# Zokrates/ZoKrates

Hardware: AMD Instinct MI355X
Metric: groth16_proofs_per_sec (higher is better)
Workload: dtype u32

## Files before the change

### zokrates_amd/csrc/core.cuh

```cuda
#pragma once
#include <algorithm>
#include <atomic>
#include <chrono>
#include <cstdio>
#include <memory>
#include <new>
#include <string>
#include <system_error>
#include <thread>
#include <type_traits>
#include <unordered_set>
#include <vector>

#include "../../include/zkhip.h"
#include "devrt.h"
#include "ntt_geom.h"
#include "msm_geom.h"
#include "ec.cuh"
#include "kernels_msm.cuh"
#include "kernels_ntt.cuh"
#include "zpack.cuh"
#include "wingest.cuh"
#include "wplan.h"
#include "wexec.cuh"
#include "xplan.h"

namespace zk {

struct CurveBn254 {
    static constexpr int ID = ZKHIP_CURVE_BN128;
    typedef Fe<Bn254Fr> Fr;
    typedef Fe<Bn254Fq> Fq;
    typedef Fe2<Bn254Fq> Fq2;
    static constexpr u64 GENERATOR = 5;
    static constexpr int TWO_ADICITY = 28;
    static const u32* g1_gen() { static const u32 t[] = {0x00000001u, 0x00000000u, 0x00000000u, 0x00000000u, 0x00000000u, 0x00000000u, 0x00000000u, 0x00000000u, 0x00000002u, 0x00000000u, 0x00000000u, 0x00000000u, 0x00000000u, 0x00000000u, 0x00000000u, 0x00000000u}; return t; }
    static const u32* g2_gen() { static const u32 t[] = {0xd992f6edu, 0x46debd5cu, 0xf75edaddu, 0x674322d4u, 0x5e5c4479u, 0x426a0066u, 0x121f1e76u, 0x1800deefu, 0xaef312c2u, 0x97e485b7u, 0x35a9e712u, 0xf1aa4933u, 0x31fb5d25u, 0x7260bfb7u, 0x920d483au, 0x198e9393u, 0x66fa7daau, 0x4ce6cc01u, 0x0c43d37bu, 0xe3d1e769u, 0x8dcb408fu, 0x4aab7180u, 0xdb8c6debu, 0x12c85ea5u, 0xd122975bu, 0x55acdadcu, 0x70b38ef3u, 0xbc4b3133u, 0x690c3395u, 0xec9e99adu, 0x585ff075u, 0x090689d0u}; return t; }
};
struct CurveBls381 {
    static constexpr int ID = ZKHIP_CURVE_BLS12_381;
    typedef Fe<Bls381Fr> Fr;
    typedef Fe<Bls381Fq> Fq;
    typedef Fe2<Bls381Fq> Fq2;
    static constexpr u64 GENERATOR = 7;
    static constexpr int TWO_ADICITY = 32;
    static const u32* g1_gen() { static const u32 t[] = {0xdb22c6bbu, 0xfb3af00au, 0xf97a1aefu, 0x6c55e83fu, 0x171bac58u, 0xa14e3a3fu, 0x9774b905u, 0xc3688c4fu, 0x4fa9ac0fu, 0x2695638cu, 0x3197d794u, 0x17f1d3a7u, 0x46c5e7e1u, 0x0caa2329u, 0xa2888ae4u, 0xd03cc744u, 0x2c04b3edu, 0x00db18cbu, 0xd5d00af6u, 0xfcf5e095u, 0x741d8ae4u, 0xa09e30edu, 0xe3aaa0f1u, 0x08b3f481u}; return t; }
    static const u32* g2_gen() { static const u32 t[] = {0xc121bdb8u, 0xd48056c8u, 0xa805bbefu, 0x0bac0326u, 0x7ae3d177u, 0xb4510b64u, 0xfa403b02u, 0xc6e47ad4u, 0x2dc51051u, 0x26080527u, 0xf08f0a91u, 0x024aa2b2u, 0x5d042b7eu, 0xe5ac7d05u, 0x13945d57u, 0x334cf112u, 0xdc7f5049u, 0xb5da61bbu, 0x9920b61au, 0x596bd0d0u, 0x88274f65u, 0x7dacd3a0u, 0x52719f60u, 0x13e02b60u, 0x08b82801u, 0xe1935486u, 0x3baca289u, 0x923ac9ccu, 0x5160d12cu, 0x6d429a69u, 0x8cbdd3a7u, 0xadfd9baau, 0xda2e351au, 0x8cc9cdc6u, 0x727d6e11u, 0x0ce5d527u, 0xf05f79beu, 0xaaa9075fu, 0x5cec1da1u, 0x3f370d27u, 0x572e99abu, 0x267492abu, 0x85a763afu, 0xcb3e287eu, 0x2bc28b99u, 0x32acd2b0u, 0x2ea734ccu, 0x0606c4a0u}; return t; }
};
struct CurveBls377 {
    static constexpr int ID = ZKHIP_CURVE_BLS12_377;
    typedef Fe<Bls377Fr> Fr;
    typedef Fe<Bls377Fq> Fq;
    typedef Fe2<Bls377Fq> Fq2;
    static constexpr u64 GENERATOR = 22;
    static constexpr int TWO_ADICITY = 47;
    static const u32* g1_gen() { static const u32 t[] = {0xb21be9efu, 0xeab9b16eu, 0xffcd394eu, 0xd5481512u, 0xbd37cb5cu, 0x188282c8u, 0xaa9d41bbu, 0x85951e2cu, 0xbf87ff54u, 0xc8fc6225u, 0xfe740a67u, 0x008848deu, 0x559c8ea6u, 0xfd82de55u, 0x34a9591au, 0xc2fe3d36u, 0x4fb82305u, 0x6d182ad4u, 0xca3e52d9u, 0xbd7fb348u, 0x30afeec4u, 0x1f674f5du, 0xc5102effu, 0x01914a69u}; return t; }
    static const u32* g2_gen() { static const u32 t[] = {0x7c005196u, 0x74e3e48fu, 0xbb535402u, 0x71889f52u, 0x57db6b9bu, 0x7ea501f5u, 0x203e5031u, 0xc565f071u, 0xa3841d01u, 0xc89630a2u, 0x71c785feu, 0x018480beu, 0x6ea16afeu, 0xb26bfefau, 0xbff76fe6u, 0x5cf89984u, 0x0799c9deu, 0xe7223eceu, 0x6651cecbu, 0x532777eeu, 0xb1b140d5u, 0x70dc5a51u, 0xe7004031u, 0x00ea6040u, 0x09fd4ddfu, 0xf0940944u, 0x6d8c7c2eu, 0xf2cf8888u, 0xf832d204u, 0xe458c282u, 0x74b49a58u, 0xde03ed72u, 0xcbb2efb4u, 0xd960736bu, 0x5d446f7bu, 0x00690d66u, 0x85eb8f93u, 0xd9a1cdd1u, 0x5e52270bu, 0x4279b83fu, 0xcee304c2u, 0x2463b01au, 0x3d591bf1u, 0x61ef11acu, 0x151a70aau, 0x9e549da3u, 0xd2835518u, 0x00f8169fu}; return t; }
};

struct ApiError {
    int32_t code;
    std::string msg;
};
static inline void require(bool ok, int32_t code, const char* msg) {
    if (!ok) throw ApiError{code, msg};
}
static const char* const Z0_NOT_ONE_MSG = "z[0] must be 1 (ark instance variable 0 is the constant ONE)";

struct DBuf {
    void* p = nullptr;
    size_t cap = 0;
    DBuf() {}
    DBuf(const DBuf&) = delete;
    DBuf& operator=(const DBuf&) = delete;
    ~DBuf() { dev_free(p); }
    void swap(DBuf& o) { std::swap(p, o.p); std::swap(cap, o.cap); }
    void release() { dev_free(p); p = nullptr; cap = 0; }
    void ensure(size_t bytes) {
        if (bytes <= cap) return;
        dev_free(p);
        p = nullptr;
        cap = 0;
        p = dev_alloc(bytes);
        cap = bytes;
    }
};
template <class T> static inline T* ptr(const DBuf& b) { return (T*)b.p; }

static inline unsigned blocks_for(u64 n, unsigned threads) { return (unsigned)((n + threads - 1) / threads); }
static inline int ilog2_floor(u64 x) { int l = 0; while (x >>= 1) ++l; return l; }
static inline int ilog2_ceil(u64 x) { int l = 0; while (((u64)1 << l) < x) ++l; return l; }

}

using namespace zk;

struct NttPlanBase {
    int curve, logN;
    virtual ~NttPlanBase() {}
};
struct MsmSort {
    DBuf dig, sorted, cnt, off, cursor, chunk_sum, grand;
    DBuf pairs, ccur, tile_off;
    Event ready = nullptr;
};
struct MsmLane {
    Stream stream = 0;
    bool made = false;
    bool high_priority = false;
    DBuf lane_key, heavy, partial, bucket, rows, cols;
    Event done = nullptr;
};
static constexpr int ZK_NLANES = 5;
static constexpr int ZK_NSLOTS = 4;
struct ProofSlot {
    DBuf scalars, zmont, va, vb, vc, ws1, ws2, zflag;
    DBuf verdict;
    int check_idx = -1;
    MsmSort sorts[3];
    MsmLane lanes[ZK_NLANES];
    void* h_ws = nullptr;
    size_t h_ws_cap = 0;
    Event ev[4] = {nullptr, nullptr, nullptr, nullptr};
    Event acc_b[ZK_NLANES] = {}, acc_e[ZK_NLANES] = {};
    Event ntt_b = nullptr, ntt_e = nullptr;
    Event g1_go = nullptr;
    Event half_ready = nullptr;
    int half = -1;
    bool lone = false;
    bool split_pending = false;
    const zkhip_pk* split_pk = nullptr;
    const zkhip_r1cs* split_cs = nullptr;
    bool split_bound = false;
    bool ready = false;
    bool busy = false;
    uint8_t r[32], s[32];
    std::shared_ptr<const WPlanTables> wit;
    void* h_inputs = nullptr;
    size_t h_inputs_cap = 0;
    std::chrono::steady_clock::time_point t_start;
};
struct PackedZ {
    const uint8_t* bytes;
    size_t len;
    u64 tags_off, index_off, payload_off;
};
struct zkhip_wplan;
struct WitnessZ {
    const uint8_t* bytes;
    size_t len;
    u64 count;
    const zkhip_wplan* plan;
};
struct zkhip_queue {
    zkhip_ctx* ctx = nullptr;
    const zkhip_pk* pk = nullptr;
    const zkhip_r1cs* cs = nullptr;
    u32 cap = 0;
    u64 head = 0, next = 0;
    bool checked = false;
    bool broken = false;
    std::string dev_err;
};
struct zkhip_ctx {
    int device = 0;
    Stream stream = 0;
    Stream out_stream = 0;
    Stream ntt_stream = 0;
    bool out_made = false, ntt_made = false;
    Stream ws = 0;
    bool serial = false;
    bool g2_first = true;
    MsmKnobs msm;
    int b_sort_mode = 0;
    bool fuse_z = true;
    int z_gate = 1;
    int g2_head_start = 1;
    int split_min_log = 18;
    int ntt_single_max = 10;
    int ntt_max_sublog = 11;
    int ntt_cols = 2;
    std::vector<Stream> idle_streams;
    std::string pipe_plan;
    bool pipes_made = false;
    Stream ntt_lone_stream = 0;
    bool ntt_lone_made = false;
    int ntt_fuse_first = 1;
    int tenants = 1;
    int nslots = 3;
    bool checked = false;
    struct Unsatisfied { u32 proof; u64 first_row, n_bad; };
    std::vector<Unsatisfied> unsat;
    std::string err;
    std::string desc;
    ProofSlot slots[ZK_NSLOTS];
    ProofSlot* cur = &slots[0];
    zkhip_queue* queue = nullptr;
    DBuf tmp;
    DBuf wraw, wowner;
    Stream verify_stream = 0;
    bool verify_made = false;
    DBuf vfy[11];
    Stream exec_stream = 0;
    bool exec_made = false;
    DBuf xstore, xargs, xverdict, xptrs, xfile, xinputs;
    int exec_chunk = 0;
    bool exec_wide = false;
    int exec_wide_min = 0;
    u64 exec_last[4] = {0, 0, 0, 0};
    DBuf zpack;
    std::vector<std::unique_ptr<NttPlanBase>> plans;
    std::unordered_set<const void*> lds_opted;
    struct Shard {
        DBuf send[2], recv, out;
        Event packed[2] = {nullptr, nullptr};
        unsigned turn = 0;
        std::vector<uint8_t> host;
    } shard;
};
#define ZK_PIPE_PLAN_RESIDENT "M=2,N=3,O=1,n=3,G0=0,Z0=1,H0=0,G1=3,Z1=1,H1=0,G2=3,Z2=2,H2=1"
struct PipeWant { Stream* target; bool* made; bool high; int cls; bool done; };
static inline void make_pipe_streams(zkhip_ctx* ctx) {
    if (ctx->pipes_made || ctx->pipe_plan.empty() || ctx->serial) return;
    ctx->pipes_made = true;
    auto find = [&](const std::string& key) -> int {
        size_t pos = 0;
        const std::string& pl = ctx->pipe_plan;
        while (pos < pl.size()) {
            size_t end = pl.find(',', pos);
            if (end == std::string::npos) end = pl.size();
            const std::string tok = pl.substr(pos, end - pos);
            const size_t eq = tok.find('=');
            if (eq != std::string::npos && tok.substr(0, eq) == key && eq + 1 < tok.size() && tok[eq + 1] >= '0' && tok[eq + 1] <= '3') return tok[eq + 1] - '0';
            pos = end + 1;
        }
        return -1;
    };
    std::vector<PipeWant> want;
    static bool dummy_made;
    int c;
    if ((c = find("M")) >= 0) { stream_sync(ctx->stream); stream_destroy(ctx->stream); ctx->stream = 0; want.push_back({&ctx->stream, &dummy_made, true, c, false}); }
    if ((c = find("N")) >= 0 && !ctx->ntt_made) want.push_back({&ctx->ntt_stream, &ctx->ntt_made, true, c, false});
    if ((c = find("n")) >= 0) want.push_back({&ctx->ntt_lone_stream, &ctx->ntt_lone_made, true, c, false});
    if ((c = find("O")) >= 0 && !ctx->out_made) want.push_back({&ctx->out_stream, &ctx->out_made, false, c, false});
    static const char names[3] = {'Z', 'G', 'H'};
    static const int lane_of[3] = {0, 3, 4};
    for (int k = 0; k < std::min(ctx->nslots, ZK_NSLOTS); ++k)
        for (int t = 0; t < 3; ++t) {
            MsmLane& lane = ctx->slots[k].lanes[lane_of[t]];
            const std::string up(1, names[t]);
            c = find(up + std::to_string(k)); if (c < 0) c = find(up);
            if (c >= 0 && !lane.made) want.push_back({&lane.stream, &lane.made, t == 1 && ctx->g2_first, c, false});
        }
    size_t left = want.size();
    for (int t = 0; left; ++t) {
        PipeWant* pick = nullptr;
        for (auto& w : want) if (!w.done && w.cls == (t & 3)) { pick = &w; break; }
        if (pick) { *pick->target = pick->high ? stream_create_high_priority() : stream_create(); *pick->made = true; pick->done = true; --left; }
        else ctx->idle_streams.push_back(stream_create_low_priority());
    }
    ctx->ws = ctx->stream;
}
static inline void slot_init(zkhip_ctx* ctx, ProofSlot& sl) {
    if (sl.ready) return;
    for (auto& so : sl.sorts) so.ready = event_create();
    for (int k = 0; k < ZK_NLANES; ++k) {
        sl.lanes[k].high_priority = k == 3 && ctx->g2_first;
        sl.lanes[k].done = event_create();
        sl.acc_b[k] = event_create();
// ... 770 lines not shown
    }
    static void export_image(zkhip_pk* pk, uint8_t* out, u64 cap) {
        zkhip_ctx* ctx = pk->ctx;
        require(cap >= export_size(pk), ZKHIP_ERR_BAD_ARG, "output buffer too small (see zkhip_pk_export_size)");
        PkImageHeader h;
        memset(&h, 0, sizeof(h));
        memcpy(h.magic, PK_IMAGE_MAGIC, 8);
        h.curve = pk->curve; h.scheme = pk->scheme;
        h.m = pk->m; h.w = pk->w; h.l = pk->l; h.hlen = pk->hlen; h.N = pk->N;
        h.logN = pk->logN; h.c_z = pk->c_z; h.c_h = pk->c_h; h.sets = pk->s_z | (pk->s_h << 8);
        h.rank = pk->rank; h.world = pk->world;
        h.ntt_split = pk->ntt_log1;
        h.z_lo = pk->z_lo; h.z_n = pk->z_n; h.h_lo = pk->h_lo; h.h_n = pk->h_n;
        h.len_delta = pk->delta_g1_canon.size(); h.len_g2z2 = pk->g_gamma2_z2_canon.size();
        const bool with_bound = pk->h_bound.p && pk->l_bound.p;
        if (with_bound) {
            h.len_bound[0] = table_bytes<Fq>(pk->h_n, 1);
            h.len_bound[1] = table_bytes<Fq>(pk->z_n, 1);
            h.bound_fp[0] = pk->bound_fp[0]; h.bound_fp[1] = pk->bound_fp[1];
        }
        uint8_t* p = out + sizeof(h);
        memcpy(p, pk->delta_g1_canon.data(), h.len_delta); p += h.len_delta;
        memcpy(p, pk->g_gamma2_z2_canon.data(), h.len_g2z2); p += h.len_g2z2;
        for_each_table(pk, [&](int k, DBuf& b, auto f, u64, u64 n) {
            h.len_buf[k] = table_bytes<typename decltype(f)::type>(n, 1);
            dev_d2h(p, b.p, h.len_buf[k], ctx->stream);
            p += h.len_buf[k];
        });
        memcpy(out, &h, sizeof(h));
        if (with_bound) {
            dev_d2h(p, pk->h_bound.p, h.len_bound[0], ctx->stream); p += h.len_bound[0];
            dev_d2h(p, pk->l_bound.p, h.len_bound[1], ctx->stream); p += h.len_bound[1];
        }
        stream_sync(ctx->stream);
    }
    static void import_image(zkhip_ctx* ctx, const uint8_t* bytes, size_t len, zkhip_pk* pk) {
        PkImageHeader h;
        memcpy(&h, bytes, sizeof(h));
        require(h.scheme == 0 || h.scheme == 1, ZKHIP_ERR_PARSE, "key image: unknown scheme");
        u64 total = sizeof(PkImageHeader), rest = len - sizeof(PkImageHeader);
        const u64 parts[9] = {h.len_delta, h.len_g2z2, h.len_buf[0], h.len_buf[1], h.len_buf[2], h.len_buf[3], h.len_buf[4], h.len_bound[0], h.len_bound[1]};
        for (u64 part : parts) {
            require(part <= rest, ZKHIP_ERR_PARSE, "key image truncated");
            rest -= part;
            total += part;
        }
        require(total == len, ZKHIP_ERR_PARSE, "trailing bytes after key image");
        int s_z = h.sets & 0xff, s_h = (h.sets >> 8) & 0xff;
        require(h.world >= 1 && h.rank < h.world && h.logN >= 0 && h.logN <= 3 * NTT_MAX_SUBLOG && h.N == ((u64)1 << h.logN) && h.z_n <= h.m + 2 &&
                    h.h_n <= h.N && h.c_z >= 2 && h.c_z <= MSM_MAX_C && h.c_h >= 2 && h.c_h <= MSM_MAX_C && s_z >= 1 && s_h >= 1 && (h.sets >> 16) == 0,
                ZKHIP_ERR_PARSE, "key image: inconsistent header");
        pk->scheme = h.scheme;
        pk->m = h.m; pk->w = h.w; pk->l = h.l; pk->hlen = h.hlen; pk->N = h.N; pk->logN = h.logN;
        pk->c_z = h.c_z; pk->c_h = h.c_h; pk->rank = h.rank; pk->world = h.world;
        pk->z_lo = h.z_lo; pk->z_n = h.z_n; pk->h_lo = h.h_lo; pk->h_n = h.h_n;
        pk->ntt_log1 = h.ntt_split;
        auto shape_z = [&](int sets) { return msm_shape(&ctx->msm,h.z_n, C::Fr::Params::BITS, true, h.c_z, sets); };
        auto shape_h = [&](int sets) { return msm_shape(&ctx->msm,h.h_n, C::Fr::Params::BITS, true, h.c_h, sets); };
        bool sizes_ok = h.m + 2 < ((u64)1 << 31) && h.z_lo <= h.m + 2 && h.z_n <= h.m + 2 - h.z_lo && h.h_lo <= h.N && h.h_n <= h.N - h.h_lo &&
                        h.len_delta <= 4096 && h.len_g2z2 <= 4096;
        for_each_table(pk, [&](int k, DBuf&, auto f, u64, u64 n) {
            sizes_ok = sizes_ok && h.len_buf[k] == table_bytes<typename decltype(f)::type>(n, 1);
        });
        const bool with_bound = h.len_bound[0] || h.len_bound[1];
        if (with_bound)
            sizes_ok = sizes_ok && h.len_bound[0] == table_bytes<Fq>(h.h_n, 1) && h.len_bound[1] == table_bytes<Fq>(h.z_n, 1) && (h.bound_fp[0] | h.bound_fp[1]) != 0;
        require(sizes_ok, ZKHIP_ERR_PARSE, "key image: array sizes do not match the header");
        require(get_plan<C>(ctx, h.logN)->split() == h.ntt_split, ZKHIP_ERR_PARSE,
                "key image: written under another NTT split (NTT_SINGLE_MAX_LOG / NTT_MAX_SUBLOG) than this context uses; re-import the proving key");
        {
            const int W_z = shape_z(1).W, W_h = shape_h(1).W;
            const int fixed = ctx->msm.msm_sets;
            const u64 budget = msm_table_budget(ctx, h.z_n, h.h_n, h.N, W_z, shape_z(1).K);
            if (fixed) s_z = std::min(fixed, W_z), s_h = std::min(fixed, W_h);
            else {
                const MsmSets s = msm_pick_sets({s_z, s_h}, {W_z, W_h}, {W_z, W_h}, budget, [&](MsmSets t) { return tables_need(pk, shape_z(t.z), shape_h(t.h)); });
                s_z = s.z, s_h = s.h;
            }
        }
        const MsmShape shz = shape_z(s_z), shh = shape_h(s_h);
        require(shz.c == h.c_z && (int)shz.sets == s_z && shh.c == h.c_h && (int)shh.sets == s_h, ZKHIP_ERR_PARSE,
                "key image: window width / bucket sets not usable under this context's settings; re-import the proving key");
        pk->s_z = s_z; pk->s_h = s_h;
        const uint8_t* p = bytes + sizeof(h);
        pk->delta_g1_canon.assign(p, p + h.len_delta); p += h.len_delta;
        pk->g_gamma2_z2_canon.assign(p, p + h.len_g2z2); p += h.len_g2z2;
        for_each_table(pk, shz, shh, [&](int k, DBuf& b, auto f, u64, u64 n, const MsmShape& sh) {
            b.ensure(table_bytes<typename decltype(f)::type>(n, sh.levels));
            const uint8_t* src = p;
            dev_h2d_fill(b.p, h.len_buf[k], 64, ctx->stream, [src](char* out, size_t off, size_t len) { memcpy(out, src + off, len); });
            p += h.len_buf[k];
        });
        stream_sync(ctx->stream);
        table_levels(ctx, pk);
        if (with_bound) install_bound(ctx, pk, p, p + h.len_bound[0], false, h.bound_fp);
    }
    static void count_points_at_infinity(zkhip_ctx* ctx, zkhip_pk* pk) {
        u64 cnt[5];
        for_each_table(pk, [&](int k, DBuf& b, auto f, u64, u64 n) {
            cnt[k] = count_infinite<typename decltype(f)::type>(ctx, b.p, n);
            pk->inf_many[k] = cnt[k] * 2048 > n;
        });
        const bool gm17 = pk->scheme == 1;
        u32 family = 0;
        if (ctx->b_sort_mode == 1) family = gm17 ? 0xbu : 0xau;
        else if (ctx->b_sort_mode == 0)
            for (int k = 0; k < 4; ++k)
                if (cnt[k] * 10 > pk->z_n) family |= 1u << k;
        pk->thin_mask = 0;
        pk->thin_keep.release();
        if (family && pk->z_n) {
            const size_t words = (size_t)((pk->z_n + 31) / 32);
            pk->thin_keep.ensure(words * 4);
            dev_memset(pk->thin_keep.p, 0, words * 4, ctx->stream);
            for_each_table(pk, [&](int k, DBuf& b, auto f, u64, u64 n) {
                if (family >> k & 1) mark_finite<typename decltype(f)::type>(ctx, b.p, n, ptr<u32>(pk->thin_keep));
            });
            std::vector<u32> host(words);
            dev_d2h(host.data(), pk->thin_keep.p, words * 4, ctx->stream);
            stream_sync(ctx->stream);
            u64 left_out = 0;
            for (u64 i = 0; i < pk->z_n; ++i) left_out += !((host[i >> 5] >> (i & 31)) & 1u);
            if (ctx->b_sort_mode == 1 || left_out * 10 > pk->z_n) {
                pk->thin_mask = family;
                for (int k = 0; k < 4; ++k) pk->inf_many_thin[k] = (cnt[k] - std::min(cnt[k], left_out)) * 2048 > pk->z_n;
            } else {
                pk->thin_keep.release();
            }
        }
    }
    template <class F>
    static void to_table(zkhip_ctx* ctx, DBuf& buf, u64 lo, u64 count, const MsmShape& sh) {
        DBuf out;
        out.ensure(table_bytes<F>(count, sh.levels));
        if (count) points_to_packed<F>(ctx, ptr<Aff<F>>(buf) + lo, out.p, count);
        stream_sync(ctx->stream);
        buf.swap(out);
        out.release();
        msm_table_levels<F>(ctx, buf.p, count, sh.level_bits(), (int)sh.levels);
    }
};

template <class C>
struct Prover {
    typedef typename C::Fr Fr;
    typedef typename C::Fq Fq;
    typedef typename C::Fq2 Fq2;
    typedef SlotSums<C> Lay;
    typedef Transforms<C> Tr;
    static constexpr int FQB = Fq::BYTES;

    static CsrDev csr(const zkhip_r1cs* cs, int k) { return CsrDev{ptr<u64>(cs->rp[k]), ptr<u32>(cs->col[k]), cs->val[k].p}; }

    static void matvec(zkhip_ctx* ctx, const zkhip_r1cs* cs, const Fr* zmont, Fr* a, Fr* b, Fr* c, u64 n, u64 l, u64 N, int nmat = 3, int mat0 = 0) {
        int g[3];
        matvec_lanes(cs, g, nmat, mat0);
        ZK_LAUNCH((k_matvec<Fr>), dim3(blocks_for(N, 256 / gmax_rows(g)), nmat), dim3(256), 0, ctx->ws, csr(cs, 0), csr(cs, 1), csr(cs, 2), zmont, a, b, c, n,
                  l, N, g[0], g[1], g[2], cs->l + cs->w, mat0);
        if (cs->n_huge)
            ZK_LAUNCH((k_matvec_huge<Fr>), dim3((unsigned)cs->n_huge), dim3(MATVEC_HUGE_THREADS), 0, ctx->ws, csr(cs, 0), csr(cs, 1), csr(cs, 2), zmont, a, b, c,
                      ptr<u64>(cs->long_rows), cs->l + cs->w);
        if (cs->n_long > cs->n_huge)
            ZK_LAUNCH((k_matvec_long<Fr>), dim3(blocks_for(cs->n_long - cs->n_huge, 4)), dim3(256), 0, ctx->ws, csr(cs, 0), csr(cs, 1), csr(cs, 2), zmont, a, b, c,
                      ptr<u64>(cs->long_rows) + cs->n_huge, cs->n_long - cs->n_huge, cs->l + cs->w);
    }
    static unsigned gmax_rows(const int g[3]) { return (unsigned)std::max(g[0], std::max(g[1], g[2])); }

    static void witness_map(zkhip_ctx* ctx, const zkhip_r1cs* cs, NttPlan<C>* pl, bool bound = false, int half = -1, bool check = false) {
        Stream s = ctx->ws;
        const u64 N = pl->N;
        ctx->cur->va.ensure(3 * N * sizeof(Fr));
        Fr *a = ptr<Fr>(ctx->cur->va), *b = a + N, *c = b + N;
        if (half >= 0) {
            Fr* v = a + (u64)half * N;
            matvec(ctx, cs, ptr<Fr>(ctx->cur->zmont), a, b, c, cs->n, cs->l, N, 1, half);
            event_record(ctx->cur->ntt_b, s);
            Tr::ntt_kind_a(ctx, pl, v, true, ptr<Fr>(pl->s_coset), 1, 0);
            Tr::ntt_kind_b(ctx, pl, v, false, nullptr, 1, 0);
            event_record(ctx->cur->ntt_e, s);
            return;
        }
        matvec(ctx, cs, ptr<Fr>(ctx->cur->zmont), a, b, c, cs->n, cs->l, N, (bound && !check) ? 2 : 3);
        if (check) enqueue_check(*ctx->cur, a, b, c, cs->n, s);
        event_record(ctx->cur->ntt_b, s);
        Tr::ntt_quotient(ctx, pl, a, 2, c, bound, [&](const Fr& zinv) {
            ZK_LAUNCH((k_quotient<typename Fr::Params>), dim3(blocks_for(N, 256)), dim3(256), 0, s, a, b, zinv, a, N);
        });
        event_record(ctx->cur->ntt_e, s);
    }

    static void verdict_reset(ProofSlot& sl, Stream st) {
        sl.verdict.ensure(16);
        dev_memset(sl.verdict.p, 0xff, 8, st);
        dev_memset((uint8_t*)sl.verdict.p + 8, 0, 8, st);
    }
    static void enqueue_check(ProofSlot& sl, const Fr* a, const Fr* b, const Fr* c, u64 n, Stream s) {
        ZK_LAUNCH((k_r1cs_check<typename Fr::Params>), dim3(blocks_for(n, 256)), dim3(256), 0, s, a, b, c, n, ptr<unsigned long long>(sl.verdict));
    }
    static bool unsatisfied(zkhip_ctx* ctx, const ProofSlot& sl, const Lay& ly) {
        if (sl.check_idx < 0) return false;
        u64 v[2];
        memcpy(v, ly.verdict(sl), 16);
        if (!v[1]) return false;
        ctx->unsat.push_back({(u32)sl.check_idx, v[0], v[1]});
        return true;
    }
    static void raise_unsatisfied(const zkhip_ctx* ctx, u32 count, const zkhip_r1cs* cs) {
        if (ctx->unsat.empty()) return;
        const auto& u = ctx->unsat.front();
        char msg[200];
        snprintf(msg, sizeof(msg), "proof %u of %u: constraint %llu of %llu is not satisfied (%llu in all)", u.proof, count, (unsigned long long)u.first_row,
                 (unsigned long long)cs->n, (unsigned long long)u.n_bad);
        throw ApiError{ZKHIP_ERR_UNSATISFIED, msg};
    }
    static void r1cs_check(zkhip_ctx* ctx, const zkhip_r1cs* cs, const uint8_t* z_host, const void* z_dev, u64 out[2]) {
        ProofSlot& sl = *ctx->cur;
        Stream s = ctx->stream;
        ctx->ws = s;
        const u64 m = cs->l + cs->w, n = cs->n;
        const Fr* z = stage_z(ctx, sl, m, m + 2, z_host, z_dev, true, true);
        sl.zmont.ensure(m * 32);
        ZK_LAUNCH((k_mul_const<Fr>), dim3(blocks_for(m, 256)), dim3(256), 0, s, z, ptr<Fr>(sl.zmont), m, fe_to_mont(rp_factor<Fr>()));
        sl.vc.ensure(3 * std::max<u64>(n, 1) * sizeof(Fr));
        Fr *ra = ptr<Fr>(sl.vc), *rb = ra + n, *rc = rb + n;
        if (n) matvec(ctx, cs, ptr<Fr>(sl.zmont), ra, rb, rc, n, 0, n);
        enqueue_check(sl, ra, rb, rc, n, s);
        u32 flag = 0;
        dev_d2h(&flag, sl.zflag.p, 4, s);
        dev_d2h(out, sl.verdict.p, 16, s);
        stream_sync(s);
        require_canonical(flag);
    }

    static void upload_z(zkhip_ctx* ctx, DBuf& dst, u64 m, u64 cap, const uint8_t* z, DBuf& flag) {
        Fr z0 = fe_from_bytes_canon<Fr>(z);
        Fr one = Fr::zero(); one.v[0] = 1;
        require(z0.equals(one), ZKHIP_ERR_BAD_ARG, Z0_NOT_ONE_MSG);
        dst.ensure(cap * 32);
        dev_h2d(dst.p, z, m * 32, ctx->stream);
        flag.ensure(4);
        dev_memset(flag.p, 0, 4, ctx->stream);
        ZK_LAUNCH((k_check_canonical<Fr>), dim3(blocks_for(m, 256)), dim3(256), 0, ctx->stream, ptr<Fr>(dst), m, ptr<u32>(flag));
    }
    static void unpack_z(zkhip_ctx* ctx, DBuf& dst, u64 m, u64 cap, const PackedZ& zp, DBuf& flag) {
        Stream s = ctx->stream;
        dst.ensure(cap * 32);
        ctx->zpack.ensure(zp.len);
        dev_h2d(ctx->zpack.p, zp.bytes, zp.len, s);
        flag.ensure(4);
        dev_memset(flag.p, 0, 4, s);
        const uint8_t* d = ptr<uint8_t>(ctx->zpack);
        ZK_LAUNCH((k_unpack_assignment<Fr>), dim3(blocks_for(m, ZPACK_BLOCK_ELEMS)), dim3(256), 0, s, d + zp.tags_off, (const u64*)(d + zp.index_off),
                  d + zp.payload_off, ptr<Fr>(dst), m, ptr<u32>(flag));
    }
    static void ingest_z(zkhip_ctx* ctx, DBuf& dst, u64 m, u64 cap, const WitnessZ& wz, DBuf& flag) {
        Stream s = ctx->stream;
        const zkhip_wplan* plan = wz.plan;
        const u64 slots = (wz.len + 15) / 16;
        dst.ensure(cap * 32);
        ctx->wraw.ensure(slots * 16);
        ctx->wowner.ensure(m * 4);
        dev_h2d(ctx->wraw.p, wz.bytes, wz.len, s);
        dev_memset(ctx->wowner.p, 0, m * 4, s);
        flag.ensure(16);
        dev_memset(flag.p, 0, 8, s);
        dev_memset((uint8_t*)flag.p + 8, 0xff, 8, s);
        ZK_LAUNCH((k_witness_claim<Fr>), dim3(blocks_for(wz.count, WIT_BLOCK)), dim3(WIT_BLOCK), 0, s, ptr<uint4>(ctx->wraw), slots, wz.count, ptr<u32>(plan->pos),
                  (u64)plan->host->pos.size(), ptr<u32>(plan->neg), (u64)plan->host->neg.size(), witness_id_bound(wz.count), ptr<u32>(ctx->wowner), ptr<u32>(flag));
        ZK_LAUNCH((k_witness_gather<Fr>), dim3(blocks_for(m, WIT_BLOCK)), dim3(WIT_BLOCK), 0, s, ptr<uint8_t>(ctx->wraw), ptr<u32>(ctx->wowner), ptr<Fr>(dst), m,
                  ptr<u32>(flag), (unsigned long long*)((uint8_t*)flag.p + 8));
    }
    static void require_verdict(u32 flag, u32 low, const WPlanTables* wit) {
        require(!(flag & WIT_FLAG_NON_CANONICAL), ZKHIP_ERR_PARSE, "non-canonical field element in the witness");
        require(!(flag & WIT_FLAG_ID_RANGE), ZKHIP_ERR_PARSE, "variable id out of range in the witness");
        if (flag & WIT_FLAG_MISSING) {
            const std::string name = wit && low < wit->order.size() ? witness_var_name(wit->order[low]) : "column " + std::to_string(low);
            throw ApiError{ZKHIP_ERR_UNSATISFIED, "assignment missing for variable " + name};
        }
        require_canonical(flag);
    }
    static void require_verdict(const ProofSlot& sl, const Lay& ly) {
        u32 low = 0;
        memcpy(&low, ly.zflag(sl) + 4, 4);
        require_verdict(ly.zflag_word(sl), low, sl.wit.get());
    }
    static const Fr* stage_z(zkhip_ctx* ctx, ProofSlot& sl, u64 m, u64 cap, const uint8_t* z_host, const void* z_dev, bool checked, bool in_place = false,
                             const PackedZ* zp = nullptr, const WitnessZ* wz = nullptr) {
        Stream st = ctx->stream;
        sl.wit.reset();
        if (wz) {
            const u64 l = wz->plan->host->l;
            if (sl.h_inputs_cap < l * 32) {
                host_free_pinned(sl.h_inputs);
                sl.h_inputs = nullptr; sl.h_inputs_cap = 0;
                sl.h_inputs = host_alloc_pinned(l * 32);
                sl.h_inputs_cap = l * 32;
            }
            ingest_z(ctx, sl.scalars, m, cap, *wz, sl.zflag);
            dev_d2h_pinned(sl.h_inputs, sl.scalars.p, l * 32, st);
            sl.wit = wz->plan->host;
            if (checked) verdict_reset(sl, st);
            return ptr<Fr>(sl.scalars);
        }
        if (zp) {
            unpack_z(ctx, sl.scalars, m, cap, *zp, sl.zflag);
            if (checked) verdict_reset(sl, st);
            return ptr<Fr>(sl.scalars);
        }
        if (z_host) {
            upload_z(ctx, sl.scalars, m, cap, z_host, sl.zflag);
        } else {
            if (!in_place) {
                sl.scalars.ensure(cap * 32);
                dev_d2d(sl.scalars.p, z_dev, m * 32, st);
            }
            sl.zflag.ensure(4);
            dev_memset(sl.zflag.p, 0, 4, st);
        }
        if (checked) verdict_reset(sl, st);
        return (z_host || !in_place) ? ptr<Fr>(sl.scalars) : (const Fr*)z_dev;
    }
    static void require_canonical(u32 flag) {
        require(flag == 0, ZKHIP_ERR_BAD_ARG, "an assignment entry is not a canonical field element (>= r)");
    }
    static void stage_scalars(zkhip_ctx* ctx, NttPlan<C>* pl, void* d_scalars, u64 m, const uint8_t* r, const uint8_t* s_) {
        Stream s = ctx->stream;
        ctx->cur->zmont.ensure(m * 32);
        dev_h2d((uint8_t*)d_scalars + m * 32, r, 32, s);
        dev_h2d((uint8_t*)d_scalars + (m + 1) * 32, s_, 32, s);
        ZK_LAUNCH((k_mul_const<Fr>), dim3(blocks_for(m, 256)), dim3(256), 0, s, (const Fr*)d_scalars, ptr<Fr>(ctx->cur->zmont), m, pl->k_to_rp);
    }

    static void enqueue(zkhip_ctx* ctx, ProofSlot& sl, const zkhip_pk* pk, const zkhip_r1cs* cs, const uint8_t* z_host, const void* z_dev,
                        const uint8_t* r, const uint8_t* s_, bool lone = false, int check_idx = -1, const PackedZ* zp = nullptr,
                        const WitnessZ* wz = nullptr) {
        enqueue_head(ctx, sl, pk, cs, z_host, z_dev, r, s_, lone, -1, check_idx, zp, wz);
        enqueue_tail(ctx, sl, pk, cs);
    }
    static bool can_split(const zkhip_ctx* ctx, const zkhip_pk* pk, const zkhip_r1cs* cs) {
        return pk->scheme == 0 && is_bound(pk, cs) && pk->logN >= ctx->split_min_log;
    }
    static bool is_bound(const zkhip_pk* pk, const zkhip_r1cs* cs) { return pk->bound_uid != 0 && pk->bound_uid == cs->uid; }
    static NttPlan<C>* open_slot(zkhip_ctx* ctx, ProofSlot& sl, const zkhip_pk* pk) {
        require(!sl.busy, ZKHIP_ERR_DEVICE, "internal: proof slot still in flight");
        make_pipe_streams(ctx);
        slot_init(ctx, sl);
        NttPlan<C>* pl = get_plan<C>(ctx, pk->logN);
        require(pl->split() == pk->ntt_log1, ZKHIP_ERR_BAD_ARG, "the key's h bases were ordered for another NTT split (NTT_SINGLE_MAX_LOG changed): reload the key");
        sl.t_start = std::chrono::steady_clock::now();
        ctx->cur = &sl;
        ctx->ws = ctx->stream;
        return pl;
    }
    static void enqueue_head(zkhip_ctx* ctx, ProofSlot& sl, const zkhip_pk* pk, const zkhip_r1cs* cs, const uint8_t* z_host, const void* z_dev,
                             const uint8_t* r, const uint8_t* s_, bool lone, int half, int check_idx = -1, const PackedZ* zp = nullptr,
                             const WitnessZ* wz = nullptr) {
        PkLoader<C>::check_match(pk, cs, 0);
        const bool bound = is_bound(pk, cs);
        require(half < 0 || (bound && half <= 1), ZKHIP_ERR_BAD_ARG, "internal: only a proof over a bound key splits its witness map");
        Fr rr = fe_from_bytes_canon<Fr>(r), ss = fe_from_bytes_canon<Fr>(s_);
        require(canon_lt_mod(rr) && canon_lt_mod(ss), ZKHIP_ERR_BAD_ARG, "r or s not a canonical field element");
        NttPlan<C>* pl = open_slot(ctx, sl, pk);
        sl.half = half;
        sl.lone = lone;
        sl.check_idx = half < 0 ? check_idx : -1;
        memcpy(sl.r, r, 32);
        memcpy(sl.s, s_, 32);
        Stream st = ctx->stream;
        stage_z(ctx, sl, pk->m, pk->m + 2, z_host, z_dev, sl.check_idx >= 0, false, zp, wz);
        stage_scalars(ctx, pl, sl.scalars.p, pk->m, r, s_);
        event_record(sl.ev[0], st);

        const Lay ly(ctx, pk);
        ly.reserve(sl);
        start_z_lanes(ctx, sl, pk, ly);

        Stream wn = ctx->serial ? st : slot_ntt_stream(ctx, sl);
        stream_wait_event(wn, sl.ev[0]);
        event_record(sl.ev[1], wn);
        ctx->ws = wn;
        witness_map(ctx, cs, pl, bound, half, sl.check_idx >= 0);
        ctx->ws = ctx->stream;
        if (half >= 0) {
            event_record(sl.half_ready, wn);
            sl.split_pk = pk;
            sl.split_cs = cs;
            sl.split_bound = bound;
            sl.split_pending = true;
        }
    }
    static void enqueue_tail(zkhip_ctx* ctx, ProofSlot& sl, const zkhip_pk* pk, const zkhip_r1cs* cs) {
        const u64 N = pk->N;
        ctx->cur = &sl;
        Stream wn = ctx->serial ? ctx->stream : slot_ntt_stream(ctx, sl);
        const u32* h_scalars = ptr<u32>(sl.va) + (sl.half >= 0 ? 2 * N * 8 : 0);
        if (sl.half >= 0) {
            Fr* a = ptr<Fr>(sl.va);
            ZK_LAUNCH((k_quotient<typename Fr::Params>), dim3(blocks_for(N, 256)), dim3(256), 0, wn, a, a + N, fe_from_mont(get_plan<C>(ctx, pk->logN)->zinv), a + 2 * N, N);
        }
        lanes_after_h(ctx, sl, pk, Lay(ctx, pk), sl.half >= 0 ? sl.split_bound : is_bound(pk, cs), sl.lone, h_scalars, wn);
    }

    static void start_z_lanes(zkhip_ctx* ctx, ProofSlot& sl, const zkhip_pk* pk, const Lay& ly) {
        if (!pk->z_n) return;
        const u32* digits = ptr<u32>(sl.scalars) + pk->z_lo * 8;
        msm_prepare(ctx, ctx->stream, sl.sorts[0], digits, ly.shz, pk->z_n);
        if (pk->thin_mask) msm_prepare(ctx, ctx->stream, sl.sorts[2], digits, ly.shz, pk->z_n, ptr<u32>(pk->thin_keep), &sl.sorts[0]);
        if (z_gate(ctx) < 2) run_g2(ctx, sl, pk, ly, nullptr);
    }
    static void run_g2(zkhip_ctx* ctx, ProofSlot& sl, const zkhip_pk* pk, const Lay& ly, Event after) {
        const bool thin = pk->thin_mask & 8;
        msm_run<Fq2>(ctx, sl.lanes[3], sl.sorts[thin ? 2 : 0], pk->b2_ext.p, with_inf(ly.shz, thin ? pk->inf_many_thin[3] : pk->inf_many[3]), ly.ws2(sl),
                     sl.acc_b[4], sl.acc_e[4], after, ly.hs2(sl));
    }
    static void lanes_after_h(zkhip_ctx* ctx, ProofSlot& sl, const zkhip_pk* pk, const Lay& ly, bool bound, bool lone, const u32* h_scalars, Stream wn) {
        Stream st = ctx->stream;
        event_record(sl.ev[2], wn);
        if (pk->z_n) {
            const int gate = z_gate(ctx);
            const Event h_ready = gate ? sl.ev[2] : nullptr;
            if (gate >= 2) run_g2(ctx, sl, pk, ly, h_ready);
            Event g1_after = h_ready;
            constexpr bool g2_owns_simds = MsmTuning<typename Unsat<Fq2>::type>::ACCUM_WPE == 1;
            if (g2_owns_simds && lone && !ctx->serial && (ctx->g2_head_start == 2 || (ctx->g2_head_start == 1 && bound))) {
                if (h_ready) stream_wait_event(st, h_ready);
                stream_wait_event(st, sl.acc_e[4]);
                event_record(sl.g1_go, st);
                g1_after = sl.g1_go;
            }
            run_z_g1(ctx, sl, pk, ly, g1_after, bound);
        } else {
            empty_msm(ctx, sl, ly, true);
        }
        if (pk->h_n) {
            msm_prepare(ctx, wn, sl.sorts[1], h_scalars + pk->h_lo * 8, ly.shh, pk->h_n);
            msm_run<Fq>(ctx, sl.lanes[4], sl.sorts[1], bound ? pk->h_bound.p : pk->h_sigma.p, with_inf(ly.shh, bound ? pk->inf_many_bound[1] : pk->inf_many[4]),
                        ly.ws1(sl, 3), sl.acc_b[3], sl.acc_e[3], nullptr, ly.hs1(sl, 3));
        } else {
            empty_msm(ctx, sl, ly, false);
        }
        copy_out(ctx, sl, ly);
    }

    static void run_z_g1(zkhip_ctx* ctx, ProofSlot& sl, const zkhip_pk* pk, const Lay& ly, Event h_ready, bool bound) {
        const void* tab[3] = {pk->a_ext.p, pk->b1_ext.p, bound ? pk->l_bound.p : pk->l_ext.p};
        auto thin = [&](int k) { return (bound && k == 2) ? 0u : (pk->thin_mask >> k) & 1u; };
        auto inf_many = [&](int k) { return (bound && k == 2) ? pk->inf_many_bound[0] : thin(k) ? pk->inf_many_thin[k] : pk->inf_many[k]; };
        if (!ctx->fuse_z) {
            for (int k = 0; k < 3; ++k)
                msm_run<Fq>(ctx, sl.lanes[k], thin(k) ? sl.sorts[2] : sl.sorts[0], tab[k], with_inf(ly.shz, inf_many(k)), ly.ws1(sl, k), sl.acc_b[k], sl.acc_e[k], h_ready,
                            ly.hs1(sl, k));
            return;
        }
        for (u32 which = 0; which < 2; ++which) {
            int member[3], nm = 0;
            for (int k = 0; k < 3; ++k)
                if (thin(k) == which) member[nm++] = k;
            if (!nm) continue;
            const int lead = member[0];
            const void* tabs[3];
            bool many = false;
            for (int q = 0; q < nm; ++q) { tabs[q] = tab[member[q]]; many = many || inf_many(member[q]); }
            const int step = nm > 1 ? member[1] - member[0] : 1;
            msm_run_tables<Fq>(ctx, sl.lanes[lead], which ? sl.sorts[2] : sl.sorts[0], tabs, nm, with_inf(ly.shz, many), ly.ws1(sl, lead), (u32)(step * ly.Wmax),
                               sl.acc_b[lead], sl.acc_e[lead], h_ready, ly.hs1(sl, lead));
            Stream s0 = ctx->serial ? ctx->stream : lane_stream(sl.lanes[lead]);
            for (int q = 1; q < nm; ++q) {
                event_record(sl.acc_b[member[q]], s0);
                event_record(sl.acc_e[member[q]], s0);
                event_record(sl.lanes[member[q]].done, s0);
            }
        }
    }

    static void copy_out(zkhip_ctx* ctx, ProofSlot& sl, const Lay& ly) {
        Stream st = ctx->stream;
        Stream so = ctx->serial ? st : ctx_out_stream(ctx);
        for (int k = 0; k < ZK_NLANES; ++k) stream_wait_event(so, sl.lanes[k].done);
        sl.zflag.ensure(4);
        dev_d2h_pinned(ly.zflag(sl), sl.zflag.p, 4, so);
        if (sl.wit) dev_d2h_pinned(ly.zflag(sl) + 4, (const uint8_t*)sl.zflag.p + 8, 4, so);
        if (sl.check_idx >= 0) {
            stream_wait_event(so, sl.ev[2]);
            dev_d2h_pinned(ly.verdict(sl), sl.verdict.p, 16, so);
        }
        event_record(sl.ev[3], so);
        sl.busy = true;
    }

    static void empty_msm(zkhip_ctx* ctx, ProofSlot& sl, const Lay& ly, bool over_z) {
        Stream st = ctx->stream;
        const int k0 = over_z ? 0 : 3, nk = over_z ? 3 : 1;
        dev_memset(ly.ws1(sl, k0), 0, nk * ly.lane_bytes(), st);
        memset(ly.hs1(sl, k0), 0, nk * ly.lane_bytes());
        if (over_z) {
            dev_memset(ly.ws2(sl), 0, ly.b2(), st);
            memset(ly.hs2(sl), 0, ly.b2());
        }
        for (int k = over_z ? 0 : 4; k < (over_z ? 4 : 5); ++k) {
            const int e = k == 3 ? 4 : k == 4 ? 3 : k;
            event_record(sl.acc_b[e], st);
            event_record(sl.acc_e[e], st);
            event_record(sl.lanes[k].done, st);
        }
    }

    struct Sums {
        Xyzz<Fq> a, b1, l, h;
        Xyzz<Fq2> b2;
    };
    static Sums collect(zkhip_ctx* ctx, ProofSlot& sl, const zkhip_pk* pk) {
        require(sl.busy, ZKHIP_ERR_DEVICE, "internal: no proof in flight in this slot");
        event_sync(sl.ev[3]);
        sl.busy = false;
        split_clear(sl);
        const Lay ly(ctx, pk);
        require_verdict(sl, ly);
        Sums g;
        HostThreads th;
        th.run([&] { g.a = msm_combine(ly.hs1(sl, 0), ly.shz); });
        th.run([&] { g.b1 = msm_combine(ly.hs1(sl, 1), ly.shz); });
        th.run([&] { g.l = msm_combine(ly.hs1(sl, 2), ly.shz); });
        th.run([&] { g.h = msm_combine(ly.hs1(sl, 3), ly.shh); });
// ... 38 lines not shown
        out[8 * FQB] = inf_a; out[8 * FQB + 1] = inf_b; out[8 * FQB + 2] = inf_c;
    }
    static constexpr size_t PROOF_BYTES = 8 * FQB + 3;
    static void fill_timings(ProofSlot& sl, zkhip_timings* tm, std::chrono::steady_clock::time_point t_fin) {
        const auto t_end = std::chrono::steady_clock::now();
        if (tm) {
            memset(tm, 0, sizeof(*tm));
            for (int k = 0; k < 4; ++k) tm->msm_z_ms = std::max(tm->msm_z_ms, event_elapsed_ms(sl.ev[0], sl.lanes[k].done));
            tm->ntt_ms = event_elapsed_ms(sl.ev[1], sl.ev[2]);
            tm->kernel_ntt_ms = event_elapsed_ms(sl.ntt_b, sl.ntt_e);
            tm->msm_h_ms = event_elapsed_ms(sl.ev[2], sl.lanes[4].done);
            tm->finish_ms = std::chrono::duration<float, std::milli>(t_end - t_fin).count();
            tm->total_ms = std::chrono::duration<float, std::milli>(t_end - sl.t_start).count();
            for (int k = 0; k < 4; ++k) tm->kernel_msm_accum_g1_ms += event_elapsed_ms(sl.acc_b[k], sl.acc_e[k]);
            tm->kernel_msm_accum_g2_ms = event_elapsed_ms(sl.acc_b[4], sl.acc_e[4]);
        }
    }
    static void finish(zkhip_ctx* ctx, ProofSlot& sl, const zkhip_pk* pk, uint8_t* out, zkhip_timings* tm) {
        require(pk->world == 1, ZKHIP_ERR_BAD_ARG, "this proving key is one shard of a multi-GPU key: use zkhip_prove_g16_partial + zkhip_combine_g16");
        require(sl.busy, ZKHIP_ERR_DEVICE, "internal: no proof in flight in this slot");
        const Lay ly(ctx, pk);
        const Fr rr = fe_from_bytes_canon<Fr>(sl.r), ss = fe_from_bytes_canon<Fr>(sl.s);
        Sums g;
        Xyzz<Fq> sA, rB1, rsD;
        std::chrono::steady_clock::time_point t_fin;
        try {
            HostThreads th;
            th.run([&] { rsD = rs_delta(pk, rr, ss); });
            event_sync(sl.lanes[3].done);
            g.b2 = msm_combine(ly.hs2(sl), ly.shz);
            for (int k = 0; k < 3; ++k) event_sync(sl.lanes[k].done);
            g.a = msm_combine(ly.hs1(sl, 0), ly.shz);
            g.b1 = msm_combine(ly.hs1(sl, 1), ly.shz);
            th.run([&] { sA = xyzz_mul_limbs(g.a, ss.v, Fr::N); });
            th.run([&] { rB1 = xyzz_mul_limbs(g.b1, rr.v, Fr::N); });
            g.l = msm_combine(ly.hs1(sl, 2), ly.shz);
            event_sync(sl.lanes[4].done);
            t_fin = std::chrono::steady_clock::now();
            g.h = msm_combine(ly.hs1(sl, 3), ly.shh);
            event_sync(sl.ev[3]);
            th.join();
        } catch (...) {
            sl.busy = false;
            throw;
        }
        sl.busy = false;
        require_verdict(sl, ly);
        if (unsatisfied(ctx, sl, ly)) memset(out, 0, PROOF_BYTES);
        else assemble_tail(g, sA, rB1, rsD, out);
        fill_timings(sl, tm, t_fin);
    }
    static Xyzz<Fq> rs_delta(const zkhip_pk* pk, const Fr& rr, const Fr& ss) {
        const Fr rs = fe_from_mont(fe_mul(fe_to_mont(rr), fe_to_mont(ss)));
        uint8_t dec[2 * FQB];
        decode_point<FQB, 2>(pk->delta_g1_canon.data(), dec);
        Aff<Fq> d1;
        memcpy(&d1, dec, sizeof(d1));
        d1 = PkLoader<C>::to_mont_point(d1);
        return xyzz_mul_limbs(Xyzz<Fq>::from_affine(d1), rs.v, Fr::N);
    }
    template <class F>
    static Xyzz<F> canonical(const Xyzz<F>& p) {
        if (p.is_inf()) return Xyzz<F>::inf();
        const Aff<F> a = xyzz_to_affine(p);
        return {a.x, a.y, F::one(), F::one()};
    }
    static void emit_partial(zkhip_ctx* ctx, ProofSlot& sl, const zkhip_pk* pk, uint8_t* partial_out, zkhip_timings* tm) {
        Sums g = collect(ctx, sl, pk);
        const auto t_fin = std::chrono::steady_clock::now();
        HostThreads th;
        th.run([&] { g.a = canonical(g.a); });
        th.run([&] { g.b1 = canonical(g.b1); });
        th.run([&] { g.l = canonical(g.l); });
        th.run([&] { g.h = canonical(g.h); });
        g.b2 = canonical(g.b2);
        th.join();
        memcpy(partial_out, &g, sizeof(g));
        fill_timings(sl, tm, t_fin);
    }
    static void prove_partial(zkhip_ctx* ctx, const zkhip_pk* pk, const zkhip_r1cs* cs, const uint8_t* z_host, const void* z_dev, const uint8_t* r,
                              const uint8_t* s_, uint8_t* partial_out, zkhip_timings* tm) {
        enqueue(ctx, ctx->slots[0], pk, cs, z_host, z_dev, r, s_);
        emit_partial(ctx, ctx->slots[0], pk, partial_out, tm);
    }
    static void split_begin(zkhip_ctx* ctx, const zkhip_pk* pk, const zkhip_r1cs* cs, const uint8_t* z_host, const void* z_dev, const uint8_t* r,
                            const uint8_t* s_, int half) {
        require(is_bound(pk, cs) && pk->scheme == 0 && (half == 0 || half == 1), ZKHIP_ERR_BAD_ARG,
                "only a Groth16 proof over a key bound to its constraint system splits its witness map (half = 0: a, 1: b)");
        enqueue_head(ctx, ctx->slots[0], pk, cs, z_host, z_dev, r, s_, false, half);
    }
    static const void* split_half_ptr(zkhip_ctx* ctx, const zkhip_pk* pk, int half) { return ptr<Fr>(ctx->slots[0].va) + (u64)half * pk->N; }
    static void split_clear(ProofSlot& sl) {
        sl.split_pending = false;
        sl.split_pk = nullptr;
        sl.split_cs = nullptr;
        sl.half = -1;
    }
    static ProofSlot& split_slot(zkhip_ctx* ctx, const zkhip_pk* pk, Stream* wn = nullptr) {
        ProofSlot& s0 = ctx->slots[0];
        require(s0.split_pending && s0.half >= 0, ZKHIP_ERR_BAD_ARG, "no split proof pending in this context");
        require(s0.split_pk == pk, ZKHIP_ERR_BAD_ARG, "the split proof pending in this context was begun with another proving key");
        if (wn) *wn = ctx->serial ? ctx->stream : ctx_ntt_stream(ctx);
        return ctx->slots[0];
    }
    static void split_fetch(zkhip_ctx* ctx, const zkhip_pk* pk, const void* src, int src_device, Event src_ready) {
        Stream wn;
        ProofSlot& sl = split_slot(ctx, pk, &wn);
        if (src_ready) event_sync(src_ready);
        dev_copy_between(ptr<Fr>(sl.va) + (u64)(1 - sl.half) * pk->N, ctx->device, src, src_device, pk->N * sizeof(Fr), wn);
    }
    static void split_fetch_host(zkhip_ctx* ctx, const zkhip_pk* pk, const uint8_t* other_half) {
        Stream wn;
        ProofSlot& sl = split_slot(ctx, pk, &wn);
        dev_h2d(ptr<Fr>(sl.va) + (u64)(1 - sl.half) * pk->N, other_half, pk->N * sizeof(Fr), wn);
    }
    static void split_half_out(zkhip_ctx* ctx, const zkhip_pk* pk, uint8_t* out) {
        Stream wn;
        ProofSlot& sl = split_slot(ctx, pk, &wn);
        dev_d2h(out, ptr<Fr>(sl.va) + (u64)sl.half * pk->N, pk->N * sizeof(Fr), wn);
        stream_sync(wn);
    }
    static void split_end_partial(zkhip_ctx* ctx, const zkhip_pk* pk, const zkhip_r1cs* cs, uint8_t* partial_out, zkhip_timings* tm) {
        ProofSlot& sl = split_slot(ctx, pk);
        require(sl.split_cs == cs, ZKHIP_ERR_BAD_ARG, "the split proof pending in this context was begun with another constraint system");
        enqueue_tail(ctx, sl, pk, cs);
        emit_partial(ctx, ctx->slots[0], pk, partial_out, tm);
    }
    static void split_end_device_sums(zkhip_ctx* ctx, const zkhip_pk* pk, const zkhip_r1cs* cs, const void** d_ws1, size_t* b1, const void** d_ws2, size_t* b2,
                                      zkhip_timings* tm) {
        ProofSlot& sl = split_slot(ctx, pk);
        require(sl.split_cs == cs, ZKHIP_ERR_BAD_ARG, "the split proof pending in this context was begun with another constraint system");
        enqueue_tail(ctx, sl, pk, cs);
        hand_out_sums(ctx, ctx->slots[0], pk, d_ws1, b1, d_ws2, b2, tm);
    }
    static int can_shard(zkhip_ctx* ctx, const zkhip_pk* pk, const zkhip_r1cs* cs, u32 G, u32 k) {
        if (pk->scheme != 0 || is_bound(pk, cs)) return -1;
        const NttPlan<C>* pl = get_plan<C>(ctx, pk->logN);
        return (Tr::shard_ok(pl, G) && pk->h_lo == (u64)k * (pl->N / G) && pk->h_n == pl->N / G) ? pl->split() : -1;
    }
    static void shard_begin(zkhip_ctx* ctx, const zkhip_pk* pk, const zkhip_r1cs* cs, const uint8_t* z_host, const uint8_t* r, const uint8_t* s_, u32 G, u32 k) {
        ProofSlot& sl = ctx->slots[0];
        PkLoader<C>::check_match(pk, cs, 0);
        require(z_host && pk->scheme == 0 && !is_bound(pk, cs), ZKHIP_ERR_BAD_ARG, "internal: only a Groth16 proof over an unbound key shards its witness map");
        Fr rr = fe_from_bytes_canon<Fr>(r), ss = fe_from_bytes_canon<Fr>(s_);
        require(canon_lt_mod(rr) && canon_lt_mod(ss), ZKHIP_ERR_BAD_ARG, "r or s not a canonical field element");
        NttPlan<C>* pl = open_slot(ctx, sl, pk);
        sl.half = -1;
        sl.lone = false;
        sl.check_idx = -1;
        memcpy(sl.r, r, 32);
        memcpy(sl.s, s_, 32);
        Stream st = ctx->stream;
        stage_z(ctx, sl, pk->m, pk->m + 2, z_host, nullptr, false);
        stage_scalars(ctx, pl, sl.scalars.p, pk->m, r, s_);
        event_record(sl.ev[0], st);
        const Lay ly(ctx, pk);
        ly.reserve(sl);
        start_z_lanes(ctx, sl, pk, ly);
        Stream wn = ctx->serial ? st : slot_ntt_stream(ctx, sl);
        stream_wait_event(wn, sl.ev[0]);
        event_record(sl.ev[1], wn);
        ctx->ws = wn;
        shard_witness_map(ctx, cs, pl, G, k, 0, nullptr);
        ctx->ws = ctx->stream;
        sl.split_pk = pk;
        sl.split_cs = cs;
        sl.split_bound = false;
        sl.split_pending = true;
    }
    static ProofSlot& shard_slot(zkhip_ctx* ctx, const zkhip_pk* pk, const zkhip_r1cs* cs) {
        ProofSlot& s0 = ctx->slots[0];
        require(s0.split_pending && s0.half < 0 && s0.split_pk == pk && s0.split_cs == cs, ZKHIP_ERR_BAD_ARG, "no sharded proof of these handles pending in this context");
        return s0;
    }
    static void shard_step(zkhip_ctx* ctx, const zkhip_pk* pk, const zkhip_r1cs* cs, u32 G, u32 k, int step, zkhip_ctx* const* members) {
        ProofSlot& sl = shard_slot(ctx, pk, cs);
        ctx->cur = &sl;
        ctx->ws = ctx->serial ? ctx->stream : slot_ntt_stream(ctx, sl);
        shard_witness_map(ctx, cs, get_plan<C>(ctx, pk->logN), G, k, step, members);
        ctx->ws = ctx->stream;
    }
    static void shard_end_partial(zkhip_ctx* ctx, const zkhip_pk* pk, const zkhip_r1cs* cs, uint8_t* partial_out, zkhip_timings* tm) {
        ProofSlot& sl = shard_slot(ctx, pk, cs);
        enqueue_tail(ctx, sl, pk, cs);
        emit_partial(ctx, ctx->slots[0], pk, partial_out, tm);
    }
    static void shard_end_device_sums(zkhip_ctx* ctx, const zkhip_pk* pk, const zkhip_r1cs* cs, const void** d_ws1, size_t* b1, const void** d_ws2, size_t* b2,
                                      zkhip_timings* tm) {
        ProofSlot& sl = shard_slot(ctx, pk, cs);
        enqueue_tail(ctx, sl, pk, cs);
        hand_out_sums(ctx, ctx->slots[0], pk, d_ws1, b1, d_ws2, b2, tm);
    }
    static void prove_device_sums(zkhip_ctx* ctx, const zkhip_pk* pk, const zkhip_r1cs* cs, const uint8_t* z_host, const uint8_t* r,
                                  const uint8_t* s_, const void** d_ws1, size_t* b1, const void** d_ws2, size_t* b2, zkhip_timings* tm) {
        enqueue(ctx, ctx->slots[0], pk, cs, z_host, nullptr, r, s_);
        hand_out_sums(ctx, ctx->slots[0], pk, d_ws1, b1, d_ws2, b2, tm);
    }
    static void hand_out_sums(zkhip_ctx* ctx, ProofSlot& sl, const zkhip_pk* pk, const void** d_ws1, size_t* b1, const void** d_ws2, size_t* b2,
                              zkhip_timings* tm) {
        require(sl.busy, ZKHIP_ERR_DEVICE, "internal: no proof in flight in this slot");
        event_sync(sl.ev[3]);
        sl.busy = false;
        split_clear(sl);
        const Lay ly(ctx, pk);
        *b1 = ly.b1();
        *b2 = ly.b2();
        require_canonical(ly.zflag_word(sl));
        *d_ws1 = sl.ws1.p;
        *d_ws2 = sl.ws2.p;
        fill_timings(sl, tm, std::chrono::steady_clock::now());
    }
    static void record_from_sums(zkhip_ctx* ctx, const zkhip_pk* pk, const uint8_t* ws1, const uint8_t* ws2, uint8_t* record_out) {
        const Lay ly(ctx, pk);
        std::vector<Xyzz<Fq>> a1(ly.b1() / sizeof(Xyzz<Fq>));
        std::vector<Xyzz<Fq2>> a2(ly.b2() / sizeof(Xyzz<Fq2>));
        memcpy(a1.data(), ws1, ly.b1());
        memcpy(a2.data(), ws2, ly.b2());
        Sums g;
        g.a = msm_combine(ly.lane(a1.data(), 0), ly.shz);
        g.b1 = msm_combine(ly.lane(a1.data(), 1), ly.shz);
        g.l = msm_combine(ly.lane(a1.data(), 2), ly.shz);
        g.h = msm_combine(ly.lane(a1.data(), 3), ly.shh);
        g.b2 = msm_combine(a2.data(), ly.shz);
        memcpy(record_out, &g, sizeof(g));
    }
    static Sums sum_partials(u32 count, const uint8_t* partials) {
        Sums t;
        t.a = t.b1 = t.l = t.h = Xyzz<Fq>::inf();
        t.b2 = Xyzz<Fq2>::inf();
        for (u32 i = 0; i < count; ++i) {
            Sums g;
            memcpy(&g, partials + (size_t)i * sizeof(Sums), sizeof(g));
            t.a = xyzz_add(t.a, g.a); t.b1 = xyzz_add(t.b1, g.b1); t.l = xyzz_add(t.l, g.l); t.h = xyzz_add(t.h, g.h);
            t.b2 = xyzz_add(t.b2, g.b2);
        }
        return t;
    }
    static void combine(const zkhip_pk* pk, u32 count, const uint8_t* partials, const uint8_t* r, const uint8_t* s_, uint8_t* out) {
        const Sums t = sum_partials(count, partials);
        Fr rr = fe_from_bytes_canon<Fr>(r), ss = fe_from_bytes_canon<Fr>(s_);
        require(canon_lt_mod(rr) && canon_lt_mod(ss), ZKHIP_ERR_BAD_ARG, "r or s not a canonical field element");
        assemble(pk, t, r, s_, out);
    }
    static constexpr size_t PARTIAL_BYTES = sizeof(Sums);

    static void prove(zkhip_ctx* ctx, const zkhip_pk* pk, const zkhip_r1cs* cs, const uint8_t* z_host, const void* z_dev, const uint8_t* r, const uint8_t* s_,
                      uint8_t* out, zkhip_timings* tm) {
        ctx->unsat.clear();
        enqueue(ctx, ctx->slots[0], pk, cs, z_host, z_dev, r, s_, true, ctx->checked ? 0 : -1);
        finish(ctx, ctx->slots[0], pk, out, tm);
        raise_unsatisfied(ctx, 1, cs);
    }
    template <class Enq, class Fin>
    static void run_batch(zkhip_ctx* ctx, const zkhip_r1cs* cs, u32 count, zkhip_timings* tm, Enq enq, Fin fin) {
        zkhip_timings acc, one;
        memset(&acc, 0, sizeof(acc));
        const auto t0 = std::chrono::steady_clock::now();
        ctx->unsat.clear();
        try {
            const u32 NS = (u32)ctx->nslots;
            for (u32 i = 0; i < count + NS - 1; ++i) {
                if (i < count) enq(i, ctx->slots[i % NS]);
                if (i >= NS - 1 && i - (NS - 1) < count) {
                    const u32 j = i - (NS - 1);
                    fin(j, ctx->slots[j % NS], &one);
                    float* a = (float*)&acc; const float* b = (const float*)&one;
                    for (size_t k = 0; k < sizeof(acc) / sizeof(float); ++k) a[k] += b[k];
                }
            }
        } catch (...) {
            for (auto& sl : ctx->slots) sl.busy = false;
            dev_sync_all();
            throw;
        }
        if (tm) {
            *tm = acc;
            tm->total_ms = std::chrono::duration<float, std::milli>(std::chrono::steady_clock::now() - t0).count();
        }
        raise_unsatisfied(ctx, count, cs);
    }
    static void prove_batch(zkhip_ctx* ctx, const zkhip_pk* pk, const zkhip_r1cs* cs, u32 count, const uint8_t* z_host, void* const* z_dev,
                            const uint8_t* rs, uint8_t* proofs_out, zkhip_timings* tm) {
        run_batch(ctx, cs, count, tm,
                  [&](u32 i, ProofSlot& sl) {
                      enqueue(ctx, sl, pk, cs, z_host ? z_host + (size_t)i * pk->m * 32 : nullptr, z_host ? nullptr : z_dev[i], rs + (size_t)i * 64,
                              rs + (size_t)i * 64 + 32, false, ctx->checked ? (int)i : -1);
                  },
                  [&](u32 j, ProofSlot& sl, zkhip_timings* one) { finish(ctx, sl, pk, proofs_out + (size_t)j * PROOF_BYTES, one); });
    }
    static void assignment_upload(zkhip_ctx* ctx, zkhip_assignment* a, const uint8_t* z) {
        DBuf flag;
        upload_z(ctx, a->scalars, a->m, a->m + 2, z, flag);
        u32 verdict = 0;
        dev_d2h(&verdict, flag.p, 4, ctx->stream);
        stream_sync(ctx->stream);
        require_canonical(verdict);
    }
    static void assignment_upload_packed(zkhip_ctx* ctx, zkhip_assignment* a, const uint8_t* packed, size_t len, u64 tags_off, u64 index_off,
                                         u64 payload_off) {
        Stream s = ctx->stream;
        DBuf flag;
        unpack_z(ctx, a->scalars, a->m, a->m + 2, PackedZ{packed, len, tags_off, index_off, payload_off}, flag);
        u32 verdict = 0;
        dev_d2h(&verdict, flag.p, 4, s);
        stream_sync(s);
        require_canonical(verdict);
    }
// ... 18 lines not shown
        const u64 per_instance = h.store_bytes_per_instance() + h.n_args * 32 + 4 + sizeof(void*) + (witness_out ? file_bytes : 0) + (inputs_out ? n_in * 32 : 0);
        const u64 chunk = std::min<u64>(ctx->exec_chunk > 0 ? (u64)ctx->exec_chunk : exec_chunk_default(ctx, per_instance), count);
        ctx->xstore.ensure(h.slots * chunk * sizeof(Fr));
        ctx->xargs.ensure(std::max<u64>(h.n_args, 1) * chunk * 32);
        ctx->xverdict.ensure(chunk * 4);
        if (made) ctx->xptrs.ensure(chunk * sizeof(void*));
        if (witness_out) ctx->xfile.ensure(chunk * file_bytes);
        if (inputs_out) ctx->xinputs.ensure(std::max<u64>(n_in, 1) * chunk * 32);
        std::vector<u32> verdict(chunk);
        std::vector<void*> ptrs(chunk);
        std::vector<uint8_t> tmp;
        u64 n_failed = 0;
        const bool wide = ctx->exec_wide;
        const u32 wide_min = (u32)(ctx->exec_wide_min > 0 ? ctx->exec_wide_min : EXEC_WIDE_MIN_DEFAULT);
        const u32 n_levels = h.level_start.empty() ? 0 : (u32)h.level_start.size() - 1;
        u64 launches = 1;
        if (wide) {
            launches = 0;
            bool in_run = false;
            for (u32 lv = 0; lv < n_levels; ++lv) {
                const bool narrow = h.level_start[lv + 1] - h.level_start[lv] < wide_min;
                launches += !narrow || !in_run;
                in_run = narrow;
            }
        }
        ctx->exec_last[0] = wide ? 2 : 1;
        ctx->exec_last[1] = (count + chunk - 1) / chunk;
        ctx->exec_last[2] = launches;
        ctx->exec_last[3] = wide_min;
        for (u64 c0 = 0; c0 < count; c0 += chunk) {
            const u32 c = (u32)std::min<u64>(chunk, count - c0);
            const dim3 waves(blocks_for(c, WX_BLOCK));
            if (h.n_args) dev_h2d(ctx->xargs.p, args + c0 * h.n_args * 32, (size_t)c * h.n_args * 32, s);
            if (!wide) {
                ZK_LAUNCH((k_exec_program<Fr>), waves, dim3(WX_BLOCK), 0, s, ptr<u32>(plan->code), ptr<u32>(plan->pool), ptr<uint8_t>(ctx->xargs), (u32)h.n_args, c, chunk,
                          ptr<Fr>(ctx->xstore), ptr<u32>(ctx->xverdict));
            } else {
                ZK_LAUNCH((k_exec_begin<Fr>), waves, dim3(WX_BLOCK), 0, s, c, ptr<Fr>(ctx->xstore), ptr<u32>(ctx->xverdict));
                for (u32 lv = 0; lv < n_levels;) {
                    const u32 first = h.level_start[lv], width = h.level_start[lv + 1] - first;
                    if (width >= wide_min) {
                        ZK_LAUNCH((k_exec_level<Fr>), dim3(blocks_for(width, WX_BLOCK), std::min<u32>(c, 65535)), dim3(WX_BLOCK), 0, s, ptr<u32>(plan->code), ptr<u32>(plan->pool),
                                  ptr<u32>(plan->sched), first, width, ptr<uint8_t>(ctx->xargs), (u32)h.n_args, c, chunk, ptr<Fr>(ctx->xstore), ptr<u32>(ctx->xverdict));
                        ++lv;
                        continue;
                    }
                    u32 end = lv + 1;
                    while (end < n_levels && h.level_start[end + 1] - h.level_start[end] < wide_min) ++end;
                    ZK_LAUNCH((k_exec_levels_run<Fr>), dim3(c), dim3(WX_RUN_BLOCK), 0, s, ptr<u32>(plan->code), ptr<u32>(plan->pool), ptr<u32>(plan->sched),
                              ptr<u32>(plan->level_start), lv, end, ptr<uint8_t>(ctx->xargs), (u32)h.n_args, chunk, ptr<Fr>(ctx->xstore), ptr<u32>(ctx->xverdict));
                    lv = end;
                }
            }
            dev_d2h(verdict.data(), ctx->xverdict.p, (size_t)c * 4, s);
            stream_sync(s);
            for (u32 i = 0; i < c; ++i) {
                const bool ok = verdict[i] == WX_RAN_THROUGH;
                n_failed += !ok;
                status[c0 + i] = ok ? ZKHIP_OK : ZKHIP_ERR_UNSATISFIED;
                const u64 st = ok ? ~(u64)0 : verdict[i];
                if (first_statement) first_statement[c0 + i] = st;
                if (first_row) first_row[c0 + i] = ok || st >= h.row_of.size() || h.row_of[st] == XPLAN_NO_ROW ? ~(u64)0 : h.row_of[st];
                ptrs[i] = nullptr;
                if (made && ok) {
                    std::unique_ptr<zkhip_assignment> a(new zkhip_assignment());
                    a->curve = h.curve; a->ctx = ctx; a->m = m;
                    a->scalars.ensure((m + 2) * 32);
                    ptrs[i] = a->scalars.p;
                    (*made)[c0 + i] = std::move(a);
                }
            }
            if (made) {
                dev_h2d(ctx->xptrs.p, ptrs.data(), (size_t)c * sizeof(void*), s);
                ZK_LAUNCH((k_exec_gather<Fr>), dim3((unsigned)(m + 2), waves.x), dim3(WX_BLOCK), 0, s, ptr<Fr>(ctx->xstore), chunk, c, (const u32*)nullptr, m,
                          ptr<u32>(ctx->xverdict), (Fr* const*)ctx->xptrs.p, (Fr*)nullptr, (u64)0, 1, 2u);
            }
            if (witness_out) {
                ZK_LAUNCH((k_exec_witness_file<Fr>), dim3((unsigned)entries, waves.x), dim3(WX_BLOCK), 0, s, ptr<Fr>(ctx->xstore), chunk, c,
                          (const long long*)plan->file_ids.p, ptr<u32>(plan->file_slots), entries, ptr<u32>(ctx->xverdict), ptr<uint8_t>(ctx->xfile), file_bytes);
                if (witness_cap_each == file_bytes) {
                    dev_d2h(witness_out + c0 * file_bytes, ctx->xfile.p, (size_t)c * file_bytes, s);
                } else {
                    tmp.resize((size_t)c * file_bytes);
                    dev_d2h(tmp.data(), ctx->xfile.p, tmp.size(), s);
                    stream_sync(s);
                    for (u32 i = 0; i < c; ++i) memcpy(witness_out + (c0 + i) * witness_cap_each, tmp.data() + (size_t)i * file_bytes, file_bytes);
                }
            }
            if (inputs_out && n_in) {
                ZK_LAUNCH((k_exec_gather<Fr>), dim3((unsigned)n_in, waves.x), dim3(WX_BLOCK), 0, s, ptr<Fr>(ctx->xstore), chunk, c, ptr<u32>(plan->input_cols), n_in,
                          ptr<u32>(ctx->xverdict), (Fr* const*)nullptr, ptr<Fr>(ctx->xinputs), n_in, 0, 0u);
                if (inputs_cap_each == n_in) {
                    dev_d2h(inputs_out + c0 * n_in * 32, ctx->xinputs.p, (size_t)c * n_in * 32, s);
                } else {
                    tmp.resize((size_t)c * n_in * 32);
                    dev_d2h(tmp.data(), ctx->xinputs.p, tmp.size(), s);
                    stream_sync(s);
                    for (u32 i = 0; i < c; ++i) memcpy(inputs_out + (c0 + i) * inputs_cap_each * 32, tmp.data() + (size_t)i * n_in * 32, n_in * 32);
                }
            }
            stream_sync(s);
        }
        return n_failed;
    }

    template <class F, int NC>
    static void msm_api(zkhip_ctx* ctx, u64 n, const uint8_t* bases, const uint8_t* scalars, uint8_t* out) {
        constexpr int PB = FQB * NC;
        memset(out, 0, PB + 1);
        if (n == 0) { out[PB] = 1; return; }
        require(n < ((u64)1 << 31), ZKHIP_ERR_BAD_ARG, "too many points");
        Stream s = ctx->stream;
        std::vector<uint8_t> host(n * PB);
        for (u64 i = 0; i < n; ++i) decode_point<FQB, NC>(bases + i * PB, &host[i * PB]);
        DBuf d_bases, d_ws;
        d_bases.ensure(host.size());
        dev_h2d(d_bases.p, host.data(), host.size(), s);
        ZK_LAUNCH((k_to_mont<Fq>), dim3(blocks_for(n * NC, 256)), dim3(256), 0, s, ptr<Fq>(d_bases), ptr<Fq>(d_bases), n * NC);
        ctx->cur->scalars.ensure(n * 32);
        dev_h2d(ctx->cur->scalars.p, scalars, n * 32, s);
        const MsmShape sh = msm_shape(&ctx->msm,n, Fr::Params::BITS, false);
        d_ws.ensure((size_t)sh.nsums() * sizeof(Xyzz<F>));
        DBuf d_packed;
        d_packed.ensure(n * packed_point_bytes<F>());
#ifdef ZK_TEST_MSM_RACE
        msm_prepare(ctx, s, ctx->cur->sorts[0], ptr<u32>(ctx->cur->scalars), sh, 0);
        points_to_packed<F>(ctx, ptr<Aff<F>>(d_bases), d_packed.p, n);
#else
        points_to_packed<F>(ctx, ptr<Aff<F>>(d_bases), d_packed.p, n);
        msm_prepare(ctx, s, ctx->cur->sorts[0], ptr<u32>(ctx->cur->scalars), sh, 0);
#endif
        msm_run<F>(ctx, ctx->cur->lanes[0], ctx->cur->sorts[0], d_packed.p, sh, ptr<Xyzz<F>>(d_ws), nullptr, nullptr);
        stream_wait_event(s, ctx->cur->lanes[0].done);
        std::vector<Xyzz<F>> ws(sh.nsums());
        dev_d2h(ws.data(), d_ws.p, ws.size() * sizeof(Xyzz<F>), s);
        stream_sync(s);
        Xyzz<F> res = msm_combine(ws.data(), sh);
        if (res.is_inf()) { out[PB] = 1; return; }
        Aff<F> a = xyzz_to_affine(res);
        uint8_t tmp[sizeof(Aff<F>)];
        Aff<F> canon = from_mont_point(a);
        memcpy(tmp, &canon, sizeof(canon));
        memcpy(out, tmp, PB);
    }
    static Aff<Fq> from_mont_point(const Aff<Fq>& p) { return {fe_from_mont(p.x), fe_from_mont(p.y)}; }
    static Aff<Fq2> from_mont_point(const Aff<Fq2>& p) { return {fe_from_mont(p.x), fe_from_mont(p.y)}; }

    static void witness_map_api(zkhip_ctx* ctx, const zkhip_r1cs* cs, const uint8_t* z, uint8_t* h_out) {
        ctx->ws = ctx->stream;
        NttPlan<C>* pl = get_plan<C>(ctx, cs->logN);
        const u64 m = cs->l + cs->w;
        uint8_t zero[32] = {0};
        upload_z(ctx, ctx->cur->scalars, m, m + 2, z, ctx->cur->zflag);
        stage_scalars(ctx, pl, ctx->cur->scalars.p, m, zero, zero);
        witness_map(ctx, cs, pl);
        ctx->cur->vb.ensure(pl->N * sizeof(Fr));
        ZK_LAUNCH((k_sigma_permute<Fr>), dim3(blocks_for(pl->N, 256)), dim3(256), 0, ctx->stream, ptr<Fr>(ctx->cur->va), ptr<Fr>(ctx->cur->vb), pl->N,
                  pl->N1, pl->N2, 1, pl->N3);
        dev_d2h(h_out, ctx->cur->vb.p, pl->N * 32, ctx->stream);
        stream_sync(ctx->stream);
    }

    static void shard_witness_map(zkhip_ctx* ctx, const zkhip_r1cs* cs, NttPlan<C>* pl, u32 G, u32 k, int step, zkhip_ctx* const* members, bool check = false) {
        require(Tr::shard_ok(pl, G), ZKHIP_ERR_BAD_ARG, "internal: this transform does not shard");
        const ShardGeom g = ntt_shard_geom(pl->N1, pl->Nb, G);
        Stream s = ctx->ws;
        const u64 N = pl->N;
        Fr *a = ptr<Fr>(ctx->cur->va), *b = a + N, *c = b + N;
        const bool three = pl->log3 > 0;
        if (step == 0) {
            ctx->cur->va.ensure(3 * N * sizeof(Fr));
            a = ptr<Fr>(ctx->cur->va); b = a + N; c = b + N;
            Tr::shard_state(ctx, g, 3);
            matvec(ctx, cs, ptr<Fr>(ctx->cur->zmont), a, b, c, cs->n, cs->l, N, 3);
            if (check) enqueue_check(*ctx->cur, a, b, c, cs->n, s);
            event_record(ctx->cur->ntt_b, s);
            Tr::ntt_cols(ctx, pl, g, k, a, true, ptr<Fr>(pl->tw_inv), 3, N);
            Tr::shard_pack(ctx, g, k, a, 3, N, true);
        } else if (step == 1) {
            Tr::shard_fetch(ctx, g, k, a, 3, N, false, members);
            if (three) Tr::ntt_mid(ctx, pl, g, k, a, true, ptr<Fr>(pl->tw2_inv), pl->Nb - 1, 3, N);
            Tr::ntt_rows(ctx, pl, g, k, a, true, ptr<Fr>(pl->s_coset), 2, N);
            Tr::ntt_rows(ctx, pl, g, k, c, true, ptr<Fr>(pl->s_cexit), 1, 0, 1);
            if (three) {
                Tr::ntt_rows(ctx, pl, g, k, a, false, ptr<Fr>(pl->tw2_fwd), 2, N, 0, nullptr, pl->Nb - 1);
                Tr::ntt_mid(ctx, pl, g, k, a, false, ptr<Fr>(pl->tw_fwd), ~(u64)0, 2, N);
            } else {
                Tr::ntt_rows(ctx, pl, g, k, a, false, ptr<Fr>(pl->tw_fwd), 2, N);
            }
            Tr::shard_pack(ctx, g, k, a, 2, N, false);
        } else if (step == 2) {
            Tr::shard_fetch(ctx, g, k, a, 2, N, true, members);
            Tr::ntt_cols(ctx, pl, g, k, a, false, nullptr, 2, N);
            const u64 off = g.strip_origin(k);
            ZK_LAUNCH((k_quotient_strip<typename Fr::Params>), dim3(blocks_for(g.range_len(), 256)), dim3(256), 0, s, a + off, b + off, pl->zinv_rp, a + off, pl->N1,
                      ilog2_floor(g.W), pl->Nb);
            Tr::ntt_cols(ctx, pl, g, k, a, true, ptr<Fr>(pl->tw_inv), 1, 0);
            Tr::shard_pack(ctx, g, k, a, 1, 0, true);
        } else {
            Tr::shard_fetch(ctx, g, k, a, 1, 0, false, members);
            if (three) Tr::ntt_mid(ctx, pl, g, k, a, true, ptr<Fr>(pl->tw2_inv), pl->Nb - 1, 1, 0);
            Tr::ntt_rows(ctx, pl, g, k, a, true, ptr<Fr>(pl->s_cosetinv_canon), 1, 0, 1, c);
            event_record(ctx->cur->ntt_e, s);
        }
    }
    static int witness_map_shardable_api(zkhip_ctx* ctx, const zkhip_r1cs* cs, u32 G) { return Tr::ntt_shardable_api(ctx, (u32)cs->logN, G); }
    static void shard_witness_map_api(zkhip_ctx* ctx, const zkhip_r1cs* cs, const uint8_t* z, uint8_t* h_out, u32 G, u32 k, int step, zkhip_ctx* const* members) {
        ctx->ws = ctx->stream;
        NttPlan<C>* pl = get_plan<C>(ctx, cs->logN);
        if (step == 0) {
            const u64 m = cs->l + cs->w;
            uint8_t zero[32] = {0};
            upload_z(ctx, ctx->cur->scalars, m, m + 2, z, ctx->cur->zflag);
            stage_scalars(ctx, pl, ctx->cur->scalars.p, m, zero, zero);
        }
        shard_witness_map(ctx, cs, pl, G, k, step, members);
        if (step == 3) Tr::range_out(ctx, pl, ntt_shard_geom(pl->N1, pl->Nb, G), k, ptr<Fr>(ctx->cur->va), 0, Fr::one(), Fr::one(), h_out);
    }

    template <class F, class Launch>
    static void field_op_api(zkhip_ctx* ctx, u64 count, unsigned T, const uint8_t* a, const uint8_t* b, uint8_t* out, Launch launch) {
        Stream s = ctx->stream;
        const size_t bytes = count * sizeof(F);
        ctx->cur->va.ensure(bytes); ctx->cur->vb.ensure(bytes);
        dev_h2d(ctx->cur->va.p, a, bytes, s);
        dev_h2d(ctx->cur->vb.p, b, bytes, s);
        const unsigned B = blocks_for(count, T);
        ZK_LAUNCH((k_to_mont<F>), dim3(B), dim3(T), 0, s, ptr<F>(ctx->cur->va), ptr<F>(ctx->cur->va), count);
        ZK_LAUNCH((k_to_mont<F>), dim3(B), dim3(T), 0, s, ptr<F>(ctx->cur->vb), ptr<F>(ctx->cur->vb), count);
        launch(dim3(B), dim3(T), s, ptr<F>(ctx->cur->va), ptr<F>(ctx->cur->vb));
        ZK_LAUNCH((k_from_mont<F>), dim3(B), dim3(T), 0, s, ptr<F>(ctx->cur->va), ptr<F>(ctx->cur->va), count);
        dev_d2h(out, ctx->cur->va.p, bytes, s);
        stream_sync(s);
    }

    static void r1cs_load(zkhip_ctx* ctx, zkhip_r1cs* cs, const u64* const rp[3], const u32* const col[3], const uint8_t* const val[3]) {
        Stream s = ctx->stream;
        std::vector<u64> long_rows, huge_rows;
        const u64 huge_min = env_int("ZKHIP_MATVEC_HUGE", 0, 1, 1) ? (u64)MATVEC_HUGE : ~(u64)0;
        for (int k = 0; k < 3; ++k) {
            const u64 nnz = rp[k][cs->n];
            require(rp[k][0] == 0, ZKHIP_ERR_BAD_ARG, "rowptr[0] must be 0");
            for (u64 i = 0; i < cs->n; ++i) require(rp[k][i] <= rp[k][i + 1], ZKHIP_ERR_BAD_ARG, "rowptr not monotone");
            cs->nnz_short[k] = nnz;
            for (u64 i = 0; i < cs->n; ++i)
                if (rp[k][i + 1] - rp[k][i] > MATVEC_LONG) {
                    (rp[k][i + 1] - rp[k][i] > huge_min ? huge_rows : long_rows).push_back((u64)k << 32 | i);
                    cs->nnz_short[k] -= rp[k][i + 1] - rp[k][i];
                }
            for (u64 q = 0; q < nnz; ++q) require(col[k][q] < cs->l + cs->w, ZKHIP_ERR_BAD_ARG, "column index out of range");
            cs->nnz[k] = nnz;
            cs->rp[k].ensure((cs->n + 1) * 8);
            cs->col[k].ensure(std::max<u64>(nnz, 1) * 4);
            cs->val[k].ensure(std::max<u64>(nnz, 1) * 32);
            dev_h2d(cs->rp[k].p, rp[k], (cs->n + 1) * 8, s);
            if (nnz) {
                dev_h2d(cs->col[k].p, col[k], nnz * 4, s);
                dev_h2d(cs->val[k].p, val[k], nnz * 32, s);
                ZK_LAUNCH((k_to_mont<Fr>), dim3(blocks_for(nnz, 256)), dim3(256), 0, s, ptr<Fr>(cs->val[k]), ptr<Fr>(cs->val[k]), nnz);
            }
        }
        cs->n_huge = huge_rows.size();
        long_rows.insert(long_rows.begin(), huge_rows.begin(), huge_rows.end());
        cs->n_long = long_rows.size();
        if (cs->n_long) {
            cs->long_rows.ensure(cs->n_long * 8);
            dev_h2d(cs->long_rows.p, long_rows.data(), cs->n_long * 8, s);
        }
        stream_sync(s);
    }
};

}

#include "setup.cuh"
#include "gm17.cuh"
#include "pairing.cuh"

namespace zk {
struct CurveOps {
    void (*pk_load)(zkhip_ctx*, int scheme, const uint8_t*, size_t, zkhip_pk*);
    u64 (*pk_export_size)(const zkhip_pk*);
    void (*pk_export)(zkhip_pk*, uint8_t*, u64);
    void (*pk_import)(zkhip_ctx*, const uint8_t*, size_t, zkhip_pk*);
    void (*pk_bind)(zkhip_ctx*, zkhip_pk*, const zkhip_r1cs*);
    void (*pk_bind_check)(zkhip_ctx*, const zkhip_pk*, const zkhip_r1cs*);
    void (*pk_unbind)(zkhip_pk*);
    void (*bound_level0_from_file)(zkhip_ctx*, int scheme, const zkhip_r1cs*, const uint8_t*, size_t, std::vector<uint8_t>&, std::vector<uint8_t>&, u64 fp[2]);
    void (*install_bound_ranges)(zkhip_ctx*, zkhip_pk*, const zkhip_r1cs*, const uint8_t*, size_t, const uint8_t*, size_t, const u64 fp[2]);
    void (*r1cs_fingerprint)(zkhip_ctx*, const zkhip_r1cs*, u64 fp[2]);
    bool (*can_split)(const zkhip_ctx*, const zkhip_pk*, const zkhip_r1cs*);
    void (*split_begin)(zkhip_ctx*, const zkhip_pk*, const zkhip_r1cs*, const uint8_t*, const void*, const uint8_t*, const uint8_t*, int half);
    const void* (*split_half_ptr)(zkhip_ctx*, const zkhip_pk*, int half);
    void (*split_fetch)(zkhip_ctx*, const zkhip_pk*, const void*, int, Event);
    void (*split_fetch_host)(zkhip_ctx*, const zkhip_pk*, const uint8_t*);
    void (*split_half_out)(zkhip_ctx*, const zkhip_pk*, uint8_t*);
    void (*split_end_partial)(zkhip_ctx*, const zkhip_pk*, const zkhip_r1cs*, uint8_t*, zkhip_timings*);
    void (*split_end_device_sums)(zkhip_ctx*, const zkhip_pk*, const zkhip_r1cs*, const void**, size_t*, const void**, size_t*, zkhip_timings*);
    void (*r1cs_load)(zkhip_ctx*, zkhip_r1cs*, const u64* const rp[3], const u32* const col[3], const uint8_t* const val[3]);
    void (*prove)(zkhip_ctx*, const zkhip_pk*, const zkhip_r1cs*, const uint8_t* z_host, const void* z_dev, const uint8_t*, const uint8_t*, uint8_t*,
                  zkhip_timings*);
    void (*prove_batch)(zkhip_ctx*, const zkhip_pk*, const zkhip_r1cs*, u32, const uint8_t*, void* const*, const uint8_t*, uint8_t*, zkhip_timings*);
    void (*prove_partial)(zkhip_ctx*, const zkhip_pk*, const zkhip_r1cs*, const uint8_t*, const void*, const uint8_t*, const uint8_t*, uint8_t*,
                          zkhip_timings*);
    void (*combine)(const zkhip_pk*, u32, const uint8_t*, const uint8_t*, const uint8_t*, uint8_t*);
    size_t partial_bytes;
    void (*prove_device_sums)(zkhip_ctx*, const zkhip_pk*, const zkhip_r1cs*, const uint8_t*, const uint8_t*, const uint8_t*, const void**, size_t*,
                              const void**, size_t*, zkhip_timings*);
    void (*gm17_prove_device_sums)(zkhip_ctx*, const zkhip_pk*, const zkhip_r1cs*, const uint8_t*, const uint8_t*, const void**, size_t*, const void**,
                                   size_t*, zkhip_timings*);
    void (*record_from_sums)(zkhip_ctx*, const zkhip_pk*, const uint8_t*, const uint8_t*, uint8_t*);
    void (*assignment_upload)(zkhip_ctx*, zkhip_assignment*, const uint8_t*);
    void (*assignment_upload_packed)(zkhip_ctx*, zkhip_assignment*, const uint8_t*, size_t, u64, u64, u64);
    void (*assignment_upload_witness)(zkhip_ctx*, zkhip_assignment*, const WitnessZ&, uint8_t* head);
    u64 (*compute_witness)(zkhip_ctx*, const zkhip_xplan*, u32, const uint8_t*, std::vector<std::unique_ptr<zkhip_assignment>>*, uint8_t*, u64, uint8_t*, u64,
                           int32_t*, u64*, u64*);
    void (*r1cs_check)(zkhip_ctx*, const zkhip_r1cs*, const uint8_t*, const void*, u64 out[2]);
    void (*ntt)(zkhip_ctx*, u32, int, uint8_t*);
    void (*witness_map)(zkhip_ctx*, const zkhip_r1cs*, const uint8_t*, uint8_t*);
    int (*ntt_shardable)(zkhip_ctx*, u32 log_n, u32 G);
    void (*shard_ntt_begin)(zkhip_ctx*, u32 G, u32 k, u32 log_n, int dir, const uint8_t*);
    void (*shard_ntt_end)(zkhip_ctx*, u32 G, u32 k, u32 log_n, int dir, uint8_t*, zkhip_ctx* const* members);
    int (*witness_map_shardable)(zkhip_ctx*, const zkhip_r1cs*, u32 G);
    void (*shard_witness_map)(zkhip_ctx*, const zkhip_r1cs*, const uint8_t* z, uint8_t* h_out, u32 G, u32 k, int step, zkhip_ctx* const* members);
    int (*can_shard)(zkhip_ctx*, const zkhip_pk*, const zkhip_r1cs*, u32 G, u32 k);
    void (*shard_begin)(zkhip_ctx*, const zkhip_pk*, const zkhip_r1cs*, const uint8_t*, const uint8_t*, const uint8_t*, u32 G, u32 k);
    void (*shard_step)(zkhip_ctx*, const zkhip_pk*, const zkhip_r1cs*, u32 G, u32 k, int step, zkhip_ctx* const* members);
    void (*shard_end_partial)(zkhip_ctx*, const zkhip_pk*, const zkhip_r1cs*, uint8_t*, zkhip_timings*);
    void (*shard_end_device_sums)(zkhip_ctx*, const zkhip_pk*, const zkhip_r1cs*, const void**, size_t*, const void**, size_t*, zkhip_timings*);
    void (*msm_g1)(zkhip_ctx*, u64, const uint8_t*, const uint8_t*, uint8_t*);
    void (*msm_g2)(zkhip_ctx*, u64, const uint8_t*, const uint8_t*, uint8_t*);
    void (*field_op)(zkhip_ctx*, int field, int op, u64, const uint8_t*, const uint8_t*, uint8_t*);
    void (*group_op)(zkhip_ctx*, int group, int form, int op, u64, const u32*, const u32*, const u32*, const uint8_t*, u32*);
    void (*setup)(zkhip_ctx*, const zkhip_r1cs*, const uint8_t*, const uint8_t*, const uint8_t*, uint8_t*, u64);
    void (*pairing_products)(zkhip_ctx*, u64 count, u32 pairs_per_item, const uint8_t* g1, const uint8_t* g2, uint8_t* ok_out);
    void (*tower_op)(zkhip_ctx*, int op, u64 count, const u32*, const u32*, u32*);
    void (*vk_load)(zkhip_ctx*, int scheme, const uint8_t*, size_t, zkhip_vk*);
    void (*verify)(zkhip_ctx*, const zkhip_vk*, u64 count, const uint8_t* proofs, const uint8_t* inputs, uint8_t* ok_out);
    u32 tower_limbs;
    void (*gm17_prove)(zkhip_ctx*, const zkhip_pk*, const zkhip_r1cs*, const uint8_t*, const void*, const uint8_t*, uint8_t*, zkhip_timings*);
    void (*gm17_prove_batch)(zkhip_ctx*, const zkhip_pk*, const zkhip_r1cs*, u32, const uint8_t*, void* const*, const uint8_t*, uint8_t*,
                             zkhip_timings*);
    void (*gm17_setup)(zkhip_ctx*, const zkhip_r1cs*, const uint8_t*, const uint8_t*, const uint8_t*, uint8_t*, u64);
    u64 (*gm17_key_bytes)(u64, u64, u64);
    void (*gm17_prove_partial)(zkhip_ctx*, const zkhip_pk*, const zkhip_r1cs*, const uint8_t*, const void*, const uint8_t*, uint8_t*, zkhip_timings*);
    void (*gm17_combine)(const zkhip_pk*, u32, const uint8_t*, const uint8_t*, uint8_t*);
    void (*queue_check)(const zkhip_pk*, const zkhip_r1cs*);
    void (*queue_enqueue)(zkhip_ctx*, ProofSlot&, const zkhip_pk*, const zkhip_r1cs*, const uint8_t* z_host, const void* z_dev, const PackedZ*, const WitnessZ*,
                          const uint8_t* rnd, bool checked);
    void (*queue_finish)(zkhip_ctx*, ProofSlot&, const zkhip_pk*, uint8_t*, zkhip_timings*);
};
template <class C>
static void field_op_dispatch(zkhip_ctx* ctx, int field, int op, u64 count, const uint8_t* a, const uint8_t* b, uint8_t* out) {
    typedef typename C::Fr Fr;
    typedef typename C::Fq Fq;
    typedef typename C::Fq2 Fq2;
    typedef Prover<C> P;
    if (field == 0) P::template field_op_api<Fr>(ctx, count, 256, a, b, out, [&](dim3 g, dim3 t, Stream s, Fr* x, Fr* y) { ZK_LAUNCH((k_field_op<Fr>), g, t, 0, s, x, y, x, count, op); });
    else if (field == 1) P::template field_op_api<Fq>(ctx, count, 256, a, b, out, [&](dim3 g, dim3 t, Stream s, Fq* x, Fq* y) { ZK_LAUNCH((k_field_op<Fq>), g, t, 0, s, x, y, x, count, op); });
    else if (field == 2) P::template field_op_api<Fq2>(ctx, count, 64, a, b, out, [&](dim3 g, dim3 t, Stream s, Fq2* x, Fq2* y) { ZK_LAUNCH((k_field_op_fq2<typename Fq2::Params, false>), g, t, 0, s, x, y, x, count, op); });
    else if (field == 3) P::template field_op_api<Fq2>(ctx, count, 64, a, b, out, [&](dim3 g, dim3 t, Stream s, Fq2* x, Fq2* y) { ZK_LAUNCH((k_field_op_fq2<typename Fq2::Params, true>), g, t, 0, s, x, y, x, count, op); });
    else if (field == 4) P::template field_op_api<Fr>(ctx, count, 64, a, b, out, [&](dim3 g, dim3 t, Stream s, Fr* x, Fr* y) { ZK_LAUNCH((k_field_op_unsat<typename Fr::Params>), g, t, 0, s, x, y, x, count, op); });
    else P::template field_op_api<Fq>(ctx, count, 64, a, b, out, [&](dim3 g, dim3 t, Stream s, Fq* x, Fq* y) { ZK_LAUNCH((k_field_op_unsat<typename Fq::Params>), g, t, 0, s, x, y, x, count, op); });
}
template <class C>
static void group_op_dispatch(zkhip_ctx* ctx, int group, int form, int op, u64 count, const u32* a, const u32* b, const u32* k, const uint8_t* flags, u32* out) {
    if (group == 1) group_op_run<typename C::Fq>(ctx, form, op, count, a, b, k, flags, out);
// ... 75 lines not shown
```

### zokrates_amd/csrc/gm17.cuh

```cuda
#pragma once

namespace zk {

template <class P>
__global__ void k_sap_rows(const Fe<P>* __restrict__ ra, const Fe<P>* __restrict__ rb, const Fe<P>* __restrict__ rc, const Fe<P>* __restrict__ z,
                           Fe<P>* __restrict__ sa, Fe<P>* __restrict__ sc, Fe<P>* __restrict__ ext, u64 n, u64 l, u64 m) {
    ZK_PRIO_HIGH();
    typedef Fe<P> F;
    u64 i = (u64)blockIdx.x * blockDim.x + threadIdx.x;
    if (i >= n + l) return;
    if (i < n) {
        const F a = ra[i], b = rb[i];
        const F d = fe_sub(a, b);
        const F e = rp_sqr(d);
        sa[2 * i] = fe_add(a, b);
        sa[2 * i + 1] = d;
        if (sc) {
            sc[2 * i] = fe_add(fe_dbl(fe_dbl(rc[i])), e);
            sc[2 * i + 1] = e;
        }
        ext[m + i] = rp_to_plain(e);
    } else if (i == n) {
        sa[2 * n] = rp_one<P>();
        if (sc) sc[2 * n] = rp_one<P>();
    } else {
        const u64 j = i - n;
        const F x = z[j], one = rp_one<P>();
        const F d = fe_sub(x, one);
        const F f = rp_sqr(d);
        sa[2 * n + 2 * j - 1] = fe_add(x, one);
        sa[2 * n + 2 * j] = d;
        if (sc) {
            sc[2 * n + 2 * j - 1] = fe_add(fe_dbl(fe_dbl(x)), f);
            sc[2 * n + 2 * j] = f;
        }
        ext[m + n - 1 + j] = rp_to_plain(f);
    }
}
template <class P>
__global__ void k_sap_quotient(const Fe<P>* __restrict__ a, Fe<P> zinv, Fe<P>* __restrict__ out, u64 n) {
    ZK_PRIO_HIGH();
    u64 i = (u64)blockIdx.x * blockDim.x + threadIdx.x;
    if (i >= n) return;
    const Fu<P> aa = fu_sqr_inl(fu_unpack<P>(a[i].v));
    out[i] = rp_canon(fu_mul_inl(aa, fu_unpack<P>(zinv.v)));
}
template <class F>
__global__ void k_gm17_coeffs(const F* __restrict__ a, const F* __restrict__ c, F gamma, F ab, F two_g2z, F* __restrict__ aq, F* __restrict__ c1,
                              F* __restrict__ c2, F* __restrict__ vq, u64 n) {
    u64 i = (u64)blockIdx.x * blockDim.x + threadIdx.x;
    if (i >= n) return;
    const F v = fe_add(fe_mul(gamma, c[i]), fe_mul(ab, a[i]));
    aq[i] = fe_from_mont(fe_mul(gamma, a[i]));
    c1[i] = fe_from_mont(fe_mul(gamma, v));
    c2[i] = fe_from_mont(fe_mul(two_g2z, a[i]));
    vq[i] = fe_from_mont(v);
}

template <class C>
struct Gm17 {
    typedef typename C::Fr Fr;
    typedef typename C::Fq Fq;
    typedef typename C::Fq2 Fq2;
    typedef PkLoader<C> L;
    typedef Prover<C> P;
    static constexpr int FQB = Fq::BYTES;
    static constexpr int G1B = 2 * FQB, G2B = 4 * FQB;

    static Fr add_mod(const Fr& a, const Fr& b) {
        return fe_from_mont(fe_add(fe_to_mont(a), fe_to_mont(b)));
    }
    static void enqueue(zkhip_ctx* ctx, ProofSlot& sl, const zkhip_pk* pk, const zkhip_r1cs* cs, const uint8_t* z_host, const void* z_dev,
                        const uint8_t* d1, const uint8_t* r, int check_idx = -1, const PackedZ* zp = nullptr, const WitnessZ* wz = nullptr) {
        L::check_match(pk, cs, 1);
        const u64 m = cs->l + cs->w, n = cs->n, l = cs->l, M = pk->m, D = pk->N;
        Fr dd = fe_from_bytes_canon<Fr>(d1), rr = fe_from_bytes_canon<Fr>(r);
        require(canon_lt_mod(dd) && canon_lt_mod(rr), ZKHIP_ERR_BAD_ARG, "d1 or r not a canonical field element");
        const Fr rho = add_mod(dd, rr);
        const bool bound = P::is_bound(pk, cs);
        NttPlan<C>* pl = P::open_slot(ctx, sl, pk);
        sl.check_idx = check_idx;
        memcpy(sl.r, rho.v, 32);
        memset(sl.s, 0, 32);
        Stream st = ctx->stream;
        P::stage_z(ctx, sl, m, M + 2, z_host, z_dev, check_idx >= 0, false, zp, wz);
        uint8_t* d_scalars = (uint8_t*)sl.scalars.p;
        sl.zmont.ensure(m * 32);
        dev_h2d(d_scalars + M * 32, sl.r, 32, st);
        dev_memset(d_scalars + (M + 1) * 32, 0, 32, st);
        ZK_LAUNCH((k_mul_const<Fr>), dim3(blocks_for(m, 256)), dim3(256), 0, st, (const Fr*)d_scalars, ptr<Fr>(sl.zmont), m, pl->k_to_rp);
        event_record(sl.ev[0], st);

        sl.va.ensure(2 * D * sizeof(Fr));
        Fr *sa = ptr<Fr>(sl.va), *sc = sa + D;
        const u64 D0 = 2 * n + 2 * (l - 1) + 1;
        if (D0 < D) {
            dev_memset(sa + D0, 0, (D - D0) * sizeof(Fr), st);
            if (!bound) dev_memset(sc + D0, 0, (D - D0) * sizeof(Fr), st);
        }
        sl.vc.ensure(3 * std::max<u64>(n, 1) * sizeof(Fr));
        Fr *ra = ptr<Fr>(sl.vc), *rb = ra + n, *rc = rb + n;
        if (n) P::matvec(ctx, cs, ptr<Fr>(sl.zmont), ra, rb, rc, n, 0, n, (bound && check_idx < 0) ? 2 : 3);
        if (check_idx >= 0) P::enqueue_check(sl, ra, rb, rc, n, st);
        ZK_LAUNCH((k_sap_rows<typename Fr::Params>), dim3(blocks_for(n + l, 256)), dim3(256), 0, st, ra, rb, rc, ptr<Fr>(sl.zmont), sa, bound ? (Fr*)nullptr : sc,
                  (Fr*)d_scalars, n, l, m);
        event_record(sl.ev[1], st);

        const typename P::Lay ly(ctx, pk);
        ly.reserve(sl);
        P::start_z_lanes(ctx, sl, pk, ly);

        Stream wn = ctx->serial ? st : ctx_ntt_stream(ctx);
        stream_wait_event(wn, sl.ev[1]);
        ctx->ws = wn;
        event_record(sl.ntt_b, wn);
        Transforms<C>::ntt_quotient(ctx, pl, sa, 1, sc, bound, [&](const Fr& zinv) {
            ZK_LAUNCH((k_sap_quotient<typename Fr::Params>), dim3(blocks_for(D, 256)), dim3(256), 0, wn, sa, zinv, sa, D);
        });
        ctx->ws = ctx->stream;
        event_record(sl.ntt_e, wn);

        P::lanes_after_h(ctx, sl, pk, ly, bound, false, ptr<u32>(sl.va), wn);
    }

    static void finish(zkhip_ctx* ctx, ProofSlot& sl, const zkhip_pk* pk, uint8_t* out, zkhip_timings* tm) {
        require(pk->world == 1, ZKHIP_ERR_BAD_ARG, "this proving key is one shard of a multi-GPU key: use zkhip_prove_gm17_partial + zkhip_combine_gm17");
        const typename P::Sums g = P::collect(ctx, sl, pk);
        const auto t_fin = std::chrono::steady_clock::now();
        Fr rho;
        memcpy(rho.v, sl.r, 32);
        if (P::unsatisfied(ctx, sl, typename P::Lay(ctx, pk))) memset(out, 0, P::PROOF_BYTES);
        else assemble(pk, g, rho, out);
        P::fill_timings(sl, tm, t_fin);
    }
    static void assemble(const zkhip_pk* pk, const typename P::Sums& g, const Fr& rho, uint8_t* out) {
        const Fr rho2 = fe_from_mont(fe_sqr(fe_to_mont(rho)));
        uint8_t dec[2 * FQB];
        decode_point<FQB, 2>(pk->g_gamma2_z2_canon.data(), dec);
        Aff<Fq> z2;
        memcpy(&z2, dec, sizeof(z2));
        z2 = L::to_mont_point(z2);
        Xyzz<Fq> t1, t2;
        {
            HostThreads th;
            th.run([&] { t1 = xyzz_mul_limbs(g.b1, rho.v, Fr::N); });
            t2 = xyzz_mul_limbs(Xyzz<Fq>::from_affine(z2), rho2.v, Fr::N);
        }
        Xyzz<Fq> gC = xyzz_add(g.l, t1);
        gC = xyzz_add(gC, t2);
        gC = xyzz_add(gC, g.h);
        P::write_proof(g.a.is_inf(), xyzz_to_affine(g.a), g.b2.is_inf(), xyzz_to_affine(g.b2), gC.is_inf(), xyzz_to_affine(gC), out);
    }
    static void prove_partial(zkhip_ctx* ctx, const zkhip_pk* pk, const zkhip_r1cs* cs, const uint8_t* z_host, const void* z_dev, const uint8_t* rnd,
                              uint8_t* partial_out, zkhip_timings* tm) {
        check_d2(rnd);
        enqueue(ctx, ctx->slots[0], pk, cs, z_host, z_dev, rnd, rnd + 64);
        P::emit_partial(ctx, ctx->slots[0], pk, partial_out, tm);
    }
    static void prove_device_sums(zkhip_ctx* ctx, const zkhip_pk* pk, const zkhip_r1cs* cs, const uint8_t* z_host, const uint8_t* rnd,
                                  const void** d_ws1, size_t* b1, const void** d_ws2, size_t* b2, zkhip_timings* tm) {
        check_d2(rnd);
        enqueue(ctx, ctx->slots[0], pk, cs, z_host, nullptr, rnd, rnd + 64);
        P::hand_out_sums(ctx, ctx->slots[0], pk, d_ws1, b1, d_ws2, b2, tm);
    }
    static void combine(const zkhip_pk* pk, u32 count, const uint8_t* partials, const uint8_t* rnd, uint8_t* out) {
        check_d2(rnd);
        Fr dd = fe_from_bytes_canon<Fr>(rnd), rr = fe_from_bytes_canon<Fr>(rnd + 64);
        require(canon_lt_mod(dd) && canon_lt_mod(rr), ZKHIP_ERR_BAD_ARG, "d1 or r not a canonical field element");
        assemble(pk, P::sum_partials(count, partials), add_mod(dd, rr), out);
    }

    static void check_d2(const uint8_t* rnd) {
        require(canon_lt_mod(fe_from_bytes_canon<Fr>(rnd + 32)), ZKHIP_ERR_BAD_ARG, "d2 not a canonical field element");
    }
    static void prove(zkhip_ctx* ctx, const zkhip_pk* pk, const zkhip_r1cs* cs, const uint8_t* z_host, const void* z_dev, const uint8_t* rnd,
                      uint8_t* out, zkhip_timings* tm) {
        check_d2(rnd);
        ctx->unsat.clear();
        enqueue(ctx, ctx->slots[0], pk, cs, z_host, z_dev, rnd, rnd + 64, ctx->checked ? 0 : -1);
        finish(ctx, ctx->slots[0], pk, out, tm);
        P::raise_unsatisfied(ctx, 1, cs);
    }
    static void prove_batch(zkhip_ctx* ctx, const zkhip_pk* pk, const zkhip_r1cs* cs, u32 count, const uint8_t* z_host, void* const* z_dev,
                            const uint8_t* rnd, uint8_t* proofs_out, zkhip_timings* tm) {
        const u64 m = cs->l + cs->w;
        P::run_batch(ctx, cs, count, tm,
                     [&](u32 i, ProofSlot& sl) {
                         check_d2(rnd + (size_t)i * 96);
                         enqueue(ctx, sl, pk, cs, z_host ? z_host + (size_t)i * m * 32 : nullptr, z_host ? nullptr : z_dev[i], rnd + (size_t)i * 96,
                                 rnd + (size_t)i * 96 + 64, ctx->checked ? (int)i : -1);
                     },
                     [&](u32 j, ProofSlot& sl, zkhip_timings* one) { finish(ctx, sl, pk, proofs_out + (size_t)j * P::PROOF_BYTES, one); });
    }

    static u64 key_bytes(u64 n, u64 l, u64 w) {
        const SapShape sh = sap_shape(n, l, w);
        return (u64)3 * G2B + 2 * G1B + 8 + l * G1B + 8 + sh.M * G1B + 8 + sh.M * G2B + 8 + (sh.M - l) * G1B + 8 + sh.M * G1B + 3 * G1B + G2B + 8 +
               (sh.D + 1) * G1B;
    }
    static void setup(zkhip_ctx* ctx, const zkhip_r1cs* cs, const uint8_t* toxic, const uint8_t* g1b, const uint8_t* g2b, uint8_t* out, u64 cap) {
        typedef Setup<C> S;
        const u64 n = cs->n, l = cs->l, w = cs->w, m = l + w;
        const SapShape sh = sap_shape(n, l, w);
        const u64 M = sh.M, D = sh.D;
        const u64 need = key_bytes(n, l, w);
        require(cap >= need, ZKHIP_ERR_BAD_ARG, "output buffer too small (see zkhip_setup_gm17_size)");
        const Fr alpha = S::read_fr(toxic, false, ""), beta = S::read_fr(toxic + 32, false, "");
        const Fr gamma = S::read_fr(toxic + 64, true, "gamma must be non-zero");
        const Fr t = S::read_fr(toxic + 96, false, "");
        NttPlan<C>* pl = get_plan<C>(ctx, sh.logD);
        const Fr zt = fe_sub(fe_pow_u64(t, D), Fr::one());
        require(!zt.is_zero(), ZKHIP_ERR_BAD_ARG, "t lies in the evaluation domain");
        Stream s = ctx->stream;
        const unsigned T = 256;

        DBuf d_u;
        d_u.ensure(D * sizeof(Fr));
        ZK_LAUNCH((k_lagrange_at<Fr>), dim3(blocks_for(D, T)), dim3(T), 0, s, ptr<Fr>(d_u), t, pl->omega, fe_mul(zt, pl->n_inv), D);
        std::vector<Fr> u(D);
        dev_d2h(u.data(), d_u.p, D * sizeof(Fr), s);
        stream_sync(s);
        std::vector<Fr> av(M, Fr::zero()), cv(M, Fr::zero());
        HostCsr hm;
        hm.fetch(ctx, cs);
        auto val_at = [&](int k, u64 q) { return fe_from_bytes_canon<Fr>(hm.val[k].data() + q * 32); };
        HostThreads ta;
        ta.run([&] {
            for (u64 i = 0; i < n; ++i) {
                const Fr u_add = fe_add(u[2 * i], u[2 * i + 1]), u_sub = fe_sub(u[2 * i], u[2 * i + 1]);
                for (u64 q = hm.rp[0][i]; q < hm.rp[0][i + 1]; ++q) { Fr& x = av[hm.col[0][q]]; x = fe_add(x, fe_mul(u_add, val_at(0, q))); }
                for (u64 q = hm.rp[1][i]; q < hm.rp[1][i + 1]; ++q) { Fr& x = av[hm.col[1][q]]; x = fe_add(x, fe_mul(u_sub, val_at(1, q))); }
            }
            av[0] = fe_add(av[0], u[2 * n]);
            for (u64 i = 1; i < l; ++i) {
                const Fr u1 = u[2 * n + 2 * i - 1], u2 = u[2 * n + 2 * i];
                av[i] = fe_add(av[i], fe_add(u1, u2));
                av[0] = fe_add(av[0], fe_sub(u1, u2));
            }
        });
        for (u64 i = 0; i < n; ++i) {
            const Fr u4 = fe_dbl(fe_dbl(u[2 * i]));
            for (u64 q = hm.rp[2][i]; q < hm.rp[2][i + 1]; ++q) { Fr& x = cv[hm.col[2][q]]; x = fe_add(x, fe_mul(u4, val_at(2, q))); }
            cv[m + i] = fe_add(cv[m + i], fe_add(u[2 * i], u[2 * i + 1]));
        }
        cv[0] = fe_add(cv[0], u[2 * n]);
        for (u64 i = 1; i < l; ++i) {
            const Fr u1 = u[2 * n + 2 * i - 1], u2 = u[2 * n + 2 * i];
            cv[i] = fe_add(cv[i], fe_dbl(fe_dbl(u1)));
            cv[m + n - 1 + i] = fe_add(cv[m + n - 1 + i], fe_add(u1, u2));
        }
        ta.join();

        const Fr ab = fe_add(alpha, beta);
        const Fr gz = fe_mul(gamma, zt), g2z = fe_mul(gamma, gz);
        DBuf d_a, d_c, d_aq, d_c1, d_c2, d_vq, d_t;
        d_a.ensure(M * sizeof(Fr)); d_c.ensure(M * sizeof(Fr));
        d_aq.ensure(M * sizeof(Fr)); d_c1.ensure(M * sizeof(Fr)); d_c2.ensure(M * sizeof(Fr)); d_vq.ensure(M * sizeof(Fr));
        d_t.ensure((D + 1) * sizeof(Fr));
// ... 68 lines not shown
```

### zokrates_amd/csrc/kernels_ntt.cuh

```cuda
#pragma once
#include <vector>

#include "devrt.h"
#include "fieldu.cuh"
#include "ntt_geom.h"

namespace zk {

template <class F>
__global__ void k_to_mont(const F* __restrict__ in, F* __restrict__ out, u64 n) {
    ZK_PRIO_HIGH();
    u64 i = (u64)blockIdx.x * blockDim.x + threadIdx.x;
    if (i < n) out[i] = fe_to_mont(in[i]);
}
template <class F>
__global__ void k_from_mont(const F* __restrict__ in, F* __restrict__ out, u64 n) {
    u64 i = (u64)blockIdx.x * blockDim.x + threadIdx.x;
    if (i < n) out[i] = fe_from_mont(in[i]);
}
template <class P>
ZK_HD Fe<P> rp_canon(const Fu<P>& r) {
    Fe<P> o;
    fu_pack(r, o.v);
    fe_reduce_once(o);
    return o;
}
template <class P> ZK_HD Fe<P> rp_mul(const Fe<P>& a, const Fe<P>& b) { return rp_canon(fu_mul_inl(fu_unpack<P>(a.v), fu_unpack<P>(b.v))); }
template <class P> ZK_HD Fe<P> rp_sqr(const Fe<P>& a) { const Fu<P> u = fu_unpack<P>(a.v); return rp_canon(fu_sqr_inl(u)); }
template <class P> ZK_HD Fe<P> rp_one() { return rp_canon(Fu<P>::one()); }
template <class P>
ZK_HD Fe<P> rp_to_plain(const Fe<P>& a) {
    Fu<P> unit = Fu<P>::zero();
    unit.v[0] = 1;
    return rp_canon(fu_mul_inl(fu_unpack<P>(a.v), unit));
}
template <class F>
__global__ void k_mul_const(const F* __restrict__ in, F* __restrict__ out, u64 n, F k) {
    ZK_PRIO_HIGH();
    u64 i = (u64)blockIdx.x * blockDim.x + threadIdx.x;
    if (i < n) out[i] = fe_mul(in[i], k);
}
template <class F>
__global__ void k_from_rp(const F* __restrict__ in, F* __restrict__ out, u64 n) {
    ZK_PRIO_HIGH();
    u64 i = (u64)blockIdx.x * blockDim.x + threadIdx.x;
    if (i < n) out[i] = rp_to_plain(in[i]);
}
template <class P>
__global__ void k_unpack_table(const Fe<P>* __restrict__ in, Fu<P>* __restrict__ out, u64 n) {
    u64 i = (u64)blockIdx.x * blockDim.x + threadIdx.x;
    if (i < n) out[i] = fu_unpack<P>(in[i].v);
}
template <class F>
__global__ void k_check_canonical(const F* __restrict__ x, u64 n, u32* __restrict__ flag) {
    ZK_PRIO_HIGH();
    u64 i = (u64)blockIdx.x * blockDim.x + threadIdx.x;
    if (i >= n) return;
    const F v = x[i];
    bool lt = false, decided = false;
    ZK_UNROLL for (int k = F::N - 1; k >= 0; --k) {
        if (!decided && v.v[k] != F::Params::mod(k)) { lt = v.v[k] < F::Params::mod(k); decided = true; }
    }
    if (!lt) atomicOr(flag, 1u);
}
static __global__ void k_fingerprint(const u32* __restrict__ data, u64 nwords, u64 salt, unsigned long long* __restrict__ out) {
    u64 a = 0, b = 0;
    for (u64 i = (u64)blockIdx.x * blockDim.x + threadIdx.x; i < nwords; i += (u64)gridDim.x * blockDim.x) {
        u64 x = ((u64)data[i] << 32 | (u32)i) ^ (salt + (i >> 32) * 0xD6E8FEB86659FD93ull);
        x = (x ^ (x >> 30)) * 0xBF58476D1CE4E5B9ull;
        x = (x ^ (x >> 27)) * 0x94D049BB133111EBull;
        x ^= x >> 31;
        a += x;
        b += (x * 0x9E3779B97F4A7C15ull) ^ (x >> 17);
    }
    if (a | b) {
        atomicAdd(&out[0], (unsigned long long)a);
        atomicAdd(&out[1], (unsigned long long)b);
    }
}
template <class F>
__global__ void k_field_op(const F* __restrict__ a, const F* __restrict__ b, F* __restrict__ out, u64 n, int op) {
    u64 i = (u64)blockIdx.x * blockDim.x + threadIdx.x;
    if (i >= n) return;
    F x = a[i], y = b[i];
    out[i] = op == 0 ? fe_add(x, y) : op == 1 ? fe_sub(x, y) : fe_mul(x, y);
}
template <class P, bool UNSAT>
__global__ void k_field_op_fq2(const Fe2<P>* __restrict__ a, const Fe2<P>* __restrict__ b, Fe2<P>* __restrict__ out, u64 n, int op) {
    u64 i = (u64)blockIdx.x * blockDim.x + threadIdx.x;
    if (i >= n) return;
    const Fe2<P> x = a[i], y = b[i];
    if (!UNSAT) {
        out[i] = op == 0 ? fe_add(x, y) : op == 1 ? fe_sub(x, y) : op == 2 ? fe_mul(x, y) : op == 3 ? fe_sqr(x) : fe_inv(x);
        return;
    }
    const Fu2<P> ux = fu_from_fe(x), uy = fu_from_fe(y);
    Fu2<P> r;
    switch (op) {
    case 0: r = fe_add(ux, uy); break;
    case 1: r = fe_sub_k<2>(ux, uy); break;
    case 2: r = fu2_mul_inl<P, true>(ux, uy); break;
    case 3: r = fu2_sqr_inl<P, true>(ux); break;
    case 4: r = ec_inv(ux); break;
    case 5: r = fu2_mul_call(ux, uy); break;
    case 6: r = fu2_sqr_call(ux); break;
    case 7: r = fu2_mulsub_inl<P, true>(ux, uy, ux, ux); break;
    default: {
        const Fu2<P> X = fe_add(fe_dbl(ux), ux), Y = fe_dbl(fe_dbl(uy));
        r = op == 8 ? fu2_mul_inl<P, true>(X, Y) : op == 9 ? fu2_sqr_inl<P, true>(X) : fu2_mulsub_inl<P, true>(X, Y, X, fe_dbl(fe_dbl(ux)));
    } break;
    }
    out[i] = fu_to_fe(r);
}
template <class F>
__global__ void k_mul_table(const F* __restrict__ in, const F* __restrict__ tbl, F* __restrict__ out, u64 n) {
    u64 i = (u64)blockIdx.x * blockDim.x + threadIdx.x;
    if (i < n) out[i] = fe_mul(in[i], tbl[i]);
}
template <class F>
__global__ void k_pow_table(F* __restrict__ out, F base, F scale, u64 n, u32 n1, u32 n2, int mode, u32 n3 = 1) {
    u64 i = (u64)blockIdx.x * blockDim.x + threadIdx.x;
    if (i >= n) return;
    u64 e = i;
    if (mode == 1) e = (i / n2) * (i % n2);
    else if (mode == 2) e = sigma_nat(i, n1, n2, n3);
    out[i] = fe_mul(scale, fe_pow_u64(base, e));
}
template <class F>
__global__ void k_sigma_permute(const F* __restrict__ in, F* __restrict__ out, u64 n, u32 n1, u32 n2, int dir, u32 n3 = 1) {
    u64 p = (u64)blockIdx.x * blockDim.x + threadIdx.x;
    if (p >= n) return;
    u64 nat = sigma_nat(p, n1, n2, n3);
    if (dir == 0) out[p] = in[nat];
    else out[nat] = in[p];
}
template <class P>
__global__ void k_quotient(const Fe<P>* __restrict__ a, const Fe<P>* __restrict__ b, Fe<P> zinv, Fe<P>* __restrict__ out, u64 n) {
    ZK_PRIO_HIGH();
    u64 i = (u64)blockIdx.x * blockDim.x + threadIdx.x;
    if (i >= n) return;
    const Fu<P> ab = fu_mul_inl(fu_unpack<P>(a[i].v), fu_unpack<P>(b[i].v));
    out[i] = rp_canon(fu_mul_inl(ab, fu_unpack<P>(zinv.v)));
}

struct CsrDev {
    const u64* rowptr;
    const u32* col;
    const void* val;
};
static constexpr u32 MATVEC_LONG = 32;
template <class F>
__global__ void __launch_bounds__(256) k_matvec(CsrDev A, CsrDev B, CsrDev C, const F* __restrict__ z, F* __restrict__ oa, F* __restrict__ ob,
                                                F* __restrict__ oc, u64 n, u64 l, u64 N, int gA, int gB, int gC, u64 m_vars, int mat0 = 0) {
    ZK_PRIO_HIGH();
    __shared__ F sh[256];
    const int which = blockIdx.y + mat0;
    const int G = which == 0 ? gA : which == 1 ? gB : gC;
    const u32 rows_per_block = blockDim.x / (u32)G;
    if ((u64)blockIdx.x * rows_per_block >= N) return;
    const u64 i = (u64)blockIdx.x * rows_per_block + threadIdx.x / (u32)G;
    const u32 lane = threadIdx.x % (u32)G;
    const CsrDev M = which == 0 ? A : which == 1 ? B : C;
    F* out = which == 0 ? oa : which == 1 ? ob : oc;
    F acc = F::zero();
    bool mine = true;
    if (i < n) {
        const F* val = (const F*)M.val;
        const u64 b = M.rowptr[i], e = M.rowptr[i + 1];
        mine = e - b <= MATVEC_LONG;
        if (mine)
            for (u64 k = b + lane; k < e; k += (u32)G) {
                ZK_ASSERT_IDX(M.col[k] < m_vars);
                acc = fe_add(acc, fe_mul(val[k], z[M.col[k]]));
            }
    } else if (which == 0 && i < n + l && lane == 0) {
        acc = z[i - n];
    }
    if (G > 1) {
        sh[threadIdx.x] = acc;
        __syncthreads();
        for (u32 st = (u32)G >> 1; st > 0; st >>= 1) {
            if (lane < st) {
                acc = fe_add(acc, sh[threadIdx.x + st]);
                sh[threadIdx.x] = acc;
            }
            __syncthreads();
        }
    }
    if (i < N && lane == 0 && mine) out[i] = acc;
}
template <class F>
__global__ void __launch_bounds__(256) k_matvec_long(CsrDev A, CsrDev B, CsrDev C, const F* __restrict__ z, F* __restrict__ oa, F* __restrict__ ob,
                                                     F* __restrict__ oc, const u64* __restrict__ rows, u64 n_long, u64 m_vars) {
    ZK_PRIO_HIGH();
    __shared__ F sh[256];
    const u32 lane = threadIdx.x & 63u;
    const u64 slot = (u64)blockIdx.x * (blockDim.x >> 6) + (threadIdx.x >> 6);
    const bool live = slot < n_long;
    const u64 r = live ? rows[slot] : 0;
    const int which = (int)(r >> 32);
    const u64 i = r & 0xffffffffu;
    const CsrDev M = which == 0 ? A : which == 1 ? B : C;
    F acc = F::zero();
    if (live) {
        const F* val = (const F*)M.val;
        const u64 e = M.rowptr[i + 1];
        for (u64 k = M.rowptr[i] + lane; k < e; k += 64) {
            ZK_ASSERT_IDX(M.col[k] < m_vars);
            acc = fe_add(acc, fe_mul(val[k], z[M.col[k]]));
        }
    }
    sh[threadIdx.x] = acc;
    __syncthreads();
    for (u32 st = 32; st > 0; st >>= 1) {
        if (lane < st) {
            acc = fe_add(acc, sh[threadIdx.x + st]);
            sh[threadIdx.x] = acc;
        }
        __syncthreads();
    }
    if (live && lane == 0) (which == 0 ? oa : which == 1 ? ob : oc)[i] = acc;
}
static constexpr u32 MATVEC_HUGE = 512, MATVEC_HUGE_THREADS = 512;
template <class F>
__global__ void __launch_bounds__(MATVEC_HUGE_THREADS) k_matvec_huge(CsrDev A, CsrDev B, CsrDev C, const F* __restrict__ z, F* __restrict__ oa, F* __restrict__ ob,
                                                                     F* __restrict__ oc, const u64* __restrict__ rows, u64 m_vars) {
    ZK_PRIO_HIGH();
    __shared__ F sh[MATVEC_HUGE_THREADS];
    const u64 r = rows[blockIdx.x];
    const int which = (int)(r >> 32);
    const u64 i = r & 0xffffffffu;
    const CsrDev M = which == 0 ? A : which == 1 ? B : C;
    const F* val = (const F*)M.val;
    F acc = F::zero();
    const u64 e = M.rowptr[i + 1];
    for (u64 k = M.rowptr[i] + threadIdx.x; k < e; k += MATVEC_HUGE_THREADS) {
        ZK_ASSERT_IDX(M.col[k] < m_vars);
        acc = fe_add(acc, fe_mul(val[k], z[M.col[k]]));
    }
    sh[threadIdx.x] = acc;
    __syncthreads();
    for (u32 st = MATVEC_HUGE_THREADS >> 1; st > 0; st >>= 1) {
        if (threadIdx.x < st) {
            acc = fe_add(acc, sh[threadIdx.x + st]);
            sh[threadIdx.x] = acc;
        }
        __syncthreads();
    }
    if (threadIdx.x == 0) (which == 0 ? oa : which == 1 ? ob : oc)[i] = acc;
}
template <class P>
__global__ void __launch_bounds__(256) k_r1cs_check(const Fe<P>* __restrict__ a, const Fe<P>* __restrict__ b, const Fe<P>* __restrict__ c, u64 n,
                                                    unsigned long long* __restrict__ verdict) {
    ZK_PRIO_HIGH();
    const u64 i = (u64)blockIdx.x * blockDim.x + threadIdx.x;
    bool bad = false;
    if (i < n) bad = !rp_mul(a[i], b[i]).equals(c[i]);
    const unsigned long long failing = ZK_WAVE_BALLOT(bad);
    if (failing != 0 && (threadIdx.x & 63u) == 0) {
        atomicMin(&verdict[0], (unsigned long long)(i + (u64)__builtin_ctzll(failing)));
        atomicAdd(&verdict[1], (unsigned long long)__builtin_popcountll(failing));
    }
}
static constexpr int MATVEC_MAX_LANES = 16;
static_assert((u64)MATVEC_MAX_LANES * 4 > MATVEC_LONG, "the average row length never asks for more lanes than MATVEC_MAX_LANES");
static inline int matvec_group(u64 nnz, u64 n) {
    const u64 avg = n ? nnz / n : 0;
    int g = 1;
    while (g < MATVEC_MAX_LANES && (u64)g * 4 <= avg) g *= 2;
    return g;
}

static __device__ __forceinline__ int ntt_slot(int e) { return e + (e >> 5); }
template <class P>
__device__ __forceinline__ Fu<P> lds_get_u(const u32* lds, int PL, int slot) {
    Fu<P> r;
    ZK_UNROLL for (int l = 0; l < Fu<P>::N; ++l) r.v[l] = lds[l * PL + slot];
    return r;
}
template <class P>
__device__ __forceinline__ void lds_put_u(u32* lds, int PL, int slot, const Fu<P>& x) {
    ZK_UNROLL for (int l = 0; l < Fu<P>::N; ++l) lds[l * PL + slot] = x.v[l];
}

static inline u32 ntt_plan_len(int logn) {
    u32 len = 1;
    for (int L = 1 << logn; L > 4; L >>= 2) len += 3 * (u32)(L >> 2);
    return len;
}
static inline void ntt_plan_exponents(int logn, std::vector<u32>& src) {
    const u32 n = 1u << logn;
    src.clear();
    for (u32 L = n; L > 4; L >>= 2) {
        const u32 q = L >> 2, tws = n / L;
        for (u32 k = 1; k <= 3; ++k)
            for (u32 pos = 0; pos < q; ++pos) src.push_back(k * pos * tws);
    }
    src.push_back(n >> 2);
}
static constexpr u32 NTT_PLAN_STRIDE = 12;
template <class P>
__global__ void k_ntt_plan_gather(const Fu<P>* __restrict__ roots, int rstride, const u32* __restrict__ src, u32 plen, u32* __restrict__ plan) {
    static_assert(Fu<P>::N <= (int)NTT_PLAN_STRIDE, "a plan entry holds the limbs of one factor");
    const u32 i = blockIdx.x * blockDim.x + threadIdx.x;
    if (i >= plen) return;
    const Fu<P> w = roots[(size_t)src[i] * rstride];
    ZK_UNROLL for (int l = 0; l < (int)NTT_PLAN_STRIDE; ++l) plan[(size_t)i * NTT_PLAN_STRIDE + l] = l < Fu<P>::N ? w.v[l] : 0u;
}
template <class P>
__device__ __forceinline__ Fu<P> ntt_plan_get(const u32* __restrict__ plan, u32 plen, u32 i) {
    (void)plen;
    const uint4* e = (const uint4*)(plan + (size_t)i * NTT_PLAN_STRIDE);
    const uint4 a = e[0], b = e[1], c = e[2];
    const u32 w[12] = {a.x, a.y, a.z, a.w, b.x, b.y, b.z, b.w, c.x, c.y, c.z, c.w};
    Fu<P> r;
    ZK_UNROLL for (int l = 0; l < Fu<P>::N; ++l) r.v[l] = w[l];
    return r;
}

#ifndef ZK_NTT_LOOSE
#define ZK_NTT_LOOSE 1
#endif
template <class P>
__device__ __forceinline__ Fu<P> fu_mul_ntt(const Fu<P>& a, const Fu<P>& b) {
    return ZK_NTT_LOOSE ? fu_mul_loose(a, b) : fu_mul_inl(a, b);
}
template <class P>
__global__ void k_field_op_unsat(const Fe<P>* __restrict__ a, const Fe<P>* __restrict__ b, Fe<P>* __restrict__ out, u64 n, int op) {
    u64 i = (u64)blockIdx.x * blockDim.x + threadIdx.x;
    if (i >= n) return;
    typedef Fu<P> U;
    const U ux = fu_from_fe(a[i]), uy = fu_from_fe(b[i]);
    U r;
    bool below_2p = true;
    switch (op) {
    case 0: r = fe_add(ux, uy); below_2p = false; break;
    case 1: r = fe_sub_k<2>(ux, uy); below_2p = false; break;
    case 2: r = fu_mul_inl(ux, uy); break;
    case 3: r = fu_sqr_inl(ux); break;
    case 4: r = fe_sub_k<4>(ux, uy); below_2p = false; break;
    case 5: r = fu_mul_loose(ux, uy); break;
    case 6: r = fu_sqr_loose(ux); break;
    case 7: r = fe_relax(fe_dbl(fe_dbl(fe_dbl(ux)))); below_2p = false; break;
    case 8: case 9: case 10: {
        const U X = fe_add(fe_dbl(ux), ux), Y = fe_dbl(fe_dbl(uy));
        r = op == 8 ? fu_mul_loose(X, Y) : op == 9 ? fu_sqr_loose(X) : fe_sub_k<2>(fu_mul_loose(X, Y), fu_mul_loose(X, fe_dbl(fe_dbl(ux))));
        below_2p = op != 10;
    } break;
    case 11: r = fe_relax(fu_x3_numerator(ux, uy, uy)); below_2p = false; break;
    case 12: case 13: case 14: {
        const Fe<P> cx = rp_canon(ux), cy = rp_canon(uy);
        const U wx = fu_unpack<P>(cx.v), wy = fu_unpack<P>(cy.v);
        if (op == 12) r = fu_mul_ntt<P>(fe_sub_k_lazy<4>(ux, uy), wy);
        else if (op == 13) {
            const U y2 = fe_dbl(uy);
            r = fu_mul_ntt<P>(fe_sub_k_lazy<8>(fe_add(fe_dbl(ux), ux), fe_add(fe_add(fe_dbl(y2), y2), uy)), wx);
        } else r = fu_mul_ntt<P>(fe_add_lazy(ux, uy), wx);
    } break;
    default: r = fu_mul_inl(fe_neg_lazy(uy), ux); break;
    }
    if (below_2p) {
        const Fe<P> c = rp_canon(r);
        r = fu_unpack<P>(c.v);
    }
    out[i] = fu_to_fe(r);
}
template <class P>
__device__ __forceinline__ void lds_ntt_dif4(u32* lds, int PL, int SS, int logn, int nseq, const u32* __restrict__ plan, u32 plen, bool first_done = false) {
    typedef Fu<P> U;
    const int n = 1 << logn;
    const int T = blockDim.x;
    if (logn >= 2) {
        const int per_seq = n >> 2, nbf = nseq * per_seq;
        u32 off = first_done ? 3u * (u32)(n >> 2) : 0u;
        int logq = first_done ? logn - 4 : logn - 2;
        for (int L = first_done ? n >> 2 : n; L >= 4; L >>= 2, logq -= 2) {
            const int q = L >> 2;
            for (int b = threadIdx.x; b < nbf; b += T) {
                const int seq = b >> (logn - 2), bb = b & (per_seq - 1);
                const int grp = bb >> logq, pos = bb & (q - 1);
                const int base = seq * SS, i0 = grp * L + pos;
                const int s0 = base + ntt_slot(i0), s1 = base + ntt_slot(i0 + q), s2 = base + ntt_slot(i0 + 2 * q), s3 = base + ntt_slot(i0 + 3 * q);
                U t2, t3;
                {
                    const U bq = lds_get_u<P>(lds, PL, s1), d = lds_get_u<P>(lds, PL, s3);
                    t2 = fe_add(bq, d);
                    t3 = fu_mul_ntt<P>(fe_sub_k_lazy<4>(bq, d), ntt_plan_get<P>(plan, plen, plen - 1));
                }
                U t0, t1;
                {
                    const U a = lds_get_u<P>(lds, PL, s0), c = lds_get_u<P>(lds, PL, s2);
                    t0 = fe_add(a, c);
                    t1 = fe_sub_k<4>(a, c);
                }
                lds_put_u<P>(lds, PL, s0, fe_relax(fe_add(t0, t2)));
                if (L > 4) {
                    lds_put_u<P>(lds, PL, s1, fu_mul_ntt<P>(fe_sub_k_lazy<8>(t0, t2), ntt_plan_get<P>(plan, plen, off + q + pos)));
                    lds_put_u<P>(lds, PL, s2, fu_mul_ntt<P>(fe_add_lazy(t1, t3), ntt_plan_get<P>(plan, plen, off + pos)));
                    lds_put_u<P>(lds, PL, s3, fu_mul_ntt<P>(fe_sub_k_lazy<4>(t1, t3), ntt_plan_get<P>(plan, plen, off + 2 * q + pos)));
                } else {
                    lds_put_u<P>(lds, PL, s1, fe_sub_k<8>(t0, t2));
                    lds_put_u<P>(lds, PL, s2, fe_add(t1, t3));
                    lds_put_u<P>(lds, PL, s3, fe_sub_k<4>(t1, t3));
                }
            }
            off += 3 * (u32)q;
            __syncthreads();
        }
    }
    if (logn & 1) {
        const int per_seq = n >> 1, nb2 = nseq * per_seq;
        for (int b = threadIdx.x; b < nb2; b += T) {
            const int seq = b >> (logn - 1), k = b & (per_seq - 1);
            const int s0 = seq * SS + ntt_slot(2 * k), s1 = seq * SS + ntt_slot(2 * k + 1);
            const U u = lds_get_u<P>(lds, PL, s0), v = lds_get_u<P>(lds, PL, s1);
            lds_put_u<P>(lds, PL, s0, fe_add(u, v));
            lds_put_u<P>(lds, PL, s1, fe_sub_k<4>(u, v));
        }
        __syncthreads();
    }
}
template <class P>
__device__ __forceinline__ void ntt_first_round(u32* lds, int PL, int base, int logn, int pos, const Fu<P>& a, const Fu<P>& bq, const Fu<P>& c, const Fu<P>& d,
                                                const u32* __restrict__ plan, u32 plen) {
    typedef Fu<P> U;
    const int q = 1 << (logn - 2);
    const int s0 = base + ntt_slot(pos), s1 = base + ntt_slot(pos + q), s2 = base + ntt_slot(pos + 2 * q), s3 = base + ntt_slot(pos + 3 * q);
    const U t2 = fe_add(bq, d);
    const U t3 = fu_mul_ntt<P>(fe_sub_k_lazy<4>(bq, d), ntt_plan_get<P>(plan, plen, plen - 1));
    const U t0 = fe_add(a, c);
    const U t1 = fe_sub_k<4>(a, c);
    lds_put_u<P>(lds, PL, s0, fe_relax(fe_add(t0, t2)));
    lds_put_u<P>(lds, PL, s1, fu_mul_ntt<P>(fe_sub_k_lazy<8>(t0, t2), ntt_plan_get<P>(plan, plen, (u32)(q + pos))));
    lds_put_u<P>(lds, PL, s2, fu_mul_ntt<P>(fe_add_lazy(t1, t3), ntt_plan_get<P>(plan, plen, (u32)pos)));
    lds_put_u<P>(lds, PL, s3, fu_mul_ntt<P>(fe_sub_k_lazy<4>(t1, t3), ntt_plan_get<P>(plan, plen, (u32)(2 * q + pos))));
}
static __device__ __forceinline__ int bitrev_n(int x, int logn) { return logn ? (int)(__brev((unsigned)x) >> (32 - logn)) : 0; }

template <class P>
__device__ __forceinline__ Fu<P> ntt_load(const uint4* __restrict__ data, size_t g) {
    const uint4 lo = data[2 * g], hi = data[2 * g + 1];
    const u32 w[8] = {lo.x, lo.y, lo.z, lo.w, hi.x, hi.y, hi.z, hi.w};
    return fe_relax(fu_unpack<P>(w));
}
static constexpr int NTT_BATCH = 4;
template <class P>
__device__ __forceinline__ Fu<P> ntt_unpack_words(const uint4& lo, const uint4& hi) {
    const u32 w[8] = {lo.x, lo.y, lo.z, lo.w, hi.x, hi.y, hi.z, hi.w};
    return fe_relax(fu_unpack<P>(w));
}
template <class P>
__device__ __forceinline__ void ntt_store_with(uint4* __restrict__ data, size_t g, Fu<P> x, bool have_post, const uint4& plo, const uint4& phi, int canon,
                                               const uint4* __restrict__ minus, size_t pg) {
    if (have_post) {
        const u32 w[8] = {plo.x, plo.y, plo.z, plo.w, phi.x, phi.y, phi.z, phi.w};
        x = fu_mul_ntt<P>(x, fu_unpack<P>(w));
    } else {
        x = fe_relax(x);
    }
    Fe<P> o;
    fu_pack(x, o.v);
    if (canon) fe_reduce_once(o);
    if (minus) {
        const uint4 lo = minus[2 * pg], hi = minus[2 * pg + 1];
        Fe<P> m;
        m.v[0] = lo.x; m.v[1] = lo.y; m.v[2] = lo.z; m.v[3] = lo.w; m.v[4] = hi.x; m.v[5] = hi.y; m.v[6] = hi.z; m.v[7] = hi.w;
        o = fe_sub(o, m);
    }
    data[2 * g] = make_uint4(o.v[0], o.v[1], o.v[2], o.v[3]);
    data[2 * g + 1] = make_uint4(o.v[4], o.v[5], o.v[6], o.v[7]);
}
template <class P>
__device__ __forceinline__ void ntt_store(uint4* __restrict__ data, size_t g, Fu<P> x, const uint4* __restrict__ post, int canon,
                                          const uint4* __restrict__ minus, size_t pg) {
    if (post) {
        const uint4 lo = post[2 * pg], hi = post[2 * pg + 1];
        const u32 w[8] = {lo.x, lo.y, lo.z, lo.w, hi.x, hi.y, hi.z, hi.w};
        x = fu_mul_inl(x, fu_unpack<P>(w));
    } else {
        x = fe_relax(x);
    }
    Fe<P> o;
    fu_pack(x, o.v);
    if (canon) fe_reduce_once(o);
    if (minus) {
        const uint4 lo = minus[2 * pg], hi = minus[2 * pg + 1];
        Fe<P> m;
        m.v[0] = lo.x; m.v[1] = lo.y; m.v[2] = lo.z; m.v[3] = lo.w; m.v[4] = hi.x; m.v[5] = hi.y; m.v[6] = hi.z; m.v[7] = hi.w;
        o = fe_sub(o, m);
    }
    data[2 * g] = make_uint4(o.v[0], o.v[1], o.v[2], o.v[3]);
    data[2 * g + 1] = make_uint4(o.v[4], o.v[5], o.v[6], o.v[7]);
}

static __device__ __forceinline__ void ntt_tile_of(u32& tile, u32& vec) {
    tile = blockIdx.x;
    vec = blockIdx.y;
    if (gridDim.y == 2 && (gridDim.x & 7u) == 0) {
        const u32 L = blockIdx.x + gridDim.x * blockIdx.y;
        const u32 g = L >> 4, r = L & 15u;
        tile = g * 8 + (r & 7u);
        vec = r >> 3;
    }
}
#ifndef ZK_NTT_WGS_PER_CU
#define ZK_NTT_WGS_PER_CU 4
#endif
template <class P>
__global__ void __launch_bounds__(512, ZK_NTT_WGS_PER_CU) k_ntt_cols(Fe<P>* __restrict__ data_, u64 vec_stride, int log_n1, u32 n2, int C, const u32* __restrict__ plan,
                                                     u32 plen, const Fe<P>* __restrict__ post_, int canon, const Fe<P>* __restrict__ minus_ = nullptr,
                                                     u64 batch_stride = 0, u64 post_mask = ~(u64)0, int fuse_first = 1) {
    ZK_PRIO_HIGH();
    ZK_DYN_SMEM(smem);
    static_assert(P::N == 8, "Fr is 8 x 32-bit words");
    u32* lds = (u32*)smem;
    u32 tile, vec;
    ntt_tile_of(tile, vec);
    const size_t boff = (size_t)blockIdx.z * batch_stride;
    uint4* data = (uint4*)(data_ + (size_t)vec * vec_stride + boff);
    const uint4* post = (const uint4*)post_;
    const int n1 = 1 << log_n1;
    const int SS = n1 + (n1 >> 5) + 1, PL = C * SS;
    const u32 c0 = tile * C;
    const int total = C * n1;
    const int logC = 31 - __clz(C);
    const bool fused = fuse_first && total == NTT_BATCH * (int)blockDim.x && log_n1 >= 4;
    for (int e0 = threadIdx.x; e0 < total; e0 += NTT_BATCH * blockDim.x) {
        uint4 lo[NTT_BATCH] = {}, hi[NTT_BATCH] = {};
        ZK_UNROLL for (int q = 0; q < NTT_BATCH; ++q) {
            const int e = e0 + q * blockDim.x;
            if (e < total) {
                const size_t g = (size_t)(e >> logC) * n2 + c0 + (e & (C - 1));
                lo[q] = data[2 * g];
                hi[q] = data[2 * g + 1];
            }
        }
        if (fused) {
            ntt_first_round<P>(lds, PL, (e0 & (C - 1)) * SS, log_n1, e0 >> logC, ntt_unpack_words<P>(lo[0], hi[0]), ntt_unpack_words<P>(lo[1], hi[1]),
                               ntt_unpack_words<P>(lo[2], hi[2]), ntt_unpack_words<P>(lo[3], hi[3]), plan, plen);
        } else {
            ZK_UNROLL for (int q = 0; q < NTT_BATCH; ++q) {
                const int e = e0 + q * blockDim.x;
                if (e < total) lds_put_u<P>(lds, PL, (e & (C - 1)) * SS + ntt_slot(e >> logC), ntt_unpack_words<P>(lo[q], hi[q]));
            }
        }
    }
    __syncthreads();
    lds_ntt_dif4<P>(lds, PL, SS, log_n1, C, plan, plen, fused);
    for (int e0 = threadIdx.x; e0 < total; e0 += NTT_BATCH * blockDim.x) {
        uint4 plo[NTT_BATCH] = {}, phi[NTT_BATCH] = {};
        if (post) {
            ZK_UNROLL for (int q = 0; q < NTT_BATCH; ++q) {
                const int e = e0 + q * blockDim.x;
                if (e < total) {
                    const size_t pg = (boff + (size_t)(e >> logC) * n2 + c0 + (e & (C - 1))) & post_mask;
                    plo[q] = post[2 * pg];
                    phi[q] = post[2 * pg + 1];
                }
            }
        }
        ZK_UNROLL for (int q = 0; q < NTT_BATCH; ++q) {
            const int e = e0 + q * blockDim.x;
            if (e < total) {
                const int k = e >> logC, j = e & (C - 1);
                const size_t g = (size_t)k * n2 + c0 + j;
                ntt_store_with<P>(data, g, lds_get_u<P>(lds, PL, j * SS + ntt_slot(bitrev_n(k, log_n1))), post != nullptr, plo[q], phi[q], canon, (const uint4*)minus_,
                                  (boff + g) & post_mask);
            }
        }
    }
}

template <class P>
__global__ void __launch_bounds__(512, ZK_NTT_WGS_PER_CU) k_ntt_rows(Fe<P>* __restrict__ data_, u64 vec_stride, int log_n2, int R, const u32* __restrict__ plan, u32 plen,
                                                     const Fe<P>* __restrict__ post_, int canon, const Fe<P>* __restrict__ minus_ = nullptr,
                                                     u64 post_mask = ~(u64)0, int fuse_first = 1) {
    ZK_PRIO_HIGH();
    ZK_DYN_SMEM(smem);
    u32* lds = (u32*)smem;
    u32 tile, vec;
    ntt_tile_of(tile, vec);
    uint4* data = (uint4*)(data_ + (size_t)vec * vec_stride);
    const uint4* post = (const uint4*)post_;
    const int n2 = 1 << log_n2;
    const int SS = n2 + (n2 >> 5) + 1, PL = R * SS;
    const size_t base = (size_t)tile * R * n2;
    const int total = R * n2;
    const bool fused = fuse_first && total == NTT_BATCH * (int)blockDim.x && log_n2 >= 4;
    if (fused) {
        const int seq = (int)threadIdx.x >> (log_n2 - 2), pos = (int)threadIdx.x & ((n2 >> 2) - 1);
        uint4 lo[NTT_BATCH], hi[NTT_BATCH];
        ZK_UNROLL for (int q = 0; q < NTT_BATCH; ++q) {
            const size_t g = base + (size_t)seq * n2 + pos + (size_t)q * (n2 >> 2);
            lo[q] = data[2 * g];
            hi[q] = data[2 * g + 1];
        }
        ntt_first_round<P>(lds, PL, seq * SS, log_n2, pos, ntt_unpack_words<P>(lo[0], hi[0]), ntt_unpack_words<P>(lo[1], hi[1]), ntt_unpack_words<P>(lo[2], hi[2]),
                           ntt_unpack_words<P>(lo[3], hi[3]), plan, plen);
    } else {
        for (int e0 = threadIdx.x; e0 < total; e0 += NTT_BATCH * blockDim.x) {
            uint4 lo[NTT_BATCH] = {}, hi[NTT_BATCH] = {};
            ZK_UNROLL for (int q = 0; q < NTT_BATCH; ++q) {
                const int e = e0 + q * blockDim.x;
                if (e < total) {
                    lo[q] = data[2 * (base + e)];
                    hi[q] = data[2 * (base + e) + 1];
                }
            }
            ZK_UNROLL for (int q = 0; q < NTT_BATCH; ++q) {
                const int e = e0 + q * blockDim.x;
                if (e < total) lds_put_u<P>(lds, PL, (e >> log_n2) * SS + ntt_slot(e & (n2 - 1)), ntt_unpack_words<P>(lo[q], hi[q]));
            }
        }
    }
    __syncthreads();
    lds_ntt_dif4<P>(lds, PL, SS, log_n2, R, plan, plen, fused);
    for (int e0 = threadIdx.x; e0 < total; e0 += NTT_BATCH * blockDim.x) {
        uint4 plo[NTT_BATCH] = {}, phi[NTT_BATCH] = {};
        if (post) {
            ZK_UNROLL for (int q = 0; q < NTT_BATCH; ++q) {
                const int e = e0 + q * blockDim.x;
                if (e < total) {
                    const size_t pg = (base + e) & post_mask;
                    plo[q] = post[2 * pg];
                    phi[q] = post[2 * pg + 1];
                }
            }
        }
        ZK_UNROLL for (int q = 0; q < NTT_BATCH; ++q) {
            const int e = e0 + q * blockDim.x;
            if (e < total) {
                const int r = e >> log_n2, k = e & (n2 - 1);
                ntt_store_with<P>(data, base + e, lds_get_u<P>(lds, PL, r * SS + ntt_slot(bitrev_n(k, log_n2))), post != nullptr, plo[q], phi[q], canon,
                                  (const uint4*)minus_, (base + e) & post_mask);
            }
        }
    }
}

struct ShardMove {
    u64 vec_stride;
    u64 nb;
    u32 G, me, rows;
    int log_w;
    int by_row, own;
};
template <bool PACK>
static __device__ __forceinline__ void ntt_shard_move(uint4* __restrict__ vec, uint4* __restrict__ staging, const ShardMove& g) {
    const u32 v = blockIdx.y, peer = blockIdx.z;
    if (peer == g.me && !g.own) return;
    const u64 w = (u64)1 << g.log_w, block = (u64)g.rows << g.log_w;
    const u64 origin = g.by_row ? (u64)peer * g.rows * g.nb + (u64)g.me * w : (u64)g.me * g.rows * g.nb + (u64)peer * w;
    uint4* data = vec + 2 * ((u64)v * g.vec_stride + origin);
    uint4* slot = staging + 2 * (((u64)v * g.G + peer) * block);
    const u64 pieces = 2 * block;
    for (u64 q = (u64)blockIdx.x * blockDim.x + threadIdx.x; q < pieces; q += (u64)gridDim.x * blockDim.x) {
        const u64 row = q >> (g.log_w + 1), in_row = q & (2 * w - 1);
        if (PACK) slot[q] = data[2 * row * g.nb + in_row];
        else data[2 * row * g.nb + in_row] = slot[q];
    }
}
template <class P>
__global__ void __launch_bounds__(256) k_ntt_shard_pack(const Fe<P>* __restrict__ vec, Fe<P>* __restrict__ staging, ShardMove g) {
    ZK_PRIO_HIGH();
    ntt_shard_move<true>((uint4*)vec, (uint4*)staging, g);
}
template <class P>
__global__ void __launch_bounds__(256) k_ntt_shard_unpack(Fe<P>* __restrict__ vec, const Fe<P>* __restrict__ staging, ShardMove g) {
    ZK_PRIO_HIGH();
    ntt_shard_move<false>((uint4*)vec, (uint4*)staging, g);
}
template <class P>
__global__ void k_quotient_strip(const Fe<P>* __restrict__ a, const Fe<P>* __restrict__ b, Fe<P> zinv, Fe<P>* __restrict__ out, u32 rows, int log_w, u64 nb) {
    ZK_PRIO_HIGH();
    const u64 e = (u64)blockIdx.x * blockDim.x + threadIdx.x;
    if (e >= ((u64)rows << log_w)) return;
    const u64 i = (e >> log_w) * nb + (e & (((u64)1 << log_w) - 1));
    const Fu<P> ab = fu_mul_inl(fu_unpack<P>(a[i].v), fu_unpack<P>(b[i].v));
    out[i] = rp_canon(fu_mul_inl(ab, fu_unpack<P>(zinv.v)));
}
template <class F>
__global__ void k_shard_strip_pow(F* __restrict__ data, F base, u32 rows, int log_w, u64 nb, u64 i0) {
    const u64 e = (u64)blockIdx.x * blockDim.x + threadIdx.x;
    if (e >= ((u64)rows << log_w)) return;
    const u64 i = (e >> log_w) * nb + (e & (((u64)1 << log_w) - 1));
    data[i] = fe_mul(data[i], fe_pow_u64(base, i0 + i));
}
template <class F>
__global__ void k_shard_range_out(const F* __restrict__ in, F* __restrict__ out, u32 rows, u64 nb, u32 n1, u32 n2, u32 n3, u32 k1_0, int mode, F base, F scale) {
    const u64 p = (u64)blockIdx.x * blockDim.x + threadIdx.x;
    if (p >= rows * nb) return;
    const u64 k1 = p / nb, rem = p % nb;
    const u64 inner = rem / n3 + (u64)n2 * (rem % n3);
    F x = in[p];
    if (mode == 2) x = fe_mul(x, fe_mul(scale, fe_pow_u64(base, k1_0 + k1 + (u64)n1 * inner)));
    if (mode >= 1) x = rp_to_plain(x);
    out[inner * rows + k1] = x;
}

}
```

### zokrates_amd/csrc/ntt_geom.h

```cpp
#pragma once
#include <algorithm>
#include <cstddef>
#include <cstdint>

#include "ntt_shard.h"

namespace zk {

constexpr int ntt_seq_stride(int n) { return n + (n >> 5) + 1; }

struct NttGeom {
    int log1 = 0, log2 = 0, log3 = 0;
    uint64_t N = 1;
    uint32_t N1 = 1, N2 = 1, N3 = 1, M = 1;
    uint64_t Nb = 1;
    int C_cols = 1, R_rows = 1, threads_cols = 64, threads_rows = 64;
    size_t smem_cols = 0, smem_rows = 0;
    int C_mid = 1, threads_mid = 64;
    size_t smem_mid = 0;
    int last_log() const { return log3 > 0 ? log3 : log2; }
    bool launchable() const { return Nb % (uint64_t)C_cols == 0 && (N >> last_log()) % (uint64_t)R_rows == 0 && N3 % (uint32_t)C_mid == 0 && (log3 == 0 || N1 <= 65535); }
};

inline size_t ntt_tile_smem(uint32_t nseq, uint32_t n) { return (size_t)9 * nseq * ntt_seq_stride((int)n) * 4; }
inline int ntt_tile_threads(uint64_t butterflies) { return (int)std::min<uint64_t>(512, std::max<uint64_t>(64, (butterflies + 63) / 64 * 64)); }

inline NttGeom ntt_geom(int logN, int single_max, int max_sublog, uint32_t ccols) {
    NttGeom p;
    if (logN <= single_max && logN <= max_sublog) { p.log1 = 0; p.log2 = logN; p.log3 = 0; }
    else if (logN <= 2 * max_sublog) { p.log1 = logN / 2; p.log2 = logN - p.log1; p.log3 = 0; }
    else { p.log1 = logN / 3; p.log2 = (logN - p.log1) / 2; p.log3 = logN - p.log1 - p.log2; }
    p.N = (uint64_t)1 << logN;
    p.N1 = 1u << p.log1, p.N2 = 1u << p.log2, p.N3 = 1u << p.log3;
    p.Nb = (uint64_t)p.N2 * p.N3;
    p.M = std::max(p.N1, std::max(p.N2, p.N3));
    const uint32_t last = 1u << p.last_log();
    const uint64_t nrows = p.N / last;
    const uint32_t tile_rows = std::max<uint32_t>(last, (uint32_t)std::min<uint64_t>(p.N, 1024));
    p.R_rows = p.log1 == 0 ? 1 : (int)std::max<uint64_t>(1, std::min<uint64_t>(nrows, tile_rows / last));
    auto cols_per_wg = [&](uint64_t ncols, uint32_t n) { return (int)std::max<uint64_t>(1, std::min<uint64_t>(ncols, std::max<uint32_t>(ccols, 1024 / std::max<uint32_t>(n, 1)))); };
    p.C_cols = cols_per_wg(p.Nb, p.N1);
    p.smem_cols = ntt_tile_smem((uint32_t)p.C_cols, p.N1);
    p.smem_rows = ntt_tile_smem((uint32_t)p.R_rows, last);
    p.threads_cols = ntt_tile_threads((uint64_t)p.C_cols * p.N1 / 4);
    p.threads_rows = ntt_tile_threads((uint64_t)p.R_rows * last / 4);
    if (p.log3 > 0) {
        p.C_mid = cols_per_wg(p.N3, p.N2);
        p.smem_mid = ntt_tile_smem((uint32_t)p.C_mid, p.N2);
        p.threads_mid = ntt_tile_threads((uint64_t)p.C_mid * p.N2 / 4);
    }
    return p;
}
inline ShardGeom ntt_whole(const NttGeom& p) { return ntt_shard_geom(p.N1, p.Nb, 1); }

enum NttPass { NTT_COLS, NTT_MID, NTT_ROWS };
struct NttLaunch {
    uint32_t grid_x, grid_z;
    int threads;
    size_t smem;
    int nseq;
    uint64_t offset;
};
inline NttLaunch ntt_pass_shape(const NttGeom& p, NttPass pass, const ShardGeom& g, uint32_t k) {
    if (pass == NTT_MID) return {p.N3 / (uint32_t)p.C_mid, g.rows, p.threads_mid, p.smem_mid, p.C_mid, g.range_origin(k)};
    const bool cols = pass == NTT_COLS;
    const uint32_t n = cols ? p.N1 : 1u << p.last_log();
    const uint64_t have = cols ? g.W : g.range_len() / n;
    const uint32_t nseq = (uint32_t)std::min<uint64_t>((uint64_t)(cols ? p.C_cols : p.R_rows), have);
    return {(uint32_t)(have / nseq), 1, ntt_tile_threads((uint64_t)nseq * n / 4), ntt_tile_smem(nseq, n), (int)nseq, cols ? g.strip_origin(k) : g.range_origin(k)};
}

}
```

### zokrates_amd/csrc/ntt_host.cuh

```cuda
#pragma once

namespace zk {

template <class C>
struct NttPlan : NttPlanBase, NttGeom {
    typedef typename C::Fr Fr;
    typedef Fu<typename Fr::Params> FrU;
    int split() const { return log1 | (log3 << 8); }
    DBuf roots_fwd, roots_inv, tw_fwd, tw_inv, s_coset, s_cosetinv_canon;
    DBuf s_cexit;
    DBuf tw2_fwd, tw2_inv;
    DBuf plan1[2], plan2[2], plan3[2];
    u32 plen1 = 0, plen2 = 0, plen3 = 0;
    Fr omega, omega_inv, n_inv, g, g_inv, zinv;
    Fr zinv_rp;
    Fr k_to_rp, k_mont_to_rp;
};

template <class Fr>
static Fr host_root_of_unity(int two_adicity, u64 generator, int logN) {
    u32 e[Fr::N];
    u64 bw = 1;
    for (int i = 0; i < Fr::N; ++i) {
        u64 t = (u64)Fr::Params::mod(i) - bw;
        e[i] = (u32)t;
        bw = t >> 63;
    }
    for (int s = 0; s < two_adicity; ++s)
        for (int i = 0; i < Fr::N; ++i) e[i] = (e[i] >> 1) | (i + 1 < Fr::N ? e[i + 1] << 31 : 0);
    Fr root = fe_pow(fe_from_u64<typename Fr::Params>(generator), e, Fr::N);
    for (int i = logN; i < two_adicity; ++i) root = fe_sqr(root);
    return root;
}
template <class Fr>
static Fr rp_factor() {
    Fr rp = Fr::one();
    for (int i = 32 * Fr::N; i < Fu<typename Fr::Params>::B * Fu<typename Fr::Params>::N; ++i) rp = fe_add(rp, rp);
    return rp;
}

static constexpr int NTT_MAX_SUBLOG = 11;

template <class C>
static NttPlan<C>* get_plan(zkhip_ctx* ctx, int logN) {
    typedef typename C::Fr Fr;
    for (auto& p : ctx->plans)
        if (p->curve == C::ID && p->logN == logN) return (NttPlan<C>*)p.get();
    const int sub = ctx->ntt_max_sublog;
    require(logN >= 0 && logN <= 3 * sub && logN <= C::TWO_ADICITY, ZKHIP_ERR_BAD_ARG,
            "domain size unsupported (log2 N must not exceed the field's two-adicity: 28 for bn128, 32 for bls12_381, 47 for bls12_377)");
    auto* pl = new NttPlan<C>();
    ctx->plans.emplace_back(pl);
    pl->curve = C::ID;
    pl->logN = logN;
    static_cast<NttGeom&>(*pl) = ntt_geom(logN, ctx->ntt_single_max, sub, (u32)ctx->ntt_cols);
    require(pl->launchable(), ZKHIP_ERR_BAD_ARG, "internal: NTT tile does not divide the domain, or its batch exceeds the grid");
    pl->omega = host_root_of_unity<Fr>(C::TWO_ADICITY, C::GENERATOR, logN);
    pl->omega_inv = fe_inv(pl->omega);
    pl->n_inv = fe_inv(fe_from_u64<typename Fr::Params>(pl->N));
    pl->g = fe_from_u64<typename Fr::Params>(C::GENERATOR);
    pl->g_inv = fe_inv(pl->g);
    pl->zinv = fe_inv(fe_sub(fe_pow_u64(pl->g, pl->N), Fr::one()));
    Stream s = ctx->stream;
    const unsigned T = 256;
    const Fr rp = rp_factor<Fr>();
    pl->k_mont_to_rp = rp;
    pl->k_to_rp = fe_to_mont(rp);
    pl->zinv_rp = fe_mul(pl->zinv, rp);
    typedef typename NttPlan<C>::FrU FrU;
    auto to_rp = [&](DBuf& buf, u64 count) {
        ZK_LAUNCH((k_mul_const<Fr>), dim3(blocks_for(count, T)), dim3(T), 0, s, ptr<Fr>(buf), ptr<Fr>(buf), count, rp);
    };
    const Fr wM = fe_pow_u64(pl->omega, pl->N / pl->M);
    const u64 nroots = std::max<u64>(pl->M, 1);
    ctx->tmp.ensure(nroots * sizeof(Fr));
    for (int inv = 0; inv < 2; ++inv) {
        DBuf& dst = inv ? pl->roots_inv : pl->roots_fwd;
        dst.ensure(nroots * sizeof(FrU));
        ZK_LAUNCH((k_pow_table<Fr>), dim3(blocks_for(nroots, T)), dim3(T), 0, s, ptr<Fr>(ctx->tmp), inv ? fe_inv(wM) : wM, Fr::one(), nroots, 0u, 0u, 0, 1u);
        to_rp(ctx->tmp, nroots);
        ZK_LAUNCH((k_unpack_table<typename Fr::Params>), dim3(blocks_for(nroots, T)), dim3(T), 0, s, ptr<Fr>(ctx->tmp), ptr<FrU>(dst), nroots);
    }
    {
        std::vector<u32> src;
        DBuf d_src;
        for (int which = 0; which < 3; ++which) {
            if (which == 2 && pl->log3 == 0) break;
            const int lg = which == 0 ? pl->log1 : which == 1 ? pl->log2 : pl->log3;
            const u32 plen = ntt_plan_len(lg);
            (which == 0 ? pl->plen1 : which == 1 ? pl->plen2 : pl->plen3) = plen;
            ntt_plan_exponents(lg, src);
            d_src.ensure(src.size() * 4);
            dev_h2d(d_src.p, src.data(), src.size() * 4, s);
            for (int inv = 0; inv < 2; ++inv) {
                DBuf& dst = which == 0 ? pl->plan1[inv] : which == 1 ? pl->plan2[inv] : pl->plan3[inv];
                dst.ensure((size_t)plen * NTT_PLAN_STRIDE * 4);
                ZK_LAUNCH((k_ntt_plan_gather<typename Fr::Params>), dim3(blocks_for(plen, T)), dim3(T), 0, s, ptr<FrU>(inv ? pl->roots_inv : pl->roots_fwd),
                          (int)(pl->M >> lg), ptr<u32>(d_src), plen, ptr<u32>(dst));
            }
            stream_sync(s);
        }
    }
    if (pl->log1 > 0) {
        pl->tw_fwd.ensure(pl->N * sizeof(Fr));
        pl->tw_inv.ensure(pl->N * sizeof(Fr));
        ZK_LAUNCH((k_pow_table<Fr>), dim3(blocks_for(pl->N, T)), dim3(T), 0, s, ptr<Fr>(pl->tw_fwd), pl->omega, Fr::one(), pl->N, pl->N1, (u32)pl->Nb, 1, 1u);
        ZK_LAUNCH((k_pow_table<Fr>), dim3(blocks_for(pl->N, T)), dim3(T), 0, s, ptr<Fr>(pl->tw_inv), pl->omega_inv, Fr::one(), pl->N, pl->N1, (u32)pl->Nb, 1, 1u);
        to_rp(pl->tw_fwd, pl->N);
        to_rp(pl->tw_inv, pl->N);
    }
    if (pl->log3 > 0) {
        const Fr wb = fe_pow_u64(pl->omega, pl->N1), wb_inv = fe_pow_u64(pl->omega_inv, pl->N1);
        pl->tw2_fwd.ensure(pl->Nb * sizeof(Fr));
        pl->tw2_inv.ensure(pl->Nb * sizeof(Fr));
        ZK_LAUNCH((k_pow_table<Fr>), dim3(blocks_for(pl->Nb, T)), dim3(T), 0, s, ptr<Fr>(pl->tw2_fwd), wb, Fr::one(), pl->Nb, pl->N2, pl->N3, 1, 1u);
        ZK_LAUNCH((k_pow_table<Fr>), dim3(blocks_for(pl->Nb, T)), dim3(T), 0, s, ptr<Fr>(pl->tw2_inv), wb_inv, Fr::one(), pl->Nb, pl->N2, pl->N3, 1, 1u);
        to_rp(pl->tw2_fwd, pl->Nb);
        to_rp(pl->tw2_inv, pl->Nb);
    }
    pl->s_coset.ensure(pl->N * sizeof(Fr));
    pl->s_cosetinv_canon.ensure(pl->N * sizeof(Fr));
    ZK_LAUNCH((k_pow_table<Fr>), dim3(blocks_for(pl->N, T)), dim3(T), 0, s, ptr<Fr>(pl->s_coset), pl->g, pl->n_inv, pl->N, pl->N1, pl->N2, 2, pl->N3);
    to_rp(pl->s_coset, pl->N);
    ZK_LAUNCH((k_pow_table<Fr>), dim3(blocks_for(pl->N, T)), dim3(T), 0, s, ptr<Fr>(pl->s_cosetinv_canon), pl->g_inv, fe_from_mont(pl->n_inv), pl->N,
              pl->N1, pl->N2, 2, pl->N3);
    pl->s_cexit.ensure(pl->N * sizeof(Fr));
    ZK_LAUNCH((k_pow_table<Fr>), dim3(blocks_for(pl->N, T)), dim3(T), 0, s, ptr<Fr>(pl->s_cexit), Fr::one(), fe_from_mont(fe_mul(pl->n_inv, pl->zinv)), pl->N,
              0u, 0u, 0, 1u);
    lds_opt_in(ctx, (const void*)k_ntt_cols<typename Fr::Params>);
    lds_opt_in(ctx, (const void*)k_ntt_rows<typename Fr::Params>);
    stream_sync(s);
    return pl;
}

template <class C>
struct Transforms {
    typedef typename C::Fr Fr;
    static void ntt_cols(zkhip_ctx* ctx, NttPlan<C>* pl, const ShardGeom& g, u32 k, Fr* data, bool inverse, const Fr* post, int nvec,
                         u64 vec_stride, int canon = 0) {
        const NttLaunch L = ntt_pass_shape(*pl, NTT_COLS, g, k);
        ZK_LAUNCH((k_ntt_cols<typename Fr::Params>), dim3(L.grid_x, nvec), dim3(L.threads), L.smem, ctx->ws, data + L.offset, vec_stride, pl->log1, (u32)pl->Nb, L.nseq,
                  ptr<u32>(pl->plan1[inverse ? 1 : 0]), pl->plen1, post ? post + L.offset : post, canon, (const Fr*)nullptr, (u64)0, ~(u64)0, ctx->ntt_fuse_first);
    }
    static void ntt_mid(zkhip_ctx* ctx, NttPlan<C>* pl, const ShardGeom& g, u32 k, Fr* data, bool inverse, const Fr* post, u64 post_mask,
                        int nvec, u64 vec_stride) {
        const NttLaunch L = ntt_pass_shape(*pl, NTT_MID, g, k);
        ZK_LAUNCH((k_ntt_cols<typename Fr::Params>), dim3(L.grid_x, nvec, L.grid_z), dim3(L.threads), L.smem, ctx->ws, data + L.offset, vec_stride, pl->log2, pl->N3,
                  L.nseq, ptr<u32>(pl->plan2[inverse ? 1 : 0]), pl->plen2, (post && post_mask == ~(u64)0) ? post + L.offset : post, 0, (const Fr*)nullptr, pl->Nb,
                  post_mask, ctx->ntt_fuse_first);
    }
    static void ntt_rows(zkhip_ctx* ctx, NttPlan<C>* pl, const ShardGeom& g, u32 k, Fr* data, bool inverse, const Fr* post, int nvec,
                         u64 vec_stride, int canon = 0, const Fr* minus = nullptr, u64 post_mask = ~(u64)0) {
        const bool three = pl->log3 > 0;
        const NttLaunch L = ntt_pass_shape(*pl, NTT_ROWS, g, k);
        ZK_LAUNCH((k_ntt_rows<typename Fr::Params>), dim3(L.grid_x, nvec), dim3(L.threads), L.smem, ctx->ws, data + L.offset, vec_stride, pl->last_log(), L.nseq,
                  ptr<u32>((three ? pl->plan3 : pl->plan2)[inverse ? 1 : 0]), three ? pl->plen3 : pl->plen2, (post && post_mask == ~(u64)0) ? post + L.offset : post, canon,
                  minus ? minus + L.offset : minus, post_mask, ctx->ntt_fuse_first);
    }
    static void ntt_kind_a(zkhip_ctx* ctx, NttPlan<C>* pl, Fr* data, bool inverse, const Fr* final_post, int nvec = 1,
                           u64 vec_stride = 0, int canon = 0, const Fr* final_minus = nullptr) {
        const ShardGeom w = ntt_whole(*pl);
        if (pl->log1 > 0) ntt_cols(ctx, pl, w, 0, data, inverse, inverse ? ptr<Fr>(pl->tw_inv) : ptr<Fr>(pl->tw_fwd), nvec, vec_stride);
        if (pl->log3 > 0) ntt_mid(ctx, pl, w, 0, data, inverse, inverse ? ptr<Fr>(pl->tw2_inv) : ptr<Fr>(pl->tw2_fwd), pl->Nb - 1, nvec, vec_stride);
        ntt_rows(ctx, pl, w, 0, data, inverse, final_post, nvec, vec_stride, canon, final_minus);
    }
    static void ntt_kind_b(zkhip_ctx* ctx, NttPlan<C>* pl, Fr* data, bool inverse, const Fr* final_post, int nvec = 1,
                           u64 vec_stride = 0, int canon = 0) {
        const ShardGeom w = ntt_whole(*pl);
        if (pl->log3 > 0) {
            ntt_rows(ctx, pl, w, 0, data, inverse, inverse ? ptr<Fr>(pl->tw2_inv) : ptr<Fr>(pl->tw2_fwd), nvec, vec_stride, 0, nullptr, pl->Nb - 1);
            ntt_mid(ctx, pl, w, 0, data, inverse, inverse ? ptr<Fr>(pl->tw_inv) : ptr<Fr>(pl->tw_fwd), ~(u64)0, nvec, vec_stride);
            ntt_cols(ctx, pl, w, 0, data, inverse, final_post, nvec, vec_stride, canon);
        } else if (pl->log1 > 0) {
            ntt_rows(ctx, pl, w, 0, data, inverse, inverse ? ptr<Fr>(pl->tw_inv) : ptr<Fr>(pl->tw_fwd), nvec, vec_stride);
            ntt_cols(ctx, pl, w, 0, data, inverse, final_post, nvec, vec_stride, canon);
        } else {
            ntt_rows(ctx, pl, w, 0, data, inverse, final_post, nvec, vec_stride, canon);
        }
    }
    template <class Pointwise>
    static void ntt_quotient(zkhip_ctx* ctx, NttPlan<C>* pl, Fr* v, int nvec, Fr* c, bool bound, Pointwise pointwise) {
        const u64 stride = nvec > 1 ? pl->N : 0;
        ntt_kind_a(ctx, pl, v, true, ptr<Fr>(pl->s_coset), nvec, stride);
        if (!bound) ntt_kind_a(ctx, pl, c, true, ptr<Fr>(pl->s_cexit), 1, 0, 1);
        ntt_kind_b(ctx, pl, v, false, nullptr, nvec, stride);
        pointwise(bound ? fe_from_mont(pl->zinv) : pl->zinv_rp);
        if (!bound) ntt_kind_a(ctx, pl, v, true, ptr<Fr>(pl->s_cosetinv_canon), 1, 0, 1, c);
    }

    static bool shard_ok(const NttPlan<C>* pl, size_t G) { return ntt_shardable(pl->log1, pl->N1, pl->Nb, G); }
    static void shard_state(zkhip_ctx* ctx, const ShardGeom& g, u32 nvec) {
        const size_t bytes = (size_t)g.staging_len(nvec) * 32;
        ctx->shard.send[0].ensure(bytes);
        ctx->shard.send[1].ensure(bytes);
        ctx->shard.recv.ensure(bytes);
        for (Event& e : ctx->shard.packed)
            if (!e) e = event_create();
    }
    static ShardMove shard_move_args(const ShardGeom& g, u32 k, u64 vec_stride, bool by_row, bool own) {
        ShardMove a;
        a.vec_stride = vec_stride;
        a.nb = g.Nb;
        a.G = g.G;
        a.me = k;
        a.rows = g.rows;
        a.log_w = ilog2_floor(g.W);
        a.by_row = by_row ? 1 : 0;
        a.own = own ? 1 : 0;
        return a;
    }
    static unsigned shard_move_blocks(const ShardGeom& g) { return (unsigned)std::min<u64>(1024, std::max<u64>(1, (2 * g.block + 255) / 256)); }
    static void shard_pack(zkhip_ctx* ctx, const ShardGeom& g, u32 k, const Fr* data, u32 nvec, u64 vec_stride, bool by_row) {
        zkhip_ctx::Shard& sh = ctx->shard;
        const unsigned set = sh.turn & 1u;
        ZK_LAUNCH((k_ntt_shard_pack<typename Fr::Params>), dim3(shard_move_blocks(g), nvec, g.G), dim3(256), 0, ctx->ws, data, ptr<Fr>(sh.send[set]),
                  shard_move_args(g, k, vec_stride, by_row, false));
        event_record(sh.packed[set], ctx->ws);
    }
    static void shard_fetch(zkhip_ctx* ctx, const ShardGeom& g, u32 k, Fr* data, u32 nvec, u64 vec_stride, bool by_row, zkhip_ctx* const* members) {
        zkhip_ctx::Shard& sh = ctx->shard;
        const unsigned set = sh.turn & 1u;
        for (u32 j = 0; j < g.G; ++j) {
            if (j == k) continue;
            event_sync(members[j]->shard.packed[set]);
            for (u32 v = 0; v < nvec; ++v)
                dev_copy_between(ptr<Fr>(sh.recv) + g.slot_origin(v, j), ctx->device, ptr<Fr>(members[j]->shard.send[set]) + g.slot_origin(v, k), members[j]->device,
                                 (size_t)g.block * sizeof(Fr), ctx->ws);
        }
        ZK_LAUNCH((k_ntt_shard_unpack<typename Fr::Params>), dim3(shard_move_blocks(g), nvec, g.G), dim3(256), 0, ctx->ws, data, ptr<Fr>(sh.recv),
                  shard_move_args(g, k, vec_stride, by_row, false));
        ++sh.turn;
    }

    static void ntt_api(zkhip_ctx* ctx, u32 log_n, int dir, uint8_t* data) {
        NttPlan<C>* pl = get_plan<C>(ctx, (int)log_n);
        Stream s = ctx->stream;
        ctx->ws = s;
        const u64 N = pl->N;
        const unsigned T = 256, B = blocks_for(N, T);
        ctx->cur->va.ensure(N * sizeof(Fr));
        ctx->cur->vb.ensure(N * sizeof(Fr));
        ctx->cur->vc.ensure(N * sizeof(Fr));
        Fr *a = ptr<Fr>(ctx->cur->va), *b = ptr<Fr>(ctx->cur->vb), *t = ptr<Fr>(ctx->cur->vc);
        dev_h2d(a, data, N * 32, s);
        ZK_LAUNCH((k_mul_const<Fr>), dim3(B), dim3(T), 0, s, a, a, N, pl->k_to_rp);
        const bool inverse = dir == 1 || dir == 3;
        if (dir == 2) {
            ZK_LAUNCH((k_pow_table<Fr>), dim3(B), dim3(T), 0, s, t, pl->g, Fr::one(), N, 0u, 0u, 0);
            ZK_LAUNCH((k_mul_table<Fr>), dim3(B), dim3(T), 0, s, a, t, a, N);
        }
        ntt_kind_a(ctx, pl, a, inverse, nullptr, 1, 0, 1);
        ZK_LAUNCH((k_sigma_permute<Fr>), dim3(B), dim3(T), 0, s, a, b, N, pl->N1, pl->N2, 1, pl->N3);
        if (inverse) {
            ZK_LAUNCH((k_pow_table<Fr>), dim3(B), dim3(T), 0, s, t, dir == 3 ? pl->g_inv : Fr::one(), pl->n_inv, N, 0u, 0u, 0);
            ZK_LAUNCH((k_mul_table<Fr>), dim3(B), dim3(T), 0, s, b, t, b, N);
        }
        ZK_LAUNCH((k_from_rp<Fr>), dim3(B), dim3(T), 0, s, b, b, N);
        dev_d2h(data, b, N * 32, s);
        stream_sync(s);
        if (log_n > 24) {
            ctx->cur->va.release(); ctx->cur->vb.release(); ctx->cur->vc.release();
            for (size_t k = 0; k < ctx->plans.size(); ++k)
                if (ctx->plans[k].get() == pl) { ctx->plans.erase(ctx->plans.begin() + (long)k); break; }
        }
    }

    static int ntt_shardable_api(zkhip_ctx* ctx, u32 log_n, u32 G) { const NttPlan<C>* pl = get_plan<C>(ctx, (int)log_n); return shard_ok(pl, G) ? pl->split() : -1; }
    static void shard_ntt_begin(zkhip_ctx* ctx, u32 G, u32 k, u32 log_n, int dir, const uint8_t* data) {
        NttPlan<C>* pl = get_plan<C>(ctx, (int)log_n);
        require(shard_ok(pl, G), ZKHIP_ERR_BAD_ARG, "internal: this transform does not shard");
        const ShardGeom g = ntt_shard_geom(pl->N1, pl->Nb, G);
        Stream s = ctx->stream;
        ctx->ws = s;
        ctx->cur->va.ensure(pl->N * sizeof(Fr));
        shard_state(ctx, g, 1);
        zkhip_ctx::Shard& sh = ctx->shard;
        Fr* a = ptr<Fr>(ctx->cur->va);
        const u64 n = g.range_len();
        sh.host.resize(n * 32);
        for (u32 r = 0; r < pl->N1; ++r) memcpy(sh.host.data() + (size_t)r * g.W * 32, data + ((size_t)r * pl->Nb + g.strip_origin(k)) * 32, (size_t)g.W * 32);
        dev_h2d(sh.recv.p, sh.host.data(), n * 32, s);
        ZK_LAUNCH((k_mul_const<Fr>), dim3(blocks_for(n, 256)), dim3(256), 0, s, ptr<Fr>(sh.recv), ptr<Fr>(sh.recv), n, pl->k_to_rp);
        ZK_LAUNCH((k_ntt_shard_unpack<typename Fr::Params>), dim3(shard_move_blocks(g), 1, G), dim3(256), 0, s, a, ptr<Fr>(sh.recv), shard_move_args(g, k, 0, true, true));
        if (dir == 2)
            ZK_LAUNCH((k_shard_strip_pow<Fr>), dim3(blocks_for(n, 256)), dim3(256), 0, s, a + g.strip_origin(k), pl->g, pl->N1, ilog2_floor(g.W), pl->Nb, g.strip_origin(k));
        const bool inverse = dir == 1 || dir == 3;
        ntt_cols(ctx, pl, g, k, a, inverse, inverse ? ptr<Fr>(pl->tw_inv) : ptr<Fr>(pl->tw_fwd), 1, 0);
        shard_pack(ctx, g, k, a, 1, 0, true);
    }
    static void range_out(zkhip_ctx* ctx, NttPlan<C>* pl, const ShardGeom& g, u32 k, const Fr* vec, int mode, const Fr& base,
                          const Fr& scale, uint8_t* out) {
        zkhip_ctx::Shard& sh = ctx->shard;
        Stream s = ctx->ws;
        const u64 n = g.range_len();
        sh.out.ensure(n * sizeof(Fr));
        ZK_LAUNCH((k_shard_range_out<Fr>), dim3(blocks_for(n, 256)), dim3(256), 0, s, vec + g.range_origin(k), ptr<Fr>(sh.out), g.rows, pl->Nb, pl->N1, pl->N2, pl->N3,
                  k * g.rows, mode, base, scale);
        sh.host.resize(n * 32);
        dev_d2h(sh.host.data(), sh.out.p, n * 32, s);
        stream_sync(s);
        for (u64 inner = 0; inner < pl->Nb; ++inner)
            memcpy(out + (inner * pl->N1 + (u64)k * g.rows) * 32, sh.host.data() + inner * g.rows * 32, (size_t)g.rows * 32);
    }
    static void shard_ntt_end(zkhip_ctx* ctx, u32 G, u32 k, u32 log_n, int dir, uint8_t* data, zkhip_ctx* const* members) {
        NttPlan<C>* pl = get_plan<C>(ctx, (int)log_n);
        const ShardGeom g = ntt_shard_geom(pl->N1, pl->Nb, G);
        Stream s = ctx->stream;
        ctx->ws = s;
        Fr* a = ptr<Fr>(ctx->cur->va);
        const bool inverse = dir == 1 || dir == 3;
        shard_fetch(ctx, g, k, a, 1, 0, false, members);
        if (pl->log3 > 0) ntt_mid(ctx, pl, g, k, a, inverse, inverse ? ptr<Fr>(pl->tw2_inv) : ptr<Fr>(pl->tw2_fwd), pl->Nb - 1, 1, 0);
        ntt_rows(ctx, pl, g, k, a, inverse, nullptr, 1, 0, 1);
        range_out(ctx, pl, g, k, a, inverse ? 2 : 1, dir == 3 ? pl->g_inv : Fr::one(), pl->n_inv, data);
    }
};

}
```

Baseline: 110.8.

## Fuse scalar Montgomery scaling into matvec and fuse NTT passes with quotient

Removes the separate k_mul_const pass that built a zmont copy of the witness. The rp conversion factor is now applied once per output row inside the matvec kernels, and once per element in the SAP kernel. Adds a fused rows-pair kernel that runs the inverse and forward row NTTs with the coset multiply in one launch. Adds a cols-quotient kernel that does the final forward column NTT of both vectors together with the pointwise quotient, applied when the plan has two dimensions only. The aim is fewer kernel launches and fewer full-vector global memory round trips, at the cost of more complex kernels and extra LDS and register pressure.

```diff
diff --git a/zokrates_amd/csrc/core.cuh b/zokrates_amd/csrc/core.cuh
--- a/zokrates_amd/csrc/core.cuh
+++ b/zokrates_amd/csrc/core.cuh
@@ -114,7 +114,7 @@
 static constexpr int ZK_NLANES = 5;
 static constexpr int ZK_NSLOTS = 4;
 struct ProofSlot {
-    DBuf scalars, zmont, va, vb, vc, ws1, ws2, zflag;
+    DBuf scalars, va, vb, vc, ws1, ws2, zflag;
     DBuf verdict;
     int check_idx = -1;
     MsmSort sorts[3];
@@ -1191,17 +1191,18 @@
 
     static CsrDev csr(const zkhip_r1cs* cs, int k) { return CsrDev{ptr<u64>(cs->rp[k]), ptr<u32>(cs->col[k]), cs->val[k].p}; }
 
-    static void matvec(zkhip_ctx* ctx, const zkhip_r1cs* cs, const Fr* zmont, Fr* a, Fr* b, Fr* c, u64 n, u64 l, u64 N, int nmat = 3, int mat0 = 0) {
+    static void matvec(zkhip_ctx* ctx, const zkhip_r1cs* cs, const Fr* z, Fr* a, Fr* b, Fr* c, u64 n, u64 l, u64 N, int nmat = 3, int mat0 = 0) {
+        const Fr k_rp = fe_to_mont(rp_factor<Fr>());
         int g[3];
         matvec_lanes(cs, g, nmat, mat0);
-        ZK_LAUNCH((k_matvec<Fr>), dim3(blocks_for(N, 256 / gmax_rows(g)), nmat), dim3(256), 0, ctx->ws, csr(cs, 0), csr(cs, 1), csr(cs, 2), zmont, a, b, c, n,
-                  l, N, g[0], g[1], g[2], cs->l + cs->w, mat0);
+        ZK_LAUNCH((k_matvec<Fr>), dim3(blocks_for(N, 256 / gmax_rows(g)), nmat), dim3(256), 0, ctx->ws, csr(cs, 0), csr(cs, 1), csr(cs, 2), z, a, b, c, n,
+                  l, N, g[0], g[1], g[2], cs->l + cs->w, k_rp, mat0);
         if (cs->n_huge)
-            ZK_LAUNCH((k_matvec_huge<Fr>), dim3((unsigned)cs->n_huge), dim3(MATVEC_HUGE_THREADS), 0, ctx->ws, csr(cs, 0), csr(cs, 1), csr(cs, 2), zmont, a, b, c,
-                      ptr<u64>(cs->long_rows), cs->l + cs->w);
+            ZK_LAUNCH((k_matvec_huge<Fr>), dim3((unsigned)cs->n_huge), dim3(MATVEC_HUGE_THREADS), 0, ctx->ws, csr(cs, 0), csr(cs, 1), csr(cs, 2), z, a, b, c,
+                      ptr<u64>(cs->long_rows), cs->l + cs->w, k_rp);
         if (cs->n_long > cs->n_huge)
-            ZK_LAUNCH((k_matvec_long<Fr>), dim3(blocks_for(cs->n_long - cs->n_huge, 4)), dim3(256), 0, ctx->ws, csr(cs, 0), csr(cs, 1), csr(cs, 2), zmont, a, b, c,
-                      ptr<u64>(cs->long_rows) + cs->n_huge, cs->n_long - cs->n_huge, cs->l + cs->w);
+            ZK_LAUNCH((k_matvec_long<Fr>), dim3(blocks_for(cs->n_long - cs->n_huge, 4)), dim3(256), 0, ctx->ws, csr(cs, 0), csr(cs, 1), csr(cs, 2), z, a, b, c,
+                      ptr<u64>(cs->long_rows) + cs->n_huge, cs->n_long - cs->n_huge, cs->l + cs->w, k_rp);
     }
     static unsigned gmax_rows(const int g[3]) { return (unsigned)std::max(g[0], std::max(g[1], g[2])); }
 
@@ -1212,19 +1213,16 @@
         Fr *a = ptr<Fr>(ctx->cur->va), *b = a + N, *c = b + N;
         if (half >= 0) {
             Fr* v = a + (u64)half * N;
-            matvec(ctx, cs, ptr<Fr>(ctx->cur->zmont), a, b, c, cs->n, cs->l, N, 1, half);
+            matvec(ctx, cs, ptr<Fr>(ctx->cur->scalars), a, b, c, cs->n, cs->l, N, 1, half);
             event_record(ctx->cur->ntt_b, s);
-            Tr::ntt_kind_a(ctx, pl, v, true, ptr<Fr>(pl->s_coset), 1, 0);
-            Tr::ntt_kind_b(ctx, pl, v, false, nullptr, 1, 0);
+            Tr::to_coset(ctx, pl, v, 1);
             event_record(ctx->cur->ntt_e, s);
             return;
         }
-        matvec(ctx, cs, ptr<Fr>(ctx->cur->zmont), a, b, c, cs->n, cs->l, N, (bound && !check) ? 2 : 3);
+        matvec(ctx, cs, ptr<Fr>(ctx->cur->scalars), a, b, c, cs->n, cs->l, N, (bound && !check) ? 2 : 3);
         if (check) enqueue_check(*ctx->cur, a, b, c, cs->n, s);
         event_record(ctx->cur->ntt_b, s);
-        Tr::ntt_quotient(ctx, pl, a, 2, c, bound, [&](const Fr& zinv) {
-            ZK_LAUNCH((k_quotient<typename Fr::Params>), dim3(blocks_for(N, 256)), dim3(256), 0, s, a, b, zinv, a, N);
-        });
+        Tr::ntt_quotient(ctx, pl, a, 2, c, bound, nullptr);
         event_record(ctx->cur->ntt_e, s);
     }
 
@@ -1258,11 +1256,9 @@
         ctx->ws = s;
         const u64 m = cs->l + cs->w, n = cs->n;
         const Fr* z = stage_z(ctx, sl, m, m + 2, z_host, z_dev, true, true);
-        sl.zmont.ensure(m * 32);
-        ZK_LAUNCH((k_mul_const<Fr>), dim3(blocks_for(m, 256)), dim3(256), 0, s, z, ptr<Fr>(sl.zmont), m, fe_to_mont(rp_factor<Fr>()));
         sl.vc.ensure(3 * std::max<u64>(n, 1) * sizeof(Fr));
         Fr *ra = ptr<Fr>(sl.vc), *rb = ra + n, *rc = rb + n;
-        if (n) matvec(ctx, cs, ptr<Fr>(sl.zmont), ra, rb, rc, n, 0, n);
+        if (n) matvec(ctx, cs, z, ra, rb, rc, n, 0, n);
         enqueue_check(sl, ra, rb, rc, n, s);
         u32 flag = 0;
         dev_d2h(&flag, sl.zflag.p, 4, s);
@@ -1362,12 +1358,10 @@
     static void require_canonical(u32 flag) {
         require(flag == 0, ZKHIP_ERR_BAD_ARG, "an assignment entry is not a canonical field element (>= r)");
     }
-    static void stage_scalars(zkhip_ctx* ctx, NttPlan<C>* pl, void* d_scalars, u64 m, const uint8_t* r, const uint8_t* s_) {
+    static void stage_scalars(zkhip_ctx* ctx, void* d_scalars, u64 m, const uint8_t* r, const uint8_t* s_) {
         Stream s = ctx->stream;
-        ctx->cur->zmont.ensure(m * 32);
         dev_h2d((uint8_t*)d_scalars + m * 32, r, 32, s);
         dev_h2d((uint8_t*)d_scalars + (m + 1) * 32, s_, 32, s);
-        ZK_LAUNCH((k_mul_const<Fr>), dim3(blocks_for(m, 256)), dim3(256), 0, s, (const Fr*)d_scalars, ptr<Fr>(ctx->cur->zmont), m, pl->k_to_rp);
     }
 
     static void enqueue(zkhip_ctx* ctx, ProofSlot& sl, const zkhip_pk* pk, const zkhip_r1cs* cs, const uint8_t* z_host, const void* z_dev,
@@ -1407,7 +1401,7 @@
         memcpy(sl.s, s_, 32);
         Stream st = ctx->stream;
         stage_z(ctx, sl, pk->m, pk->m + 2, z_host, z_dev, sl.check_idx >= 0, false, zp, wz);
-        stage_scalars(ctx, pl, sl.scalars.p, pk->m, r, s_);
+        stage_scalars(ctx, sl.scalars.p, pk->m, r, s_);
         event_record(sl.ev[0], st);
 
         const Lay ly(ctx, pk);
@@ -1752,7 +1746,7 @@
         memcpy(sl.s, s_, 32);
         Stream st = ctx->stream;
         stage_z(ctx, sl, pk->m, pk->m + 2, z_host, nullptr, false);
-        stage_scalars(ctx, pl, sl.scalars.p, pk->m, r, s_);
+        stage_scalars(ctx, sl.scalars.p, pk->m, r, s_);
         event_record(sl.ev[0], st);
         const Lay ly(ctx, pk);
         ly.reserve(sl);
@@ -2077,7 +2071,7 @@
         const u64 m = cs->l + cs->w;
         uint8_t zero[32] = {0};
         upload_z(ctx, ctx->cur->scalars, m, m + 2, z, ctx->cur->zflag);
-        stage_scalars(ctx, pl, ctx->cur->scalars.p, m, zero, zero);
+        stage_scalars(ctx, ctx->cur->scalars.p, m, zero, zero);
         witness_map(ctx, cs, pl);
         ctx->cur->vb.ensure(pl->N * sizeof(Fr));
         ZK_LAUNCH((k_sigma_permute<Fr>), dim3(blocks_for(pl->N, 256)), dim3(256), 0, ctx->stream, ptr<Fr>(ctx->cur->va), ptr<Fr>(ctx->cur->vb), pl->N,
@@ -2097,7 +2091,7 @@
             ctx->cur->va.ensure(3 * N * sizeof(Fr));
             a = ptr<Fr>(ctx->cur->va); b = a + N; c = b + N;
             Tr::shard_state(ctx, g, 3);
-            matvec(ctx, cs, ptr<Fr>(ctx->cur->zmont), a, b, c, cs->n, cs->l, N, 3);
+            matvec(ctx, cs, ptr<Fr>(ctx->cur->scalars), a, b, c, cs->n, cs->l, N, 3);
             if (check) enqueue_check(*ctx->cur, a, b, c, cs->n, s);
             event_record(ctx->cur->ntt_b, s);
             Tr::ntt_cols(ctx, pl, g, k, a, true, ptr<Fr>(pl->tw_inv), 3, N);
@@ -2137,7 +2131,7 @@
             const u64 m = cs->l + cs->w;
             uint8_t zero[32] = {0};
             upload_z(ctx, ctx->cur->scalars, m, m + 2, z, ctx->cur->zflag);
-            stage_scalars(ctx, pl, ctx->cur->scalars.p, m, zero, zero);
+            stage_scalars(ctx, ctx->cur->scalars.p, m, zero, zero);
         }
         shard_witness_map(ctx, cs, pl, G, k, step, members);
         if (step == 3) Tr::range_out(ctx, pl, ntt_shard_geom(pl->N1, pl->Nb, G), k, ptr<Fr>(ctx->cur->va), 0, Fr::one(), Fr::one(), h_out);
diff --git a/zokrates_amd/csrc/gm17.cuh b/zokrates_amd/csrc/gm17.cuh
--- a/zokrates_amd/csrc/gm17.cuh
+++ b/zokrates_amd/csrc/gm17.cuh
@@ -4,7 +4,7 @@
 
 template <class P>
 __global__ void k_sap_rows(const Fe<P>* __restrict__ ra, const Fe<P>* __restrict__ rb, const Fe<P>* __restrict__ rc, const Fe<P>* __restrict__ z,
-                           Fe<P>* __restrict__ sa, Fe<P>* __restrict__ sc, Fe<P>* __restrict__ ext, u64 n, u64 l, u64 m) {
+                           Fe<P>* __restrict__ sa, Fe<P>* __restrict__ sc, Fe<P>* __restrict__ ext, u64 n, u64 l, u64 m, Fe<P> k_rp) {
     ZK_PRIO_HIGH();
     typedef Fe<P> F;
     u64 i = (u64)blockIdx.x * blockDim.x + threadIdx.x;
@@ -25,7 +25,7 @@
         if (sc) sc[2 * n] = rp_one<P>();
     } else {
         const u64 j = i - n;
-        const F x = z[j], one = rp_one<P>();
+        const F x = fe_mul(z[j], k_rp), one = rp_one<P>();
         const F d = fe_sub(x, one);
         const F f = rp_sqr(d);
         sa[2 * n + 2 * j - 1] = fe_add(x, one);
@@ -85,10 +85,8 @@
         Stream st = ctx->stream;
         P::stage_z(ctx, sl, m, M + 2, z_host, z_dev, check_idx >= 0, false, zp, wz);
         uint8_t* d_scalars = (uint8_t*)sl.scalars.p;
-        sl.zmont.ensure(m * 32);
         dev_h2d(d_scalars + M * 32, sl.r, 32, st);
         dev_memset(d_scalars + (M + 1) * 32, 0, 32, st);
-        ZK_LAUNCH((k_mul_const<Fr>), dim3(blocks_for(m, 256)), dim3(256), 0, st, (const Fr*)d_scalars, ptr<Fr>(sl.zmont), m, pl->k_to_rp);
         event_record(sl.ev[0], st);
 
         sl.va.ensure(2 * D * sizeof(Fr));
@@ -100,10 +98,10 @@
         }
         sl.vc.ensure(3 * std::max<u64>(n, 1) * sizeof(Fr));
         Fr *ra = ptr<Fr>(sl.vc), *rb = ra + n, *rc = rb + n;
-        if (n) P::matvec(ctx, cs, ptr<Fr>(sl.zmont), ra, rb, rc, n, 0, n, (bound && check_idx < 0) ? 2 : 3);
+        if (n) P::matvec(ctx, cs, (const Fr*)d_scalars, ra, rb, rc, n, 0, n, (bound && check_idx < 0) ? 2 : 3);
         if (check_idx >= 0) P::enqueue_check(sl, ra, rb, rc, n, st);
-        ZK_LAUNCH((k_sap_rows<typename Fr::Params>), dim3(blocks_for(n + l, 256)), dim3(256), 0, st, ra, rb, rc, ptr<Fr>(sl.zmont), sa, bound ? (Fr*)nullptr : sc,
-                  (Fr*)d_scalars, n, l, m);
+        ZK_LAUNCH((k_sap_rows<typename Fr::Params>), dim3(blocks_for(n + l, 256)), dim3(256), 0, st, ra, rb, rc, (const Fr*)d_scalars, sa, bound ? (Fr*)nullptr : sc,
+                  (Fr*)d_scalars, n, l, m, pl->k_to_rp);
         event_record(sl.ev[1], st);
 
         const typename P::Lay ly(ctx, pk);
diff --git a/zokrates_amd/csrc/kernels_ntt.cuh b/zokrates_amd/csrc/kernels_ntt.cuh
--- a/zokrates_amd/csrc/kernels_ntt.cuh
+++ b/zokrates_amd/csrc/kernels_ntt.cuh
@@ -151,7 +151,7 @@
 static constexpr u32 MATVEC_LONG = 32;
 template <class F>
 __global__ void __launch_bounds__(256) k_matvec(CsrDev A, CsrDev B, CsrDev C, const F* __restrict__ z, F* __restrict__ oa, F* __restrict__ ob,
-                                                F* __restrict__ oc, u64 n, u64 l, u64 N, int gA, int gB, int gC, u64 m_vars, int mat0 = 0) {
+                                                F* __restrict__ oc, u64 n, u64 l, u64 N, int gA, int gB, int gC, u64 m_vars, F k_rp, int mat0 = 0) {
     ZK_PRIO_HIGH();
     __shared__ F sh[256];
     const int which = blockIdx.y + mat0;
@@ -187,11 +187,11 @@
             __syncthreads();
         }
     }
-    if (i < N && lane == 0 && mine) out[i] = acc;
+    if (i < N && lane == 0 && mine) out[i] = fe_mul(acc, k_rp);
 }
 template <class F>
 __global__ void __launch_bounds__(256) k_matvec_long(CsrDev A, CsrDev B, CsrDev C, const F* __restrict__ z, F* __restrict__ oa, F* __restrict__ ob,
-                                                     F* __restrict__ oc, const u64* __restrict__ rows, u64 n_long, u64 m_vars) {
+                                                     F* __restrict__ oc, const u64* __restrict__ rows, u64 n_long, u64 m_vars, F k_rp) {
     ZK_PRIO_HIGH();
     __shared__ F sh[256];
     const u32 lane = threadIdx.x & 63u;
@@ -219,12 +219,12 @@
         }
         __syncthreads();
     }
-    if (live && lane == 0) (which == 0 ? oa : which == 1 ? ob : oc)[i] = acc;
+    if (live && lane == 0) (which == 0 ? oa : which == 1 ? ob : oc)[i] = fe_mul(acc, k_rp);
 }
 static constexpr u32 MATVEC_HUGE = 512, MATVEC_HUGE_THREADS = 512;
 template <class F>
 __global__ void __launch_bounds__(MATVEC_HUGE_THREADS) k_matvec_huge(CsrDev A, CsrDev B, CsrDev C, const F* __restrict__ z, F* __restrict__ oa, F* __restrict__ ob,
-                                                                     F* __restrict__ oc, const u64* __restrict__ rows, u64 m_vars) {
+                                                                     F* __restrict__ oc, const u64* __restrict__ rows, u64 m_vars, F k_rp) {
     ZK_PRIO_HIGH();
     __shared__ F sh[MATVEC_HUGE_THREADS];
     const u64 r = rows[blockIdx.x];
@@ -247,7 +247,7 @@
         }
         __syncthreads();
     }
-    if (threadIdx.x == 0) (which == 0 ? oa : which == 1 ? ob : oc)[i] = acc;
+    if (threadIdx.x == 0) (which == 0 ? oa : which == 1 ? ob : oc)[i] = fe_mul(acc, k_rp);
 }
 template <class P>
 __global__ void __launch_bounds__(256) k_r1cs_check(const Fe<P>* __restrict__ a, const Fe<P>* __restrict__ b, const Fe<P>* __restrict__ c, u64 n,
@@ -444,6 +444,7 @@
     return fe_relax(fu_unpack<P>(w));
 }
 static constexpr int NTT_BATCH = 4;
+static_assert(NTT_BATCH == NTT_TILE_BATCH, "ntt_geom.h sizes the tiles of k_ntt_rows_pair by the batch of the passes");
 template <class P>
 __device__ __forceinline__ Fu<P> ntt_unpack_words(const uint4& lo, const uint4& hi) {
     const u32 w[8] = {lo.x, lo.y, lo.z, lo.w, hi.x, hi.y, hi.z, hi.w};
@@ -572,6 +573,72 @@
 }
 
 template <class P>
+__device__ __forceinline__ void ntt_cols_stage(u32* lds, const uint4* __restrict__ data, int log_n1, u32 n2, int C, u32 c0, const u32* __restrict__ plan, u32 plen,
+                                               int fuse_first) {
+    const int n1 = 1 << log_n1;
+    const int SS = n1 + (n1 >> 5) + 1, PL = C * SS;
+    const int total = C * n1;
+    const int logC = 31 - __clz(C);
+    const bool fused = fuse_first && total == NTT_BATCH * (int)blockDim.x && log_n1 >= 4;
+    for (int e0 = threadIdx.x; e0 < total; e0 += NTT_BATCH * blockDim.x) {
+        uint4 lo[NTT_BATCH] = {}, hi[NTT_BATCH] = {};
+        ZK_UNROLL for (int q = 0; q < NTT_BATCH; ++q) {
+            const int e = e0 + q * blockDim.x;
+            if (e < total) {
+                const size_t g = (size_t)(e >> logC) * n2 + c0 + (e & (C - 1));
+                lo[q] = data[2 * g];
+                hi[q] = data[2 * g + 1];
+            }
+        }
+        if (fused) {
+            ntt_first_round<P>(lds, PL, (e0 & (C - 1)) * SS, log_n1, e0 >> logC, ntt_unpack_words<P>(lo[0], hi[0]), ntt_unpack_words<P>(lo[1], hi[1]),
+                               ntt_unpack_words<P>(lo[2], hi[2]), ntt_unpack_words<P>(lo[3], hi[3]), plan, plen);
+        } else {
+            ZK_UNROLL for (int q = 0; q < NTT_BATCH; ++q) {
+                const int e = e0 + q * blockDim.x;
+                if (e < total) lds_put_u<P>(lds, PL, (e & (C - 1)) * SS + ntt_slot(e >> logC), ntt_unpack_words<P>(lo[q], hi[q]));
+            }
+        }
+    }
+    __syncthreads();
+    lds_ntt_dif4<P>(lds, PL, SS, log_n1, C, plan, plen, fused);
+}
+template <class P>
+__global__ void __launch_bounds__(512, ZK_NTT_WGS_PER_CU) k_ntt_cols_quotient(Fe<P>* __restrict__ a_, const Fe<P>* __restrict__ b_, int log_n1, u32 n2, int C,
+                                                              const u32* __restrict__ plan, u32 plen, Fe<P> factor, int fuse_first = 1) {
+    ZK_PRIO_HIGH();
+    ZK_DYN_SMEM(smem);
+    u32* lds = (u32*)smem;
+    uint4* a = (uint4*)a_;
+    const uint4* b = (const uint4*)b_;
+    const int n1 = 1 << log_n1;
+    const int SS = n1 + (n1 >> 5) + 1, PL = C * SS;
+    const u32 c0 = blockIdx.x * C;
+    const int total = C * n1;
+    const int logC = 31 - __clz(C);
+    const uint4 none = make_uint4(0, 0, 0, 0);
+    ntt_cols_stage<P>(lds, a, log_n1, n2, C, c0, plan, plen, fuse_first);
+    for (int e = threadIdx.x; e < total; e += blockDim.x) {
+        const int k = e >> logC, j = e & (C - 1);
+        ntt_store_with<P>(a, (size_t)k * n2 + c0 + j, lds_get_u<P>(lds, PL, j * SS + ntt_slot(bitrev_n(k, log_n1))), false, none, none, 0, nullptr, 0);
+    }
+    __syncthreads();
+    ntt_cols_stage<P>(lds, b, log_n1, n2, C, c0, plan, plen, fuse_first);
+    const Fu<P> f = fu_unpack<P>(factor.v);
+    for (int e = threadIdx.x; e < total; e += blockDim.x) {
+        const int k = e >> logC, j = e & (C - 1);
+        const size_t g = (size_t)k * n2 + c0 + j;
+        const uint4 lo = a[2 * g], hi = a[2 * g + 1];
+        const u32 aw[8] = {lo.x, lo.y, lo.z, lo.w, hi.x, hi.y, hi.z, hi.w};
+        Fe<P> bw;
+        fu_pack(fe_relax(lds_get_u<P>(lds, PL, j * SS + ntt_slot(bitrev_n(k, log_n1)))), bw.v);
+        const Fe<P> o = rp_canon(fu_mul_inl(fu_mul_inl(fu_unpack<P>(aw), fu_unpack<P>(bw.v)), f));
+        a[2 * g] = make_uint4(o.v[0], o.v[1], o.v[2], o.v[3]);
+        a[2 * g + 1] = make_uint4(o.v[4], o.v[5], o.v[6], o.v[7]);
+    }
+}
+
+template <class P>
 __global__ void __launch_bounds__(512, ZK_NTT_WGS_PER_CU) k_ntt_rows(Fe<P>* __restrict__ data_, u64 vec_stride, int log_n2, int R, const u32* __restrict__ plan, u32 plen,
                                                      const Fe<P>* __restrict__ post_, int canon, const Fe<P>* __restrict__ minus_ = nullptr,
                                                      u64 post_mask = ~(u64)0, int fuse_first = 1) {
@@ -633,6 +700,103 @@
                 const int r = e >> log_n2, k = e & (n2 - 1);
                 ntt_store_with<P>(data, base + e, lds_get_u<P>(lds, PL, r * SS + ntt_slot(bitrev_n(k, log_n2))), post != nullptr, plo[q], phi[q], canon,
                                   (const uint4*)minus_, (base + e) & post_mask);
+            }
+        }
+    }
+}
+
+template <class P>
+__device__ __forceinline__ Fe<P> ntt_between_passes(const Fu<P>& x, const uint4& flo, const uint4& fhi) {
+    const u32 f[8] = {flo.x, flo.y, flo.z, flo.w, fhi.x, fhi.y, fhi.z, fhi.w};
+    Fe<P> o;
+    fu_pack(fu_mul_ntt<P>(x, fu_unpack<P>(f)), o.v);
+    return o;
+}
+template <class P>
+__global__ void __launch_bounds__(512, ZK_NTT_WGS_PER_CU) k_ntt_rows_pair(Fe<P>* __restrict__ data_, u64 vec_stride, int log_n2, int R, const u32* __restrict__ plan_a,
+                                                          const u32* __restrict__ plan_b, u32 plen, const Fe<P>* __restrict__ mid_, const Fe<P>* __restrict__ post_,
+                                                          int fuse_first = 1) {
+    ZK_PRIO_HIGH();
+    ZK_DYN_SMEM(smem);
+    u32* lds = (u32*)smem;
+    u32 tile, vec;
+    ntt_tile_of(tile, vec);
+    uint4* data = (uint4*)(data_ + (size_t)vec * vec_stride);
+    const uint4* mid = (const uint4*)mid_;
+    const uint4* post = (const uint4*)post_;
+    const int n2 = 1 << log_n2;
+    const int SS = n2 + (n2 >> 5) + 1, PL = R * SS;
+    const size_t base = (size_t)tile * R * n2;
+    const int total = R * n2;
+    const bool fused = fuse_first && total == NTT_BATCH * (int)blockDim.x && log_n2 >= 4;
+    const int fseq = (int)threadIdx.x >> (fused ? log_n2 - 2 : 0), fpos = (int)threadIdx.x & ((n2 >> 2) - 1);
+    if (fused) {
+        uint4 lo[NTT_BATCH], hi[NTT_BATCH];
+        ZK_UNROLL for (int q = 0; q < NTT_BATCH; ++q) {
+            const size_t g = base + (size_t)fseq * n2 + fpos + (size_t)q * (n2 >> 2);
+            lo[q] = data[2 * g];
+            hi[q] = data[2 * g + 1];
+        }
+        ntt_first_round<P>(lds, PL, fseq * SS, log_n2, fpos, ntt_unpack_words<P>(lo[0], hi[0]), ntt_unpack_words<P>(lo[1], hi[1]), ntt_unpack_words<P>(lo[2], hi[2]),
+                           ntt_unpack_words<P>(lo[3], hi[3]), plan_a, plen);
+    } else {
+        uint4 lo[NTT_BATCH] = {}, hi[NTT_BATCH] = {};
+        ZK_UNROLL for (int q = 0; q < NTT_BATCH; ++q) {
+            const int e = (int)threadIdx.x + q * (int)blockDim.x;
+            if (e < total) {
+                lo[q] = data[2 * (base + e)];
+                hi[q] = data[2 * (base + e) + 1];
+            }
+        }
+        ZK_UNROLL for (int q = 0; q < NTT_BATCH; ++q) {
+            const int e = (int)threadIdx.x + q * (int)blockDim.x;
+            if (e < total) lds_put_u<P>(lds, PL, (e >> log_n2) * SS + ntt_slot(e & (n2 - 1)), ntt_unpack_words<P>(lo[q], hi[q]));
+        }
+    }
+    __syncthreads();
+    lds_ntt_dif4<P>(lds, PL, SS, log_n2, R, plan_a, plen, fused);
+    {
+        uint4 mlo[NTT_BATCH] = {}, mhi[NTT_BATCH] = {};
+        ZK_UNROLL for (int q = 0; q < NTT_BATCH; ++q) {
+            const int e = fused ? fseq * n2 + fpos + q * (n2 >> 2) : (int)threadIdx.x + q * (int)blockDim.x;
+            if (e < total) {
+                mlo[q] = mid[2 * (base + e)];
+                mhi[q] = mid[2 * (base + e) + 1];
+            }
+        }
+        Fe<P> x[NTT_BATCH];
+        ZK_UNROLL for (int q = 0; q < NTT_BATCH; ++q) {
+            const int e = fused ? fseq * n2 + fpos + q * (n2 >> 2) : (int)threadIdx.x + q * (int)blockDim.x;
+            x[q] = Fe<P>::zero();
+            if (e < total) x[q] = ntt_between_passes<P>(lds_get_u<P>(lds, PL, (e >> log_n2) * SS + ntt_slot(bitrev_n(e & (n2 - 1), log_n2))), mlo[q], mhi[q]);
+        }
+        __syncthreads();
+        if (fused) {
+            ntt_first_round<P>(lds, PL, fseq * SS, log_n2, fpos, fe_relax(fu_unpack<P>(x[0].v)), fe_relax(fu_unpack<P>(x[1].v)), fe_relax(fu_unpack<P>(x[2].v)),
+                               fe_relax(fu_unpack<P>(x[3].v)), plan_b, plen);
+        } else {
+            ZK_UNROLL for (int q = 0; q < NTT_BATCH; ++q) {
+                const int e = (int)threadIdx.x + q * (int)blockDim.x;
+                if (e < total) lds_put_u<P>(lds, PL, (e >> log_n2) * SS + ntt_slot(e & (n2 - 1)), fe_relax(fu_unpack<P>(x[q].v)));
+            }
+        }
+    }
+    __syncthreads();
+    lds_ntt_dif4<P>(lds, PL, SS, log_n2, R, plan_b, plen, fused);
+    {
+        uint4 plo[NTT_BATCH] = {}, phi[NTT_BATCH] = {};
+        ZK_UNROLL for (int q = 0; q < NTT_BATCH; ++q) {
+            const int e = (int)threadIdx.x + q * (int)blockDim.x;
+            if (e < total) {
+                plo[q] = post[2 * (base + e)];
+                phi[q] = post[2 * (base + e) + 1];
+            }
+        }
+        ZK_UNROLL for (int q = 0; q < NTT_BATCH; ++q) {
+            const int e = (int)threadIdx.x + q * (int)blockDim.x;
+            if (e < total) {
+                const int r = e >> log_n2, k = e & (n2 - 1);
+                ntt_store_with<P>(data, base + e, lds_get_u<P>(lds, PL, r * SS + ntt_slot(bitrev_n(k, log_n2))), true, plo[q], phi[q], 0, nullptr, base + e);
             }
         }
     }
diff --git a/zokrates_amd/csrc/ntt_geom.h b/zokrates_amd/csrc/ntt_geom.h
--- a/zokrates_amd/csrc/ntt_geom.h
+++ b/zokrates_amd/csrc/ntt_geom.h
@@ -53,7 +53,9 @@
 }
 inline ShardGeom ntt_whole(const NttGeom& p) { return ntt_shard_geom(p.N1, p.Nb, 1); }
 
-enum NttPass { NTT_COLS, NTT_MID, NTT_ROWS };
+enum NttPass { NTT_COLS, NTT_MID, NTT_ROWS, NTT_ROWS_PAIR, NTT_COLS_QUOTIENT };
+constexpr int NTT_TILE_BATCH = 4;
+inline bool ntt_fuses_quotient(const NttGeom& p) { return p.log1 > 0 && p.log3 == 0; }
 struct NttLaunch {
     uint32_t grid_x, grid_z;
     int threads;
@@ -63,7 +65,7 @@
 };
 inline NttLaunch ntt_pass_shape(const NttGeom& p, NttPass pass, const ShardGeom& g, uint32_t k) {
     if (pass == NTT_MID) return {p.N3 / (uint32_t)p.C_mid, g.rows, p.threads_mid, p.smem_mid, p.C_mid, g.range_origin(k)};
-    const bool cols = pass == NTT_COLS;
+    const bool cols = pass == NTT_COLS || pass == NTT_COLS_QUOTIENT;
     const uint32_t n = cols ? p.N1 : 1u << p.last_log();
     const uint64_t have = cols ? g.W : g.range_len() / n;
     const uint32_t nseq = (uint32_t)std::min<uint64_t>((uint64_t)(cols ? p.C_cols : p.R_rows), have);
diff --git a/zokrates_amd/csrc/ntt_host.cuh b/zokrates_amd/csrc/ntt_host.cuh
--- a/zokrates_amd/csrc/ntt_host.cuh
+++ b/zokrates_amd/csrc/ntt_host.cuh
@@ -129,6 +129,8 @@
               0u, 0u, 0, 1u);
     lds_opt_in(ctx, (const void*)k_ntt_cols<typename Fr::Params>);
     lds_opt_in(ctx, (const void*)k_ntt_rows<typename Fr::Params>);
+    lds_opt_in(ctx, (const void*)k_ntt_rows_pair<typename Fr::Params>);
+    lds_opt_in(ctx, (const void*)k_ntt_cols_quotient<typename Fr::Params>);
     stream_sync(s);
     return pl;
 }
@@ -156,6 +158,18 @@
         ZK_LAUNCH((k_ntt_rows<typename Fr::Params>), dim3(L.grid_x, nvec), dim3(L.threads), L.smem, ctx->ws, data + L.offset, vec_stride, pl->last_log(), L.nseq,
                   ptr<u32>((three ? pl->plan3 : pl->plan2)[inverse ? 1 : 0]), three ? pl->plen3 : pl->plen2, (post && post_mask == ~(u64)0) ? post + L.offset : post, canon,
                   minus ? minus + L.offset : minus, post_mask, ctx->ntt_fuse_first);
+    }
+    static void ntt_rows_pair(zkhip_ctx* ctx, NttPlan<C>* pl, const ShardGeom& g, u32 k, Fr* data, const Fr* mid, const Fr* post, int nvec, u64 vec_stride) {
+        const NttLaunch L = ntt_pass_shape(*pl, NTT_ROWS_PAIR, g, k);
+        require(ntt_fuses_quotient(*pl) && ((u64)L.nseq << pl->log2) <= (u64)NTT_TILE_BATCH * (u64)L.threads, ZKHIP_ERR_DEVICE,
+                "internal: this plan's rows passes do not fuse");
+        ZK_LAUNCH((k_ntt_rows_pair<typename Fr::Params>), dim3(L.grid_x, nvec), dim3(L.threads), L.smem, ctx->ws, data + L.offset, vec_stride, pl->log2, L.nseq,
+                  ptr<u32>(pl->plan2[1]), ptr<u32>(pl->plan2[0]), pl->plen2, mid + L.offset, post + L.offset, ctx->ntt_fuse_first);
+    }
+    static void ntt_cols_quotient(zkhip_ctx* ctx, NttPlan<C>* pl, const ShardGeom& g, u32 k, Fr* data, const Fr& factor) {
+        const NttLaunch L = ntt_pass_shape(*pl, NTT_COLS_QUOTIENT, g, k);
+        ZK_LAUNCH((k_ntt_cols_quotient<typename Fr::Params>), dim3(L.grid_x), dim3(L.threads), L.smem, ctx->ws, data + L.offset, data + pl->N + L.offset, pl->log1,
+                  (u32)pl->Nb, L.nseq, ptr<u32>(pl->plan1[0]), pl->plen1, factor, ctx->ntt_fuse_first);
     }
     static void ntt_kind_a(zkhip_ctx* ctx, NttPlan<C>* pl, Fr* data, bool inverse, const Fr* final_post, int nvec = 1,
                            u64 vec_stride = 0, int canon = 0, const Fr* final_minus = nullptr) {
@@ -178,14 +192,37 @@
             ntt_rows(ctx, pl, w, 0, data, inverse, final_post, nvec, vec_stride, canon);
         }
     }
+    static void to_coset(zkhip_ctx* ctx, NttPlan<C>* pl, Fr* v, int nvec, bool forward_cols = true) {
+        const u64 stride = nvec > 1 ? pl->N : 0;
+        if (!ntt_fuses_quotient(*pl)) {
+            ntt_kind_a(ctx, pl, v, true, ptr<Fr>(pl->s_coset), nvec, stride);
+            ntt_kind_b(ctx, pl, v, false, nullptr, nvec, stride);
+            return;
+        }
+        const ShardGeom w = ntt_whole(*pl);
+        ntt_cols(ctx, pl, w, 0, v, true, ptr<Fr>(pl->tw_inv), nvec, stride);
+        ntt_rows_pair(ctx, pl, w, 0, v, ptr<Fr>(pl->s_coset), ptr<Fr>(pl->tw_fwd), nvec, stride);
+        if (forward_cols) ntt_cols(ctx, pl, w, 0, v, false, nullptr, nvec, stride);
+    }
+    static Fr quotient_factor(const NttPlan<C>* pl, bool bound) { return bound ? fe_from_mont(pl->zinv) : pl->zinv_rp; }
+    static void quotient_last(zkhip_ctx* ctx, NttPlan<C>* pl, Fr* v, Fr* c) {
+        ntt_kind_a(ctx, pl, v, true, ptr<Fr>(pl->s_cosetinv_canon), 1, 0, 1, c);
+    }
     template <class Pointwise>
     static void ntt_quotient(zkhip_ctx* ctx, NttPlan<C>* pl, Fr* v, int nvec, Fr* c, bool bound, Pointwise pointwise) {
-        const u64 stride = nvec > 1 ? pl->N : 0;
-        ntt_kind_a(ctx, pl, v, true, ptr<Fr>(pl->s_coset), nvec, stride);
         if (!bound) ntt_kind_a(ctx, pl, c, true, ptr<Fr>(pl->s_cexit), 1, 0, 1);
-        ntt_kind_b(ctx, pl, v, false, nullptr, nvec, stride);
-        pointwise(bound ? fe_from_mont(pl->zinv) : pl->zinv_rp);
-        if (!bound) ntt_kind_a(ctx, pl, v, true, ptr<Fr>(pl->s_cosetinv_canon), 1, 0, 1, c);
+        to_coset(ctx, pl, v, nvec);
+        pointwise(quotient_factor(pl, bound));
+        if (!bound) quotient_last(ctx, pl, v, c);
+    }
+    static void ntt_quotient(zkhip_ctx* ctx, NttPlan<C>* pl, Fr* v, int nvec, Fr* c, bool bound, std::nullptr_t) {
+        require(nvec == 2, ZKHIP_ERR_DEVICE, "internal: the quotient's product is of two vectors");
+        if (!bound) ntt_kind_a(ctx, pl, c, true, ptr<Fr>(pl->s_cexit), 1, 0, 1);
+        const bool fused = ntt_fuses_quotient(*pl);
+        to_coset(ctx, pl, v, 2, !fused);
+        if (fused) ntt_cols_quotient(ctx, pl, ntt_whole(*pl), 0, v, quotient_factor(pl, bound));
+        else ZK_LAUNCH((k_quotient<typename Fr::Params>), dim3(blocks_for(pl->N, 256)), dim3(256), 0, ctx->ws, v, v + pl->N, quotient_factor(pl, bound), v, pl->N);
+        if (!bound) quotient_last(ctx, pl, v, c);
     }
 
     static bool shard_ok(const NttPlan<C>* pl, size_t G) { return ntt_shardable(pl->log1, pl->N1, pl->Nb, G); }
```

After: 110.6. About the same (-0.2%).
